# Haochen-Wang409/U2PL

Hardware: AMD Instinct MI355X
Metric: train images/sec at 769x769 (R101-DeepLabv3+) (higher is better)
Workload: dtype f32

## Files before the change

### include/u2pl_hip.h

```cpp
#ifndef U2PL_HIP_H
#define U2PL_HIP_H

#include <stddef.h>
#include <stdint.h>

#ifdef __cplusplus
extern "C" {
#endif

#ifndef __HIP_PLATFORM_AMD__
typedef struct ihipStream_t* hipStream_t;
#endif

#define U2PL_SEL_MAX_SLOTS 8
#define U2PL_SEL_WORD_NVALID 0
#define U2PL_SEL_WORD_NTOTAL 1
#define U2PL_SEL_WORD_VAL 40
#define U2PL_SEL_WORD_THR 56

int u2pl_bilinear_up_f32(const float* in, long sn, long sc, long sh, long sw, int N, int C, int h, int w,
                         float* out_nchw, int H, int W, hipStream_t stream);
int u2pl_bilinear_up_bwd_f32(const float* gout_nchw, int N, int C, int H, int W, float* gin, long sn, long sc,
                             long sh, long sw, int h, int w, hipStream_t stream);
int u2pl_pseudo_label_f32(const float* logits_nchw, int N, int C, int H, int W, float* conf, long long* label,
// ... 32 lines not shown
                          int C, long P, void* workspace, float* proto, const unsigned* lowbits,
                          hipStream_t stream);
size_t u2pl_contra_phase1_workspace_bytes(long P, int C, int D);
int u2pl_contra_phase1(const float* prob, long sn, long sc, long sp, const unsigned* lbits, const float* low_mask,
                       const float* high_mask, int N2, int num_labeled, int C, int h, int w, float thr_p, float thr_n,
                       int low_rank, int high_rank, const float* rows, long ld, int D, unsigned* abits, unsigned* lowbits,
                       unsigned* nbits, int* idx, long cap, unsigned* counts, float* proto, void* workspace,
                       hipStream_t stream);
int u2pl_gather_rows_f32(const float* rows, long ld, int D, const int* list, long n, float* out,
                         hipStream_t stream);
size_t u2pl_bank_state_bytes(int C);
int u2pl_bank_init(long long* state, int C, const long long* caps_host, hipStream_t stream);
int u2pl_bank_enqueue_f32(long long* state, float* storage, int D, const float* rows, long ld, const int* idx,
                          long idx_stride, const long long* row_start_dev, const unsigned* counts_dev, int C,
                          hipStream_t stream);
int u2pl_bank_append_f32(float* bank, long cap, long tail, int D, const float* rows, long ld, const int* list,
                         long n_new, hipStream_t stream);
int u2pl_bank_append_multi_f32(const long long* desc_dev, int nclass, int D, long ld, long max_new,
                               hipStream_t stream);
size_t u2pl_infonce_job_bytes(void);
int u2pl_infonce_f32(const void* jobs_dev, int njobs, const float* rep, long ld, int D, int Q, int K,
                     float temp, float* loss_q, float* ganchor, int* anchor_pix, int* head, int* next,
                     const int* seg_len, hipStream_t stream);
size_t u2pl_infonce_fused_workspace_bytes(int njobs, int Q);
int u2pl_infonce_fused_f32(const void* jobs_dev, int njobs, const float* rep, long ld, int D, int Q, int K, float temp,
                           float* loss_q, float* ganchor, int* anchor_pix, int* head, int* next, const int* seg_len,
                           float* zero_dst, long zero_ld, const int* zero_pix, long zero_n, void* workspace,
                           float inv_valid_seg, float* loss, hipStream_t stream);
int u2pl_infonce_reduce_f32(const float* loss_q, int njobs, int Q, float inv_valid_seg, float* loss,
                            hipStream_t stream);
int u2pl_scatter_rows_ordered_f32(float* dst, long ld, int D, const int* pix, const int* next, int* head,
                                  const int* order, const int* seg_pos, const int* seg_len, const float* src, long n,
                                  const float* gout_dev, float scale, hipStream_t stream);
int u2pl_zero_rows_f32(float* dst, long ld, int D, const int* pix, long n, hipStream_t stream);

size_t u2pl_ce_workspace_bytes(void);
int u2pl_ce_fwd_f32(const float* logits_nchw, const long long* target, int ignore, int N, int C, int H, int W,
                    int unsup_weight, void* workspace, float* out3, hipStream_t stream);
int u2pl_ce_bwd_f32(const float* logits_nchw, const long long* target, int ignore, int N, int C, int H, int W,
                    const float* out3_dev, const float* gout_dev, float gmul, float* grad, hipStream_t stream);
int u2pl_ce_fwd_weighted_f32(const float* logits_nchw, const long long* target, int ignore, int N, int C, int H, int W,
                             const float* class_weight, void* workspace, float* out3, hipStream_t stream);
int u2pl_ce_bwd_weighted_f32(const float* logits_nchw, const long long* target, int ignore, int N, int C, int H, int W,
                             const float* class_weight, const float* out3_dev, const float* gout_dev, float gmul,
                             float* grad, hipStream_t stream);
int u2pl_ohem_prob_f32(const float* logits_nchw, const long long* target, int ignore, int N, int C, int H,
                       int W, float* mask_prob, unsigned* ws, hipStream_t stream);
int u2pl_ohem_apply_i64(const float* mask_prob, const unsigned* thr_bits, const long long* target, int ignore,
                        long n, long long* kept_target, hipStream_t stream);
int u2pl_confusion_hist_f32(const float* logits_nchw, const long long* target, int ignore, int N, int C, int H, int W,
                            long long* hist3c, hipStream_t stream);

int u2pl_predict_map_f32(const float* in, long sn, long sc, long sh, long sw, int N, int C, int h, int w, int H, int W,
                         unsigned char* label, const unsigned char* palette, unsigned char* rgb, hipStream_t stream);
int u2pl_infer_input_u8_f32(const unsigned char* img_hwc, int h, int w, const float* lut, float* out_hwc, int H, int W,
                            hipStream_t stream);
int u2pl_window_fuse_f32(float* pred, float* count, int C, int H, int W, const float* in, long sc, long sh, long sw, int h,
                         int w, int h0, int w0, int hc, int wc, int flip, int softmax, float weight, int bump,
                         hipStream_t stream);
int u2pl_predict_entropy_f32(const float* in, long sn, long sc, long sh, long sw, int N, int C, int h, int w, int H, int W,
                             int prob, unsigned char* label, float* entropy, hipStream_t stream);
int u2pl_reliable_map_u8(unsigned char* label, const float* entropy, const unsigned* thr_bits, long n,
                         const unsigned char* palette, unsigned char* rgb, unsigned char* heat, float heat_scale,
                         unsigned* ndropped, hipStream_t stream);
int u2pl_lut_u8(const unsigned char* in, unsigned char* out, long n, const unsigned char* lut256, hipStream_t stream);

int u2pl_conv2d_fwd_f32(const float* x, long ldx, const float* w, const float* bias, float* y, long ldy, int N,
                        int Hin, int Win, int Cin, int Hout, int Wout, int Cout, int R, int S, int stride,
                        int pad, int dil, hipStream_t stream);
int u2pl_conv2d_fwd_stat_blocks(int N, int Hout, int Wout, int Cout);
int u2pl_conv2d_fwd_bnstats_f32(const float* x, long ldx, const float* w, const float* bias, float* y, long ldy,
                                int N, int Hin, int Win, int Cin, int Hout, int Wout, int Cout, int R, int S,
                                int stride, int pad, int dil, const float* pivot, float* stats_partial,
                                hipStream_t stream);
int u2pl_colreduce_finish_f32(const float* partial, int nblk, int C, double* sums, hipStream_t stream);
int u2pl_conv2d_fwd_bnact_f32(const float* x, long ldx, const float* w, const float* bias, float* y, long ldy, int N,
                              int Hin, int Win, int Cin, int Hout, int Wout, int Cout, int R, int S, int stride,
                              int pad, int dil, const float* mean, const float* invstd, const float* gamma,
                              const float* beta, const float* res, long ldr, int relu, hipStream_t stream);
int u2pl_gemm_batched_f32(const float* x, long ldx, long zx, const float* w, long zw, float* y, long ldy, long zy,
                          long M, int K, int Nn, int batch, hipStream_t stream);
size_t u2pl_wino_tiles(int N, int H, int W, int dil, int mt);
int u2pl_wino_stat_blocks(long tiles, int O);
int u2pl_wino_input_f32(const float* x, long ldx, int N, int H, int W, int C, int dil, int mt, float* V,
                        hipStream_t stream);
int u2pl_wino_weight_f32(const float* w, int O, int C, int transposed, int mt, float* U, hipStream_t stream);
int u2pl_wino_gy_f32(const float* gy, long ldg, int N, int H, int W, int O, int dil, int mt, float* Mg,
                     hipStream_t stream);
int u2pl_wgrad_batched_splits(long M, int Cin, int Cout, int batch);
size_t u2pl_wgrad_batched_workspace_bytes(long M, int Cin, int Cout, int batch);
int u2pl_wgrad_batched_f32(const float* dy, long lddy, long zdy, const float* x, long ldx, long zx, float* part,
                           long M, int Cin, int Cout, int batch, hipStream_t stream);
int u2pl_wino_wgrad_finish_f32(const float* part, int nsplit, int O, int C, int mt, int accumulate, float* dw,
                               hipStream_t stream);
int u2pl_wino_output_f32(const float* Mb, int N, int H, int W, int O, int dil, int mt, const float* bias, float* y,
                         long ldy, float* stats_partial, const float* pivot, hipStream_t stream);
int u2pl_wino_output_bnact_f32(const float* Mb, int N, int H, int W, int O, int dil, int mt, const float* bias, float* y,
                               long ldy, const float* mean, const float* invstd, const float* gamma, const float* beta,
                               const float* res, long ldr, int relu, hipStream_t stream);
int u2pl_conv2d_fwd_bf16op_f32(const float* x, long ldx, const float* w, const float* bias, float* y, long ldy, int N,
                               int Hin, int Win, int Cin, int Hout, int Wout, int Cout, int R, int S, int stride,
                               int pad, int dil, hipStream_t stream);
int u2pl_conv2d_fwd_bnstats_bf16op_f32(const float* x, long ldx, const float* w, const float* bias, float* y, long ldy,
                                       int N, int Hin, int Win, int Cin, int Hout, int Wout, int Cout, int R, int S,
                                       int stride, int pad, int dil, const float* pivot, float* stats_partial,
                                       hipStream_t stream);
int u2pl_conv2d_dgrad_bf16op_f32(const float* dy, long lddy, const float* wT, float* dx, long lddx, int N, int Hin,
                                 int Win, int Cin, int Hout, int Wout, int Cout, int R, int S, int stride, int pad,
                                 int dil, hipStream_t stream);
int u2pl_conv2d_wgrad_bf16op_f32(const float* dy, long lddy, const float* x, long ldx, float* dw, void* workspace,
                                 int accumulate, int N, int Hin, int Win, int Cin, int Hout, int Wout, int Cout, int R,
                                 int S, int stride, int pad, int dil, hipStream_t stream);
int u2pl_conv2d_dgrad_f32(const float* dy, long lddy, const float* wT, float* dx, long lddx, int N, int Hin,
                          int Win, int Cin, int Hout, int Wout, int Cout, int R, int S, int stride, int pad,
                          int dil, hipStream_t stream);
int u2pl_weight_transpose_f32(const float* w, float* wt, int Cout, int RS, int Cin, hipStream_t stream);
size_t u2pl_conv2d_wgrad_workspace_bytes(int N, int Hout, int Wout, int Cin, int Cout, int R, int S);
int u2pl_conv2d_wgrad_f32(const float* dy, long lddy, const float* x, long ldx, float* dw, void* workspace,
                          int accumulate, int N, int Hin, int Win, int Cin, int Hout, int Wout, int Cout, int R,
                          int S, int stride, int pad, int dil, hipStream_t stream);
int u2pl_wgrad_set_tr(int on);
int u2pl_im2col_f32(const float* x, long ldx, float* col, int Kp, int N, int Hin, int Win, int Cin, int Hout,
                    int Wout, int R, int S, int stride, int pad, int dil, hipStream_t stream);

int u2pl_gconv2d_fwd_f32(const float* x, long ldx, const float* w, const float* bias, float* y, long ldy, int N, int Hin,
                         int Win, int Cin, int Hout, int Wout, int Cout, int R, int S, int stride, int pad, int dil,
                         int groups, hipStream_t stream);
int u2pl_gconv2d_dgrad_f32(const float* dy, long lddy, const float* w, float* dx, long lddx, int N, int Hin, int Win,
                           int Cin, int Hout, int Wout, int Cout, int R, int S, int stride, int pad, int dil, int groups,
                           hipStream_t stream);
size_t u2pl_gconv2d_wgrad_workspace_bytes(int N, int Hout, int Wout, int Cin, int Cout, int R, int S, int groups);
int u2pl_gconv2d_wgrad_f32(const float* dy, long lddy, const float* x, long ldx, float* dw, void* workspace,
                           int accumulate, int N, int Hin, int Win, int Cin, int Hout, int Wout, int Cout, int R,
                           int S, int stride, int pad, int dil, int groups, hipStream_t stream);

size_t u2pl_weight_split3_bytes(int rows, int K, int batch);
int u2pl_weight_split3_f32(const float* w, long zw, int rows, int K, int batch, void* out, hipStream_t stream);
int u2pl_weight_split3_multi_f32(const void* jobs, int njobs, long total, hipStream_t stream);
int u2pl_weight_split3_pad_rows(int rows);
int u2pl_wino_weight_multi_f32(const void* jobs, int njobs, long total, hipStream_t stream);
int u2pl_igemm_ws_stat_blocks(int N, int Hout, int Wout);
int u2pl_igemm_ws_set_persist(int on);
int u2pl_conv2d_fwd_ws_f32(const float* x, long ldx, const void* wsplit, const float* bias, float* y, long ldy, int N,
                           int Hin, int Win, int Cin, int Hout, int Wout, int Cout, int R, int S, int stride, int pad,
                           int dil, hipStream_t stream);
int u2pl_conv2d_fwd_bnstats_ws_f32(const float* x, long ldx, const void* wsplit, const float* bias, float* y, long ldy,
                                   int N, int Hin, int Win, int Cin, int Hout, int Wout, int Cout, int R, int S,
                                   int stride, int pad, int dil, const float* pivot, float* stats_partial,
                                   hipStream_t stream);
int u2pl_conv2d_fwd_bnact_ws_f32(const float* x, long ldx, const void* wsplit, const float* bias, float* y, long ldy, int N,
                                 int Hin, int Win, int Cin, int Hout, int Wout, int Cout, int R, int S, int stride,
                                 int pad, int dil, const float* mean, const float* invstd, const float* gamma,
                                 const float* beta, const float* res, long ldr, int relu, hipStream_t stream);
int u2pl_conv2d_dgrad_ws_f32(const float* dy, long lddy, const void* wTsplit, float* dx, long lddx, int N, int Hin,
                             int Win, int Cin, int Hout, int Wout, int Cout, int R, int S, int stride, int pad, int dil,
                             hipStream_t stream);
int u2pl_gemm_batched_ws_f32(const float* x, long ldx, long zx, const void* wsplit, float* y, long ldy, long zy, long M,
                             int K, int Nn, int batch, hipStream_t stream);

size_t u2pl_weight_split2h_bytes(int rows, int K, int batch);
int u2pl_weight_split2h_f32(const float* w, long zw, int rows, int K, int batch, void* out, void* job_scratch, hipStream_t stream);
int u2pl_weight_split2h_multi_f32(const void* jobs, int njobs, long total, hipStream_t stream);
int u2pl_weight_rebuild2h_job_bytes(void);
int u2pl_weight_rebuild2h_span(int which);
int u2pl_weight_rebuild2h_f32(const void* jobs, int n_flat, int n_wino, long seg_total, long amax_total, int wino_mblocks,
                              int wino_pblocks, hipStream_t stream);
int u2pl_amax_words(void);
int u2pl_absmax_f32(const float* x, long ld, long M, int C, float* out, int clear, hipStream_t stream);
int u2pl_bn_apply_amax_f32(const float* x, long ldx, const float* mean, const float* invstd, const float* gamma, const float* beta,
                           const float* res, long ldr, int relu, const float* drop, long rows_per_image, float* y, long ldy, long M,
                           int C, float* y_amax, hipStream_t stream);
int u2pl_bn_bwd_apply_amax_f32(const float* dy, long lddy, const float* x, long ldx, const float* y, long ldy, const float* mean,
                               const float* invstd, const float* gamma, const float* drop, long rows_per_image, const double* sums,
                               double count, float* dx, long lddx, float* dres, long lddr, long M, int C, const double* psums,
                               float* gsink, float* bsink, int accumulate, float* dx_amax, float* dres_amax, const float* relu_beta,
                               hipStream_t stream);
int u2pl_bn_bwd_sums_mx_f32(const float* dy, long lddy, const float* x, long ldx, const float* mean, const float* invstd,
                            const float* gamma, const float* beta, const float* drop, long rows_per_image, long M, int C,
                            void* workspace, double* sums, hipStream_t stream);
int u2pl_bn_apply_bits_f32(const float* x, long ldx, const float* mean, const float* invstd, const float* gamma, const float* beta,
                           const float* res, long ldr, int relu, const float* drop, long rows_per_image, float* y, long ldy, long M,
                           int C, float* y_amax, unsigned* bits, long ldb, hipStream_t stream);
int u2pl_bn_bwd_sums_bits_f32(const float* dy, long lddy, const float* x, long ldx, const unsigned* bits, long ldb,
                              const float* mean, const float* invstd, const float* drop, long rows_per_image, long M, int C,
                              void* workspace, double* sums, hipStream_t stream);
int u2pl_bn_bwd_apply_bits_f32(const float* dy, long lddy, const float* x, long ldx, const unsigned* bits, long ldb,
                               const float* mean, const float* invstd, const float* gamma, const float* drop, long rows_per_image,
                               const double* sums, double count, float* dx, long lddx, float* dres, long lddr, long M, int C,
                               const double* psums, float* gsink, float* bsink, int accumulate, float* dx_amax, float* dres_amax,
                               hipStream_t stream);
int u2pl_wino_input_amax_f32(const float* x, long ldx, int N, int H, int W, int C, int dil, int mt, float* V, float* v_amax,
                             hipStream_t stream);
int u2pl_wino_output_bnact_amax_f32(const float* Mb, int N, int H, int W, int O, int dil, int mt, const float* bias, float* y,
                                    long ldy, const float* mean, const float* invstd, const float* gamma, const float* beta,
                                    const float* res, long ldr, int relu, float* y_amax, hipStream_t stream);
int u2pl_wino_gy_amax_f32(const float* gy, long ldg, int N, int H, int W, int O, int dil, int mt, float* Mg, float* mg_amax,
                          hipStream_t stream);
int u2pl_conv2d_fwd_wsh_f32(const float* x, long ldx, const float* x_amax, const void* wsplit, const float* bias, float* y, long ldy,
                            int N, int Hin, int Win, int Cin, int Hout, int Wout, int Cout, int R, int S, int stride, int pad,
                            int dil, hipStream_t stream);
int u2pl_conv2d_fwd_bnstats_wsh_f32(const float* x, long ldx, const float* x_amax, const void* wsplit, const float* bias, float* y,
                                    long ldy, int N, int Hin, int Win, int Cin, int Hout, int Wout, int Cout, int R, int S,
                                    int stride, int pad, int dil, const float* pivot, float* stats_partial, hipStream_t stream);
int u2pl_conv2d_fwd_bnact_wsh_f32(const float* x, long ldx, const float* x_amax, const void* wsplit, const float* bias, float* y,
                                  long ldy, int N, int Hin, int Win, int Cin, int Hout, int Wout, int Cout, int R, int S,
                                  int stride, int pad, int dil, const float* mean, const float* invstd, const float* gamma,
                                  const float* beta, const float* res, long ldr, int relu, float* y_amax, hipStream_t stream);
int u2pl_conv2d_dgrad_wsh_f32(const float* dy, long lddy, const float* dy_amax, const void* wTsplit, float* dx, long lddx, int N,
                              int Hin, int Win, int Cin, int Hout, int Wout, int Cout, int R, int S, int stride, int pad, int dil,
                              hipStream_t stream);
int u2pl_gemm_batched_wsh_f32(const float* x, long ldx, long zx, const float* x_amax, const void* wsplit, float* y, long ldy, long zy,
                              long M, int K, int Nn, int batch, hipStream_t stream);
int u2pl_wgrad_h_eligible(int Cin, int Cout);
int u2pl_conv2d_wgrad_h_f32(const float* dy, long lddy, const float* dy_amax, const float* x, long ldx, const float* x_amax, float* dw,
                            void* workspace, int accumulate, int N, int Hin, int Win, int Cin, int Hout, int Wout, int Cout, int R,
                            int S, int stride, int pad, int dil, hipStream_t stream);
int u2pl_wgrad_batched_h_f32(const float* dy, long lddy, long zdy, const float* dy_amax, const float* x, long ldx, long zx,
                             const float* x_amax, float* part, long M, int Cin, int Cout, int batch, hipStream_t stream);

size_t u2pl_colreduce_workspace_bytes(long Mseg, int nseg, int C);
int u2pl_bn_stats_f32(const float* x, long ld, long M, int C, const float* pivot, void* workspace, double* sums,
                      hipStream_t stream);
int u2pl_colsum_f32(const float* x, long ld, long Mseg, int nseg, int C, void* workspace, double* sums,
                    hipStream_t stream);
int u2pl_bn_bwd_sums_f32(const float* dy, long lddy, const float* x, long ldx, const float* y, long ldy,
                         const float* mean, const float* invstd, const float* drop, long rows_per_image, long M,
                         int C, void* workspace, double* sums, hipStream_t stream);
int u2pl_bn_finalize_f32(const double* sums, double count, const float* pivot, int C, float eps, float momentum,
                         float* mean, float* invstd, float* running_mean, float* running_var, hipStream_t stream);
int u2pl_bn_eval_invstd_f32(const float* running_var, int C, float eps, float* invstd, hipStream_t stream);
int u2pl_bn_finish_finalize_f32(const float* partial, int nblk, int C, double count, const float* pivot, float eps,
                                float momentum, float* mean, float* invstd, float* running_mean, float* running_var,
                                double* sums_out, hipStream_t stream);
size_t u2pl_bn_eval_invstd_job_bytes(void);
int u2pl_bn_eval_invstd_multi_f32(const void* jobs_dev, int njobs, long total, hipStream_t stream);
int u2pl_bn_apply_f32(const float* x, long ldx, const float* mean, const float* invstd, const float* gamma,
                      const float* beta, const float* res, long ldr, int relu, const float* drop,
                      long rows_per_image, float* y, long ldy, long M, int C, hipStream_t stream);
int u2pl_bn_bwd_apply_f32(const float* dy, long lddy, const float* x, long ldx, const float* y, long ldy,
                          const float* mean, const float* invstd, const float* gamma, const float* drop,
                          long rows_per_image, const double* sums, double count, float* dx, long lddx, float* dres,
                          long lddr, long M, int C, hipStream_t stream);
int u2pl_bn_bwd_apply_pg_f32(const float* dy, long lddy, const float* x, long ldx, const float* y, long ldy,
                             const float* mean, const float* invstd, const float* gamma, const float* drop,
                             long rows_per_image, const double* sums, double count, float* dx, long lddx, float* dres,
                             long lddr, long M, int C, const double* psums, float* gsink, float* bsink, int accumulate,
                             hipStream_t stream);
int u2pl_sums_to_f32(const double* sums, int n, float scale, int accumulate, float* out, hipStream_t stream);
int u2pl_maxpool3s2_fwd_f32(const float* x, long ldx, int N, int H, int W, int C, int Ho, int Wo, float* y, long ldy,
                            unsigned char* tap, hipStream_t stream);
int u2pl_maxpool3s2_bwd_f32(const float* dy, long lddy, const unsigned char* tap, int N, int H, int W, int C, int Ho,
                            int Wo, float* dx, long lddx, hipStream_t stream);
int u2pl_copy_rows_f32(const float* src, long lds, float* dst, long ldd, long M, int C, int accumulate,
                       hipStream_t stream);
int u2pl_copy_cols_f32(const float* src, long lds, float* dst, long ldd, long M, int C, hipStream_t stream);
int u2pl_broadcast_rows_f32(const float* v, long ldv, float scale, float* dst, long ldd, long rows_per_image, long M,
                            int C, hipStream_t stream);
int u2pl_bilinear_rows_fwd_f32(const float* x, long ldx, int N, int h, int w, int C, int H, int W, float* y, long ldy,
                               hipStream_t stream);
int u2pl_bilinear_rows_bwd_f32(const float* dy, long lddy, int N, int h, int w, int C, int H, int W, float* dx,
                               long lddx, hipStream_t stream);
int u2pl_softmax_rows_f32(const float* x, long ldx, float* y, long ldy, long M, int C, hipStream_t stream);
int u2pl_sgd_step_f32(float* p, const float* g, float* buf, long n, long b1, long b2, float lr0, float lr1, float lr2,
                      float momentum, float weight_decay, int first, float grad_scale, hipStream_t stream);
int u2pl_ema_update_f32(float* t, const float* s, long n, float decay, float one_minus_decay, hipStream_t stream);
int u2pl_adam_step_f32(float* p, const float* g, float* exp_avg, float* exp_avg_sq, long n, long b1, long b2, float lr0,
                       float lr1, float lr2, float beta1, float beta2, float eps, float weight_decay,
                       float bias_correction1, float bias_correction2_sqrt, float grad_scale, hipStream_t stream);
size_t u2pl_kernel_launches(void);
int u2pl_conv_set_split(int on);
int u2pl_conv_get_split(void);
int u2pl_debug_phase1_times(unsigned* buf);
size_t u2pl_reliability_fused_workspace_bytes(int G);
size_t u2pl_reliability_fused_cand_floats(long n_px, int G);
int u2pl_reliability_fused(const float* logits_low, long sn, long sc, long sh, long sw, int B, int C, int h, int w,
                           int H, int W, const long long* label_u, const long long* label_l, int ignore, int nspec,
                           const float* q32_host, int negative_high_entropy, int hm, int wm, float* entropy,
                           long long* target_u, float* low_mask, float* high_mask, unsigned* lbits,
                           unsigned* workspace, float* cand, int G, unsigned epoch, int flags, hipStream_t stream);
int u2pl_cutmix_f32(const float* img, const long long* label, const float* conf, const int* boxes_dev, int B, int C,
                    int H, int W, float* out_img, long long* out_label, float* out_conf, hipStream_t stream);

int u2pl_dense_small_f32(const float* x, long ldx, const float* w, const float* bias, float* y, long ldy, int M, int K,
                         int Cout, hipStream_t stream);
int u2pl_strong_aug_f32(const float* img, const long long* label, const float* conf, const int* boxes_dev,
                        const unsigned long long* sel_dev, int mode, int B, int C, int H, int W, float* out_img,
                        long long* out_label, float* out_conf, hipStream_t stream);
int u2pl_label_presence_i64(const long long* label, int B, long HW, unsigned long long* bits, hipStream_t stream);

int u2pl_window_accumulate_f32(float* pred, float* count, int C, int H, int W, const float* src, int h0, int w0,
                               int hc, int wc, hipStream_t stream);
int u2pl_window_normalize_f32(float* pred, const float* count, int C, int H, int W, hipStream_t stream);

int u2pl_augment_u8_f32(const unsigned char* img, const unsigned char* lab, const int* params, int B, int H, int W,
                        int Sh, int Sw, const float* mean3, const float* std3, float* out_img, long long* out_lab,
                        hipStream_t stream);

#define U2PL_AUG_REC 16
#define U2PL_AUG_ROTATE 1
#define U2PL_AUG_BLUR 2
size_t u2pl_augment_ex_scratch_bytes(int B, int Sh, int Sw, int mode);
int u2pl_augment_ex_u8_f32(const unsigned char* img, const unsigned char* lab, const long long* offsets,
                           const int* records, int B, int H, int W, int Sh, int Sw, int ignore_label, int mode,
                           const float* mean3, const float* std3, const float* blur_w, float* scratch, float* out_img,
                           long long* out_lab, hipStream_t stream);
int u2pl_augment_lut_u8_f32(const unsigned char* img, const unsigned char* lab, const long long* offsets,
                            const int* records, int B, int H, int W, int Sh, int Sw, int ignore_label, int mode,
                            const unsigned char* lut256, const float* mean3, const float* std3, const float* blur_w,
                            float* scratch, float* out_img, long long* out_lab, hipStream_t stream);

int u2pl_half_weight_f16(const float* w, int Cout, int Cin, int R, int S, unsigned short* out, hipStream_t stream);
int u2pl_hconv2d_fwd_f16(const unsigned short* x, long ldx, const unsigned short* w, const float* scale,
                         const float* shift, const unsigned short* res, long ldr, void* y, long ldy, int N, int Hin,
                         int Win, int Cin, int Hout, int Wout, int Cout, int R, int S, int stride, int pad, int dil,
                         int relu, int out_f32, int tile, int* sat, hipStream_t stream);
int u2pl_hconv2d_stem_f16(const float* x, long ldx, const unsigned short* w, const float* scale, const float* shift,
                          unsigned short* y, long ldy, int N, int Hin, int Win, int Cin, int Hout, int Wout, int Cout,
                          int R, int S, int stride, int pad, int dil, int relu, int* sat, hipStream_t stream);
int u2pl_hmaxpool3s2_f16(const unsigned short* x, long ldx, int N, int H, int W, int C, int Ho, int Wo,
                         unsigned short* y, long ldy, hipStream_t stream);
int u2pl_hgap_f16(const unsigned short* x, long ldx, int N, int HW, int C, unsigned short* y, hipStream_t stream);
int u2pl_hbilinear_f16(const unsigned short* x, long ldx, int N, int h, int w, int C, unsigned short* y, long ldy,
                       int H, int W, hipStream_t stream);

int u2pl_wide_words(int C);
int u2pl_reliability_masks_wide(const float* entropy, const unsigned* thr_lo_bits, const unsigned* thr_hi_bits,
                                const long long* label_l, const long long* label_u, int ignore, int B, int H, int W,
                                int h, int w, int negative_high_entropy, int C, float* low_mask, float* high_mask,
                                unsigned* lbits, hipStream_t stream);
int u2pl_reliability_apply_wide(const float* entropy, const unsigned* thr_bits, const long long* label_l,
                                const long long* label_u, int ignore, int B, int H, int W, int h, int w,
                                int negative_high_entropy, int C, long long* target_u, unsigned* nkept, float* low_mask,
                                float* high_mask, unsigned* lbits, hipStream_t stream);
int u2pl_pack_class_bits_wide(const long long* onehot, int N, int C, int h, int w, unsigned* bits, hipStream_t stream);
int u2pl_unpack_class_bits_wide(const unsigned* bits, int N, int C, int h, int w, long long* onehot, hipStream_t stream);
size_t u2pl_contra_wide_workspace_bytes(long P, int C);
int u2pl_contra_wide_block_pixels(int C);
int u2pl_contra_wide_staged(int C);
int u2pl_contra_classify_wide(const float* prob, long sn, long sc, long sp, const unsigned* lbits, const float* low_mask,
                              const float* high_mask, int N2, int num_labeled, int C, int h, int w, float thr_p,
                              float thr_n, int low_rank, int high_rank, unsigned* abits, unsigned* lowbits,
                              unsigned* nbits, void* workspace, unsigned* counts, long long* offsets,
                              hipStream_t stream);
int u2pl_compact_lists_wide(const unsigned* abits, const unsigned* lowbits, const unsigned* nbits, long P, int C,
                            const void* workspace, const long long* offsets, int* idx, long idx_len,
                            hipStream_t stream);
int u2pl_class_prototypes_wide(const float* rows, long ld, int D, const int* idx, const long long* offsets,
                               const unsigned* counts, int C, float* proto, hipStream_t stream);
int u2pl_bank_init_wide(long long* state, int C, const long long* caps_host, hipStream_t stream);
int u2pl_bank_enqueue_wide_f32(long long* state, float* storage, int D, const float* rows, long ld, const int* idx,
                               const long long* list_off_dev, const long long* row_start_dev,
                               const unsigned* counts_dev, int C, hipStream_t stream);

#ifdef __cplusplus
}
#endif
#endif
```

### u2pl_amd/csrc/common.h

```cpp
#pragma once
#include <hip/hip_runtime.h>
#include <stdint.h>

#define U2PL_API extern "C" __attribute__((visibility("default")))

#define U2PL_LAUNCH_CHECK()                      \
    do {                                         \
        hipError_t e__ = hipGetLastError();      \
        if (e__ != hipSuccess) return (int)e__;  \
    } while (0)

#define U2PL_EINVAL 1001

#include <atomic>
extern std::atomic<unsigned long long> u2pl_kernel_launch_count;
#define U2PL_LAUNCH(...)                        \
    do {                                        \
        u2pl_kernel_launch_count.fetch_add(1, std::memory_order_relaxed);             \
        hipLaunchKernelGGL(__VA_ARGS__);        \
    } while (0)

#ifdef U2PL_HBM_MAXW
#define U2PL_HBM_KERNEL __attribute__((amdgpu_waves_per_eu(1, U2PL_HBM_MAXW)))
#else
// ... 2 lines not shown

static inline int cdiv(long a, long b) { return (int)((a + b - 1) / b); }
static inline int grid_for(long n, int block, int max_blocks = 256 * 16) {
    long g = (n + block - 1) / block;
    if (g > max_blocks) g = max_blocks;
    if (g < 1) g = 1;
    return (int)g;
}

__device__ __forceinline__ float wave_sum(float v) {
#pragma unroll
    for (int o = 32; o > 0; o >>= 1) v += __shfl_xor(v, o, 64);
    return v;
}
template <int CTRL>
__device__ __forceinline__ float dpp_add(float v) {
    return v + __builtin_bit_cast(float, __builtin_amdgcn_update_dpp(0, __builtin_bit_cast(int, v), CTRL, 0xf, 0xf, false));
}
__device__ __forceinline__ float wave_allsum_dpp(float v) {
    v = dpp_add<0x128>(v);
    v = dpp_add<0x124>(v);
    v = dpp_add<0x122>(v);
    v = dpp_add<0x121>(v);
    const int b = __builtin_bit_cast(int, v);
    const float r0 = __builtin_bit_cast(float, __builtin_amdgcn_readlane(b, 0)), r1 = __builtin_bit_cast(float, __builtin_amdgcn_readlane(b, 16));
    const float r2 = __builtin_bit_cast(float, __builtin_amdgcn_readlane(b, 32)), r3 = __builtin_bit_cast(float, __builtin_amdgcn_readlane(b, 48));
    return (r0 + r1) + (r2 + r3);
}
__device__ __forceinline__ float wave_sum_sgpr(float v) {
    v = dpp_add<0x128>(v);
    v = dpp_add<0x124>(v);
    v = dpp_add<0x122>(v);
    v = dpp_add<0x121>(v);
    v += __builtin_bit_cast(float, __builtin_amdgcn_update_dpp(0, __builtin_bit_cast(int, v), 0x142, 0xa, 0xf, false));
    v += __builtin_bit_cast(float, __builtin_amdgcn_update_dpp(0, __builtin_bit_cast(int, v), 0x143, 0xc, 0xf, false));
    return __builtin_bit_cast(float, __builtin_amdgcn_readlane(__builtin_bit_cast(int, v), 63));
}
__device__ __forceinline__ float lane_put(float old, float val, int lane) {
    return (int)(threadIdx.x & 63) == lane ? val : old;
}
__device__ __forceinline__ float lane_get(float v, int lane) {
    return __builtin_bit_cast(float, __builtin_amdgcn_readlane(__builtin_bit_cast(int, v), lane));
}
__device__ __forceinline__ double wave_sum_d(double v) {
#pragma unroll
    for (int o = 32; o > 0; o >>= 1) v += __shfl_xor(v, o, 64);
    return v;
}
__device__ __forceinline__ unsigned wave_sum_u(unsigned v) {
#pragma unroll
    for (int o = 32; o > 0; o >>= 1) v += __shfl_xor(v, o, 64);
    return v;
}
__device__ __forceinline__ float wave_max(float v) {
#pragma unroll
    for (int o = 32; o > 0; o >>= 1) v = fmaxf(v, __shfl_xor(v, o, 64));
    return v;
}

#define U2PL_AMAX_SHARDS 64
#define U2PL_AMAX_STRIDE 32
#define U2PL_AMAX_WORDS (U2PL_AMAX_SHARDS * U2PL_AMAX_STRIDE)
__device__ __forceinline__ unsigned amax_bits(unsigned m, float v) {
    const unsigned b = __float_as_uint(v) & 0x7fffffffu;
    return b > m ? b : m;
}
__device__ __forceinline__ unsigned amax_bits4(unsigned m, float4 v) {
    return amax_bits(amax_bits(amax_bits(amax_bits(m, v.x), v.y), v.z), v.w);
}
__device__ __forceinline__ unsigned wave_max_u(unsigned m) {
#pragma unroll
    for (int o = 32; o > 0; o >>= 1) {
        const unsigned t = (unsigned)__shfl_xor((int)m, o, 64);
        m = t > m ? t : m;
    }
    return m;
}
__device__ __forceinline__ void amax_wave_publish(unsigned m, unsigned* __restrict__ obj) {
    m = wave_max_u(m);
    if ((threadIdx.x & 63) == 0 && m != 0u) {
        const unsigned wave = blockIdx.x * (blockDim.x >> 6) + (threadIdx.x >> 6);
        atomicMax(obj + (wave & (U2PL_AMAX_SHARDS - 1)) * U2PL_AMAX_STRIDE, m);
    }
}
__device__ __forceinline__ unsigned amax_read(const unsigned* __restrict__ obj) {
    const unsigned v = *(const __attribute__((address_space(1))) unsigned*)(obj + (threadIdx.x & 63) * U2PL_AMAX_STRIDE);
    return (unsigned)__builtin_amdgcn_readfirstlane((int)wave_max_u(v));
}

__device__ __forceinline__ void block_count_flush(unsigned cnt, unsigned* __restrict__ dst) {
    __shared__ unsigned s_cnt;
    if (threadIdx.x == 0) s_cnt = 0;
    __syncthreads();
    cnt = wave_sum_u(cnt);
    if ((threadIdx.x & 63) == 0 && cnt) atomicAdd(&s_cnt, cnt);
    __syncthreads();
    if (threadIdx.x == 0 && s_cnt) atomicAdd(dst, s_cnt);
}

__device__ __forceinline__ unsigned f32_key(float f) {
    unsigned u = __float_as_uint(f);
    return (u & 0x80000000u) ? ~u : (u | 0x80000000u);
}
__device__ __forceinline__ float key_f32(unsigned k) {
    unsigned u = (k & 0x80000000u) ? (k & 0x7fffffffu) : ~k;
    return __uint_as_float(u);
}

struct AcCoord {
    int i0, i1;
    float l0, l1;
};
__device__ __forceinline__ AcCoord ac_coord(int dst, float scale, int in_size) {
    AcCoord c;
    float src = __fmul_rn((float)dst, scale);
    c.i0 = (int)src;
    if (c.i0 > in_size - 1) c.i0 = in_size - 1;
    c.i1 = c.i0 + (c.i0 < in_size - 1 ? 1 : 0);
    c.l1 = __fsub_rn(src, (float)c.i0);
    c.l0 = __fsub_rn(1.0f, c.l1);
    return c;
}
static inline float ac_scale_host(long in, long out) {
    return out > 1 ? (float)(in - 1) / (float)(out - 1) : 0.0f;
}
__device__ __forceinline__ int nearest_src(int dst, float scale, int in_size) {
    int s = (int)floorf(__fmul_rn((float)dst, scale));
    return s < in_size - 1 ? s : in_size - 1;
}

typedef unsigned int u32x4 __attribute__((ext_vector_type(4)));
#define OOB_OFF ((int)0x80000000u)
__device__ __forceinline__ __amdgpu_buffer_rsrc_t make_rsrc(const void* p, unsigned bytes) {
    return __builtin_amdgcn_make_buffer_rsrc((void*)p, (short)0, (int)bytes, 0x00020000);
}
__device__ __forceinline__ float4 buf_load4s(__amdgpu_buffer_rsrc_t r, int lane_off, int uniform_off) {
    u32x4 v = __builtin_amdgcn_raw_buffer_load_b128(r, lane_off, uniform_off, 0);
    return make_float4(__uint_as_float(v.x), __uint_as_float(v.y), __uint_as_float(v.z), __uint_as_float(v.w));
}
__device__ __forceinline__ float4 buf_load4(__amdgpu_buffer_rsrc_t r, int byte_off) {
    u32x4 v = __builtin_amdgcn_raw_buffer_load_b128(r, byte_off, 0, 0);
    return make_float4(__uint_as_float(v.x), __uint_as_float(v.y), __uint_as_float(v.z), __uint_as_float(v.w));
}

#define U2PL_GLOBAL __attribute__((address_space(1)))
template <class T>
__device__ __forceinline__ T ldg(const T* p) { return *(const U2PL_GLOBAL T*)p; }

struct BnEpi {
    const float *mean, *invstd, *gamma, *beta, *res;
    long ldr;
    int relu;
    unsigned* y_amax;
};
```

### u2pl_amd/csrc/igemm_ws.hip

```cpp
#include <stdlib.h>
#include <type_traits>
#include "common.h"
#include "conv_geom.h"
#include "u2pl_hip.h"
#include "wino_t.h"

template <int B, int E, class F>
__device__ __forceinline__ void static_for(F&& f) {
    if constexpr (B < E) {
        f(std::integral_constant<int, B>{});
        static_for<B + 1, E>(f);
    }
}

#define WS_ROW_B 64
__host__ __device__ static inline int ws_pad_rows(int rows) { return rows <= 128 ? 128 : (rows + 255) & ~255; }

__global__ void k_weight_split3(const float* __restrict__ w, long zw, unsigned short* __restrict__ out, long zo, int rows,
                                int Np, int K) {
    w += (long)blockIdx.y * zw;
    out += (long)blockIdx.y * zo;
    const int nseg = K / 8;
    const long total = (long)Np * nseg;
    for (long i = blockIdx.x * (long)blockDim.x + threadIdx.x; i < total; i += (long)gridDim.x * blockDim.x) {
// ... 371 lines not shown
        const unsigned dk_q = (8u * dq) / Cout, dk_r = 8u * dq - dk_q * Cout;
        for (; i < jend; i += 256) {
            const int n = j.kind == 0 ? (int)slow : (int)fst, sg = j.kind == 0 ? (int)fst : (int)slow;
            float4 v0 = make_float4(0.f, 0.f, 0.f, 0.f), v1 = v0;
            if (n < j.rows) {
                if (j.kind == 0) {
                    const float4* src = (const float4*)(j.src + (long)n * j.K + sg * 8);
                    v0 = src[0];
                    v1 = src[1];
                } else {
                    float e[8];
                    unsigned rs = rs0, co = co0;
#pragma unroll
                    for (int q = 0; q < 8; ++q) {
                        e[q] = j.src[((long)co * j.RS + rs) * j.rows + n];
                        if (++co == Cout) { co = 0; ++rs; }
                    }
                    v0 = make_float4(e[0], e[1], e[2], e[3]);
                    v1 = make_float4(e[4], e[5], e[6], e[7]);
                }
            }
            uint2 a0, a1, b0, b1;
            split2_f16(v0, sc, a0, a1);
            split2_f16(v1, sc, b0, b1);
            const int c = sg >> 2, s_ = sg & 3;
            const long base = (((long)c * 2) * j.Np + n) * 32 + ((s_ ^ ((n >> 2) & 3)) << 3);
            *(uint4*)(j.out + base) = make_uint4(a0.x, a0.y, b0.x, b0.y);
            *(uint4*)(j.out + base + pl) = make_uint4(a1.x, a1.y, b1.x, b1.y);
            slow += dq;
            fst += dr;
            rs0 += dk_q;
            co0 += dk_r;
            if (fst >= fast) { fst -= fast; ++slow; co0 += 8u; }
            while (co0 >= Cout) { co0 -= Cout; ++rs0; }
        }
        if (i >= end) return;
    }
}
template <int MT>
__device__ __forceinline__ void rb_pieces_wino(const RebuildJob& j, int lb) {
    constexpr int A = WinoT<MT>::A;
    const bool tr = j.kind == 3;
    const int C = tr ? j.rows : j.K;
    const unsigned total = (unsigned)j.Np * (unsigned)(j.K >> 3);
    const unsigned* __restrict__ amax = rb_tail(j);
    const long pl = (long)j.Np * 32, zs = (long)(j.K / 32) * 2 * pl;
    unsigned u = (unsigned)lb * RB_WINO_PSPAN + threadIdx.x;
    const int s_ = (int)(u & 3);
    int c = (int)((u >> 2) / (unsigned)j.Np), n = (int)((u >> 2) - (unsigned)c * (unsigned)j.Np);
    for (int it = 0; it < RB_WINO_PSPAN / 256 && u < total; ++it, u += 256) {
        const int k0 = c * 32 + s_ * 8;
        const bool live = n < j.rows;
        float tp[9][8];
        if (!tr) {
            const float* __restrict__ p = j.src + (long)(live ? n : 0) * 9 * C + k0;
#pragma unroll
            for (int t = 0; t < 9; ++t) {
                const float4 lo = *(const float4*)(p + (long)t * C), hi = *(const float4*)(p + (long)t * C + 4);
                tp[t][0] = lo.x; tp[t][1] = lo.y; tp[t][2] = lo.z; tp[t][3] = lo.w;
                tp[t][4] = hi.x; tp[t][5] = hi.y; tp[t][6] = hi.z; tp[t][7] = hi.w;
            }
        } else {
            const float* __restrict__ p = j.src + (long)k0 * 9 * C + (live ? n : 0);
#pragma unroll
            for (int q = 0; q < 8; ++q)
#pragma unroll
                for (int t = 0; t < 9; ++t) tp[8 - t][q] = p[((long)q * 9 + t) * C];
        }
        unsigned short* __restrict__ out = j.out + (((long)c * 2) * j.Np + n) * 32 + ((s_ ^ ((n >> 2) & 3)) << 3);
        static_for<0, A>([&](auto i_c) __attribute__((always_inline)) {
            constexpr int I = decltype(i_c)::value;
            float comp[A][8];
#pragma unroll
            for (int q = 0; q < 8; ++q) {
                float r[A];
                wino_filter_row<MT, I>([&](int r_, int s) { return tp[r_ * 3 + s][q]; }, r);
#pragma unroll
                for (int jj = 0; jj < A; ++jj) comp[jj][q] = live ? r[jj] : 0.f;
            }
#pragma unroll
            for (int jj = 0; jj < A; ++jj) {
                const int z = I * A + jj;
                const float sc = split2_scale(split2_exp_bits(amax[z]));
                uint2 a0, a1, b0, b1;
                split2_f16(make_float4(comp[jj][0], comp[jj][1], comp[jj][2], comp[jj][3]), sc, a0, a1);
                split2_f16(make_float4(comp[jj][4], comp[jj][5], comp[jj][6], comp[jj][7]), sc, b0, b1);
                *(uint4*)(out + z * zs) = make_uint4(a0.x, a0.y, b0.x, b0.y);
                *(uint4*)(out + z * zs + pl) = make_uint4(a1.x, a1.y, b1.x, b1.y);
            }
        });
        n += 64;
        if (n >= j.Np) { n -= j.Np; ++c; }
    }
}
__global__ __launch_bounds__(256) void k_rebuild_pieces_wino(const RebuildJob* __restrict__ wj, int n_wino) {
    const int b = (int)blockIdx.x;
    const int ji = rb_find(n_wino, b, [&](int m) { return (long)wj[m].pblk_begin; });
    const RebuildJob j = wj[ji];
    if (j.mt == 4) rb_pieces_wino<4>(j, b - j.pblk_begin);
    else rb_pieces_wino<2>(j, b - j.pblk_begin);
}
U2PL_API int u2pl_weight_rebuild2h_job_bytes(void) { return (int)sizeof(RebuildJob); }
U2PL_API int u2pl_weight_rebuild2h_span(int which) { return which == 0 ? WS_AMAX_SPAN : which == 1 ? RB_WINO_MSPAN : which == 2 ? RB_WINO_PSPAN : 0; }
U2PL_API int u2pl_weight_rebuild2h_f32(const void* jobs, int n_flat, int n_wino, long seg_total, long amax_total, int wino_mblocks,
                                       int wino_pblocks, hipStream_t stream) {
    if (n_flat < 0 || n_wino < 0 || seg_total < 0 || amax_total < 0 || wino_mblocks < 0 || wino_pblocks < 0) return U2PL_EINVAL;
    if ((n_flat == 0) != (seg_total == 0) || (n_flat == 0) != (amax_total == 0)) return U2PL_EINVAL;
    if ((n_wino == 0) != (wino_mblocks == 0) || (n_wino == 0) != (wino_pblocks == 0)) return U2PL_EINVAL;
    if (n_flat + n_wino == 0) return 0;
    const RebuildJob* rj = (const RebuildJob*)jobs;
    const int flat_blocks = cdiv(amax_total, WS_AMAX_SPAN);
    U2PL_LAUNCH(k_rebuild_clear, dim3(cdiv(n_flat + n_wino, 256)), dim3(256), 0, stream, rj, n_flat + n_wino);
    U2PL_LAUNCH_CHECK();
    U2PL_LAUNCH(k_rebuild_amax, dim3((unsigned)(flat_blocks + wino_mblocks)), dim3(256), 0, stream, rj, n_flat, n_wino, amax_total, flat_blocks);
    U2PL_LAUNCH_CHECK();
    if (n_flat) {
        U2PL_LAUNCH(k_rebuild_pieces_flat, dim3((unsigned)cdiv(seg_total, WS_AMAX_SPAN)), dim3(256), 0, stream, rj, n_flat, seg_total);
        U2PL_LAUNCH_CHECK();
    }
    if (n_wino) {
        U2PL_LAUNCH(k_rebuild_pieces_wino, dim3((unsigned)wino_pblocks), dim3(256), 0, stream, rj + n_flat, n_wino);
        U2PL_LAUNCH_CHECK();
    }
    return 0;
}
__global__ void k_absmax_rows(const float* __restrict__ x, long ld, long M, int C4, unsigned* __restrict__ out) {
    const long total = M * C4;
    unsigned m = 0;
    for (long i = blockIdx.x * (long)blockDim.x + threadIdx.x; i < total; i += (long)gridDim.x * blockDim.x) {
        const long r = i / C4;
        const int c = (int)(i - r * C4);
        m = amax_bits4(m, *(const float4*)(x + r * ld + c * 4));
    }
    amax_wave_publish(m, out);
}
U2PL_API int u2pl_amax_words(void) { return U2PL_AMAX_WORDS; }
U2PL_API int u2pl_absmax_f32(const float* x, long ld, long M, int C, float* out, int clear, hipStream_t stream) {
    if (M < 0 || C <= 0 || (C & 3) || (ld & 3)) return U2PL_EINVAL;
    if (clear) {
        hipError_t e = hipMemsetAsync(out, 0, (size_t)U2PL_AMAX_WORDS * 4, stream);
        if (e != hipSuccess) return (int)e;
    }
    if (M == 0) return 0;
    U2PL_LAUNCH(k_absmax_rows, dim3(grid_for(M * (C / 4), 512, 2048)), dim3(512), 0, stream, x, ld, M, C / 4, (unsigned*)out);
    U2PL_LAUNCH_CHECK();
    return 0;
}

#ifdef U2PL_WS_STAMPS
__device__ unsigned long long* d_ws_stamps;
static unsigned long long* g_ws_stamps = nullptr;
U2PL_API int u2pl_igemm_ws_set_stamp_buffer(void* p) { g_ws_stamps = (unsigned long long*)p; return 0; }
#endif
template <int TM, int TN, int WM, int WN, bool PW, int ABL = 0, int NP = 3>
__device__ __forceinline__ void igemm_ws_body(
    const float* __restrict__ x, long ldx, const float* __restrict__ x_amax, const unsigned short* __restrict__ ws,
    const unsigned* __restrict__ b_amax, const float* __restrict__ bias,
    float* __restrict__ y, long ldy, const ConvGeom& g, unsigned xbytes, unsigned wsbytes, unsigned ybytes, unsigned resbytes, int Np,
    float* __restrict__ stats, const float* __restrict__ pivot, long zx, long zws, long zy, const BnEpi& epi, int mtiles, int ntiles,
    int total_tiles, int tile0, const int bid, const int G) {
    constexpr int BM = 32 * TM * WM, BN = 32 * TN * WN, NT = 64 * WM * WN;
    constexpr int RPP = NT / 8, RA = BM / RPP;
    constexpr int UB = NP * BN * 4, RBU = UB / NT;
    static_assert(BM % RPP == 0 && UB % NT == 0, "tile / thread-count mismatch");
    static_assert(NP == 2 || NP == 3, "pieces per operand");
    constexpr int A_ST = NP * BM * WS_ROW_B, B_ST = NP * BN * WS_ROW_B, ST = A_ST + B_ST;
    constexpr int NPROD = NP == 3 ? 6 : 3;
    using C0 = std::integral_constant<int, 0>;
    using C1 = std::integral_constant<int, 1>;

    auto tile_of = [&](int v, int& mt, int& nt, int& z) __attribute__((always_inline)) {
        const int xcd = v & 7, j = v >> 3;
        const int q = total_tiles >> 3, r = total_tiles & 7;
        const int t = tile0 + (xcd < r ? xcd * (q + 1) : r * (q + 1) + (xcd - r) * q) + j;
        nt = t % ntiles;
        const int rest = t / ntiles;
        mt = rest % mtiles;
        z = rest / mtiles;
    };
    __amdgpu_buffer_rsrc_t rx = make_rsrc(x, xbytes), rw = make_rsrc(ws, wsbytes), ry = make_rsrc(y, ybytes);
    extern __shared__ __attribute__((aligned(16))) unsigned char smem[];
#ifdef U2PL_WS_STAMPS
    unsigned long long ph[4];
    ph[0] = __builtin_readcyclecounter();
#endif

    const int tid = threadIdx.x, lane = tid & 63, wave = tid >> 6;
    const int wm = wave / WN, wn = wave % WN;
    const long M = (long)g.N * g.Hout * g.Wout;
    const int K = g.R * g.S * g.Cin;
    const int nk = K / BK;
    int ea = 0;
    float sa = 1.f;
    if constexpr (NP == 2) {
        ea = split2_exp_bits(amax_read((const unsigned*)x_amax));
        sa = split2_scale(ea);
    }
    const int nk2 = (nk + 1) & ~1;
    const int n_my = (total_tiles - bid + G - 1) / G;
    const int cpt = g.S * (g.Cin / BK);
    auto tile_taps = [&](int mt, int& rb_, int& re_) __attribute__((always_inline)) {
        rb_ = 0;
        re_ = g.R;
        if constexpr (!PW) {
            if (g.R > 1) {
                const long mf = (long)mt * BM, ml_ = mf + BM - 1, ml = ml_ < M ? ml_ : M - 1;
                const unsigned hw = (unsigned)(g.Hout * g.Wout);
                const unsigned nf = (unsigned)mf / hw, nl = (unsigned)ml / hw;
                const int hf = (int)(((unsigned)mf - nf * hw) / (unsigned)g.Wout), hl = (int)(((unsigned)ml - nl * hw) / (unsigned)g.Wout);
                const int lim = g.Hin << g.log2div;
                auto reach = [&](int r, int ha, int hb) { return hb * g.mul + g.off_h + r * g.step >= 0 && ha * g.mul + g.off_h + r * g.step < lim; };
                int lo = g.R, hi = -1;
                for (int r = 0; r < g.R; ++r) {
                    const bool ok = nf == nl ? reach(r, hf, hl)
                                             : (reach(r, hf, g.Hout - 1) || reach(r, 0, hl) || (nl > nf + 1 && reach(r, 0, g.Hout - 1)));
                    if (ok) { lo = r < lo ? r : lo; hi = r; }
                }
                if (hi >= 0) { rb_ = lo; re_ = hi + 1; } else { rb_ = 0; re_ = 1; }
                rb_ = __builtin_amdgcn_readfirstlane(rb_);
                re_ = __builtin_amdgcn_readfirstlane(re_);
            }
        }
    };

    const int kq = tid & 7, r0 = tid >> 3;
    const int ldxb = (int)ldx * 4;
    int a_v = bid, a_kc = 0, a_c0 = 0, a_r = 0, a_s = 0;
    int a_nk = nk, a_nk2 = nk2;
    int bh[RA], bw[RA], nb[RA];
    bool mv[RA];
    int aoff[RA];
    auto a_tile_setup = [&]() __attribute__((always_inline)) {
        int mt, nt, z;
        tile_of(a_v, mt, nt, z);
        rx = make_rsrc(x + (long)__builtin_amdgcn_readfirstlane(z) * zx, xbytes);
        if constexpr (!PW) {
            int rb_, re_;
            tile_taps(mt, rb_, re_);
            a_r = rb_;
            a_nk = (re_ - rb_) * cpt;
            a_nk2 = (a_nk + 1) & ~1;
        }
#pragma unroll
        for (int i = 0; i < RA; ++i) {
            const long m = (long)mt * BM + r0 + RPP * i;
            mv[i] = m < M;
            const unsigned mm = mv[i] ? (unsigned)m : 0u;
            if constexpr (PW) {
                aoff[i] = mv[i] ? (int)mm * ldxb + kq * 16 : OOB_OFF;
            } else {
                const unsigned tq = mm / (unsigned)g.Wout;
                const int wo = (int)(mm - tq * (unsigned)g.Wout);
                const unsigned n_ = tq / (unsigned)g.Hout;
                const int ho = (int)(tq - n_ * (unsigned)g.Hout);
                bh[i] = ho * g.mul + g.off_h;
                bw[i] = wo * g.mul + g.off_w;
                nb[i] = (int)n_ * g.Hin * g.Win;
            }
        }
    };
    a_tile_setup();
    float4 ra[2][RA];
    u32x4 rb[RBU];
    auto load_a_row = [&](auto set_c, auto i_c) __attribute__((always_inline)) {
        constexpr int SET = decltype(set_c)::value, i = decltype(i_c)::value;
        const bool live = a_kc < a_nk;
        if constexpr (PW) {
            ra[SET][i] = buf_load4s(rx, live ? aoff[i] : OOB_OFF, a_kc * (BK * 4));
        } else {
            int ih, iw;
            const bool okh = gather_coord(bh[i], a_r, g.step, g.log2div, g.Hin, ih);
            const bool okw = gather_coord(bw[i], a_s, g.step, g.log2div, g.Win, iw);
            const int off = (nb[i] + ih * g.Win + iw) * ldxb + kq * 16;
            ra[SET][i] = buf_load4s(rx, (live & mv[i] & okh & okw) ? off : OOB_OFF, a_c0 * 4);
        }
    };
    auto advance_a = [&]() __attribute__((always_inline)) {
        if (a_kc + 1 < a_nk2) {
            ++a_kc;
            a_c0 += BK;
            if (a_c0 == g.Cin) {
                a_c0 = 0;
                if (++a_s == g.S) { a_s = 0; ++a_r; }
            }
        } else if (a_v + G < total_tiles) {
            a_v += G;
            a_kc = a_c0 = a_r = a_s = 0;
            a_tile_setup();
        }
    };
    auto load_a = [&](auto set_c) __attribute__((always_inline)) {
        static_for<0, RA>([&](auto i) __attribute__((always_inline)) { load_a_row(set_c, i); });
        advance_a();
    };
    int boff[RBU];
    int blds[RBU];
#pragma unroll
    for (int j = 0; j < RBU; ++j) {
        const int u = tid + j * NT, p = u / (BN * 4), wi = u - p * (BN * 4);
        boff[j] = p * Np * WS_ROW_B + wi * 16;
        blds[j] = A_ST + p * BN * WS_ROW_B + wi * 16;
    }
    const int chunk_b = NP * Np * WS_ROW_B;
    int b_v = bid, b_kc = 0, b_toff = 0;
    int b_nk = nk, b_nk2 = nk2, b_base = 0;
    auto b_tile_setup = [&]() __attribute__((always_inline)) {
        int mt, nt, z;
// ... 138 lines not shown
        constexpr int LD_START = (BS_START + RBU + RBU + RA <= NMF) ? BS_START + RBU : NMF - RBU - RA;
        static_assert(F1_START + NRD <= TAIL + NPROD * PER, "k block 1 operands would be read after their first use");
        static_assert(LD_START + RBU + RA <= NMF && LD_START >= BS_START && LD_START >= SP_START + SP_N, "plan does not fit the chunk");
        using CUR = std::integral_constant<int, cur>;
#ifdef U2PL_WS_STAMPS
        unsigned long long ts[14];
        ts[0] = __builtin_readcyclecounter();
#endif
        if constexpr (!(ABL & 16)) static_for<0, F0_PRE>([&](auto j) __attribute__((always_inline)) { do_read(CUR{}, C0{}, j); });
        __builtin_amdgcn_sched_barrier(0);
        static_for<0, NMF>([&](auto sl_c) __attribute__((always_inline)) {
            constexpr int sl = decltype(sl_c)::value;
#ifdef U2PL_WS_STAMPS
            if constexpr (sl % 4 == 0 && sl != 0) ts[sl / 4] = __builtin_readcyclecounter();
#endif
            do_mfma(std::integral_constant<int, (sl < TAIL ? NMF - TAIL + sl : sl - TAIL)>{});
            if constexpr (!(ABL & 16)) {
                if constexpr (sl < TAIL)
                    static_for<0, F0_PER>([&](auto u) __attribute__((always_inline)) { do_read(CUR{}, C0{}, std::integral_constant<int, F0_PRE + sl * F0_PER + decltype(u)::value>{}); });
                if constexpr (sl >= F1_START) do_read(CUR{}, C1{}, std::integral_constant<int, sl - F1_START>{});
            }
            if constexpr (sl >= SP_START && sl < SP_START + SP_N) {
                constexpr int k = (sl - SP_START) / SPS, step = (sl - SP_START) % SPS;
                if constexpr (step == 0) {
                    const float4 v = ra[nxt][k >> 1];
                    sp_l = (k & 1) ? v.z : v.x;
                    sp_h = (k & 1) ? v.w : v.y;
                }
                unsigned w;
                if constexpr (ABL & 1) w = (__float_as_uint(sp_h) & 0xffff0000u) | (__float_as_uint(sp_l) >> 16);
                else if constexpr (NP == 2) {
                    if constexpr (step == 0) w = split2_first(sp_l, sp_h, sa);
                    else w = split2_second(sp_l, sp_h, sa, (k & 1) ? pc[0].y : pc[0].x);
                } else {
                    if constexpr (step == 0) w = pack2_bf16_first(sp_l, sp_h);
                    else w = pack2_bf16(sp_l, sp_h);
                    if constexpr (step < 2) {
                        sp_l = sp_l - bf16_lo_f(w);
                        sp_h = sp_h - bf16_hi_f(w);
                    }
                }
                if constexpr (k & 1) pc[step].y = w; else pc[step].x = w;
                if constexpr ((k & 1) && step == SPS - 1) {
                    if constexpr (ABL & 4) {
                        asm volatile("" ::"v"(pc[0].x), "v"(pc[0].y), "v"(pc[1].x), "v"(pc[1].y));
                        if constexpr (NP == 3) asm volatile("" ::"v"(pc[2].x), "v"(pc[2].y));
                    } else {
                        unsigned char* d = smem + nxt * ST + alds[k >> 1];
                        *(uint2*)d = pc[0];
                        *(uint2*)(d + BM * WS_ROW_B) = pc[1];
                        if constexpr (NP == 3) *(uint2*)(d + 2 * BM * WS_ROW_B) = pc[2];
                    }
                }
            }
            if constexpr (sl >= BS_START && sl < BS_START + RBU) {
                constexpr int k = sl - BS_START;
                if constexpr (ABL & 2) { asm volatile("" ::"v"(rb[k].x), "v"(rb[k].y), "v"(rb[k].z), "v"(rb[k].w)); }
                else store_b(nxt, k);
            }
            if constexpr (!(ABL & 8)) {
                if constexpr (sl >= LD_START && sl < LD_START + RBU) {
                    load_b_unit(std::integral_constant<int, sl - LD_START>{});
                    if constexpr (sl == LD_START + RBU - 1) advance_b();
                }
                if constexpr (sl >= LD_START + RBU && sl < LD_START + RBU + RA) {
                    load_a_row(std::integral_constant<int, nxt>{}, std::integral_constant<int, sl - LD_START - RBU>{});
                    if constexpr (sl == LD_START + RBU + RA - 1) advance_a();
                }
            }
            __builtin_amdgcn_sched_barrier(0);
        });
#ifdef U2PL_WS_STAMPS
        ts[12] = __builtin_readcyclecounter();
#endif
        if constexpr (!(ABL & 32)) __syncthreads();
#ifdef U2PL_WS_STAMPS
        ts[13] = __builtin_readcyclecounter();
        {
            const int bsel = blockIdx.x == 0 ? 0 : blockIdx.x == 100 ? 1 : -1;
            if (d_ws_stamps && bsel >= 0 && kc >= 8 && kc < 12 && (wave == 0 || wave == (WM * WN) / 2) && lane == 0)
                for (int i = 0; i < 14; ++i) d_ws_stamps[((bsel * 2 + (wave != 0)) * 4 + (kc - 8)) * 14 + i] = ts[i];
        }
#endif
    };

    int c_v = bid;
    int c_nk2 = nk2;
    auto c_tile_setup = [&]() __attribute__((always_inline)) {
        if constexpr (!PW) {
            if (c_v < total_tiles) {
                int mt, nt, z, rb_, re_;
                tile_of(c_v, mt, nt, z);
                tile_taps(mt, rb_, re_);
                c_nk2 = ((re_ - rb_) * cpt + 1) & ~1;
            }
        }
    };
    c_tile_setup();
    float* red = (float*)(smem + 2 * ST);
    unsigned y_am = 0u;
#ifdef U2PL_WS_STAMPS
    int te_n = 0;
#endif
    auto tile_end = [&]() __attribute__((always_inline)) {
#ifdef U2PL_WS_STAMPS
        unsigned long long te[5];
        te[0] = __builtin_readcyclecounter();
#endif
        int mt, nt, z;
        tile_of(c_v, mt, nt, z);
        const int n0 = nt * BN;
        const long m0 = (long)mt * BM;
        int tid = threadIdx.x;
        asm volatile("" : "+v"(tid));
        const int lane = tid & 63, li = lane & 31, lh = lane >> 5;
        (void)lane;
        const int zs = __builtin_amdgcn_readfirstlane(z);
        ry = make_rsrc(y + (long)zs * zy, ybytes);
        const bool bn_all = epi.mean != nullptr;
        const unsigned cbytes = (unsigned)g.Cout * 4u;
        auto colparam = [&](const float* p, int col) __attribute__((always_inline)) {
            return p ? __uint_as_float(__builtin_amdgcn_raw_buffer_load_b32(make_rsrc(p, cbytes), col * 4, 0, 0)) : 0.f;
        };
        float bias_v[TN], mu[TN], is[TN], ga[TN], be[TN], pv[TN];
#pragma unroll
        for (int b = 0; b < TN; ++b) {
            const int col = n0 + wn * 32 * TN + b * 32 + li;
            bias_v[b] = colparam(bias, col);
            mu[b] = is[b] = ga[b] = be[b] = pv[b] = 0.f;
            if (bn_all) { mu[b] = colparam(epi.mean, col); is[b] = colparam(epi.invstd, col); ga[b] = colparam(epi.gamma, col); be[b] = colparam(epi.beta, col); }
            if (stats) pv[b] = colparam(pivot, col);
        }
        int dexp = 0;
        if constexpr (NP == 2) dexp = -(ea + split2_exp_bits(__builtin_amdgcn_readfirstlane((int)ldg(b_amax + zs))));
        __builtin_amdgcn_sched_barrier(0);
        static_for<0, TAIL>([&](auto sl) __attribute__((always_inline)) { do_mfma(std::integral_constant<int, NMF - TAIL + decltype(sl)::value>{}); });
        if constexpr (NP == 2) {
#pragma unroll
            for (int a = 0; a < TM; ++a)
#pragma unroll
                for (int b = 0; b < TN; ++b)
#pragma unroll
                    for (int e = 0; e < 16; ++e) acc[a][b][e] = __builtin_ldexpf(acc[a][b][e], dexp);
        }
#ifdef U2PL_WS_STAMPS
        te[1] = te[2] = __builtin_readcyclecounter();
#endif
        __builtin_amdgcn_sched_barrier(0);
        const int ldyb = (int)ldy * 4;
        const int mrow = (int)m0 + wm * 32 * TM + 4 * lh;
        if (bn_all) {
            const int ldrb = (int)epi.ldr * 4;
            const __amdgpu_buffer_rsrc_t rr = make_rsrc(epi.res, resbytes);
#pragma unroll
            for (int b = 0; b < TN; ++b) {
                const int col = n0 + wn * 32 * TN + b * 32 + li;
                float rv[TM][16];
                if (epi.res) {
#pragma unroll
                    for (int a = 0; a < TM; ++a) {
                        const int rbase = col < g.Cout ? ((mrow + a * 32) * (int)epi.ldr + col) * 4 : OOB_OFF;
#pragma unroll
                        for (int e = 0; e < 16; ++e)
                            rv[a][e] = __uint_as_float(__builtin_amdgcn_raw_buffer_load_b32(rr, rbase + ((e & 3) + 8 * (e >> 2)) * ldrb, 0, 0));
                    }
                }
#pragma unroll
                for (int a = 0; a < TM; ++a)
#pragma unroll
                    for (int e = 0; e < 16; ++e) {
                        float v = acc[a][b][e] + bias_v[b];
                        v = (v - mu[b]) * is[b] * ga[b] + be[b];
                        if (epi.res) v += rv[a][e];
                        if (epi.relu) v = fmaxf(v, 0.f);
                        acc[a][b][e] = v;
                        if (epi.y_amax && col < g.Cout && (long)(mrow + a * 32 + (e & 3) + 8 * (e >> 2)) < M) y_am = amax_bits(y_am, v);
                    }
            }
            __builtin_amdgcn_sched_barrier(0);
        }
#pragma unroll
        for (int b = 0; b < TN; ++b) {
            const int col = n0 + wn * 32 * TN + b * 32 + li;
            const float badd = bn_all ? 0.f : bias_v[b];
#pragma unroll
            for (int a = 0; a < TM; ++a) {
                const int vbase = col < g.Cout ? ((mrow + a * 32) * (int)ldy + col) * 4 : OOB_OFF;
#pragma unroll
                for (int e = 0; e < 16; ++e) {
                    const float v = bn_all ? acc[a][b][e] : acc[a][b][e] + badd;
                    __builtin_amdgcn_raw_buffer_store_b32(__float_as_uint(v), ry, vbase + ((e & 3) + 8 * (e >> 2)) * ldyb, 0, 0);
                }
            }
        }
        __builtin_amdgcn_sched_barrier(0);
        if (stats && !bn_all) {
            static_assert(BM == 128, "statistics blocks are 128 rows");
            const long left = M - m0;
            const int lim = (int)(left < BM ? left : BM) - (wm * 32 * TM + 4 * lh);
#pragma unroll
            for (int b = 0; b < TN; ++b) {
                const int cl = wn * 32 * TN + b * 32 + li;
                const float sh = bias_v[b] - pv[b];
#pragma unroll
                for (int a = 0; a < TM; ++a) {
                    float s1 = 0.f, s2 = 0.f;
#pragma unroll
                    for (int e = 0; e < 16; ++e) {
                        const float v = (a * 32 + (e & 3) + 8 * (e >> 2)) < lim ? acc[a][b][e] + sh : 0.f;
                        s1 += v;
                        s2 += v * v;
                    }
                    s1 += __shfl_xor(s1, 32, 64);
                    s2 += __shfl_xor(s2, 32, 64);
                    if (lh == 0) {
                        red[((wm * TM + a) * 2 + 0) * BN + cl] = s1;
                        red[((wm * TM + a) * 2 + 1) * BN + cl] = s2;
                    }
                }
            }
            __syncthreads();
            float* out = stats + (long)mt * 2 * g.Cout;
            for (int c = tid; c < BN; c += NT) {
                const int co = n0 + c;
                if (co < g.Cout) {
                    float a1 = red[0 * BN + c], a2 = red[1 * BN + c];
#pragma unroll
                    for (int r = 1; r < 4; ++r) { a1 += red[(2 * r) * BN + c]; a2 += red[(2 * r + 1) * BN + c]; }
                    out[co] = a1;
                    out[g.Cout + co] = a2;
                }
            }
        }
#pragma unroll
        for (int a = 0; a < TM; ++a)
#pragma unroll
            for (int b = 0; b < TN; ++b)
#pragma unroll
                for (int e = 0; e < 16; ++e) acc[a][b][e] = 0.f;
        zero_tail_operands();
        c_v += G;
        c_tile_setup();
#ifdef U2PL_WS_STAMPS
        te[3] = __builtin_readcyclecounter();
        asm volatile("s_waitcnt vmcnt(0)" ::: "memory");
        te[4] = __builtin_readcyclecounter();
        if (d_ws_stamps && blockIdx.x == 0 && (wave == 0 || wave == 5) && lane == 0 && te_n < 4)
            for (int i = 0; i < 5; ++i) d_ws_stamps[224 + 4096 + ((wave != 0) * 4 + te_n) * 5 + i] = te[i];
        ++te_n;
#endif
    };
    for (int it = 0; it < n_my; ++it) {
        for (kc = 0; kc < c_nk2; kc += 2) {
            chunk(C0{});
            chunk(C1{});
        }
        tile_end();
    }
    if (epi.y_amax) amax_wave_publish(y_am, epi.y_amax);
#ifdef U2PL_WS_STAMPS
    ph[2] = ph[3] = __builtin_readcyclecounter();
    if (d_ws_stamps && blockIdx.x < 1024 && tid == 0)
        for (int i = 0; i < 4; ++i) d_ws_stamps[224 + blockIdx.x * 4 + i] = ph[i];
#endif
}

template <int TM, int TN, int WM, int WN, bool PW, int ABL = 0, int NP = 3>
__global__ __launch_bounds__(64 * WM * WN, (WM * WN) / 4) void k_igemm_ws(
    const float* __restrict__ x, long ldx, const float* __restrict__ x_amax, const unsigned short* __restrict__ ws,
    const unsigned* __restrict__ b_amax, const float* __restrict__ bias,
    float* __restrict__ y, long ldy, ConvGeom g, unsigned xbytes, unsigned wsbytes, unsigned ybytes, unsigned resbytes, int Np,
    float* __restrict__ stats, const float* __restrict__ pivot, long zx, long zws, long zy, BnEpi epi, int mtiles, int ntiles,
    int total_tiles, int tile0) {
    igemm_ws_body<TM, TN, WM, WN, PW, ABL, NP>(x, ldx, x_amax, ws, b_amax, bias, y, ldy, g, xbytes, wsbytes, ybytes, resbytes, Np, stats,
                                               pivot, zx, zws, zy, epi, mtiles, ntiles, total_tiles, tile0, (int)blockIdx.x, (int)gridDim.x);
}
template <bool PW, int NP = 3>
__global__ __launch_bounds__(512, 2) void k_igemm_ws_mix(
    const float* __restrict__ x, long ldx, const float* __restrict__ x_amax, const unsigned short* __restrict__ ws,
    const unsigned* __restrict__ b_amax, const float* __restrict__ bias,
    float* __restrict__ y, long ldy, ConvGeom g, unsigned xbytes, unsigned wsbytes, unsigned ybytes, unsigned resbytes, int Np,
    float* __restrict__ stats, const float* __restrict__ pivot, long zx, long zws, long zy, BnEpi epi, int mtiles, int ntiles_w,
    int nwide, int wide_tiles, int narrow_tiles) {
    if ((int)blockIdx.x < nwide)
        igemm_ws_body<2, 2, 2, 4, PW, 0, NP>(x, ldx, x_amax, ws, b_amax, bias, y, ldy, g, xbytes, wsbytes, ybytes, resbytes, Np, stats, pivot,
                                             zx, zws, zy, epi, mtiles, ntiles_w, wide_tiles, 0, (int)blockIdx.x, nwide);
    else
        igemm_ws_body<2, 1, 2, 4, PW, 0, NP>(x, ldx, x_amax, ws, b_amax, bias, y, ldy, g, xbytes, wsbytes, ybytes, resbytes, Np, stats, pivot,
                                             zx, zws, zy, epi, mtiles, 2 * ntiles_w, narrow_tiles, 2 * wide_tiles, (int)blockIdx.x - nwide,
                                             (int)gridDim.x - nwide);
}

#define WS_NUM_CUS 256
static double ws_fix2() {
    static double v = -1.0;
    if (v < 0) { const char* e = getenv("U2PL_WS_FIX2"); v = (e && *e) ? atof(e) : 2.0; }
    return v;
}
static int g_ws_persist = -1;
static int ws_persist() {
    if (g_ws_persist < 0) { const char* e = getenv("U2PL_WS_PERSIST"); g_ws_persist = (e && *e) ? (atoi(e) != 0) : 1; }
    return g_ws_persist;
}
U2PL_API int u2pl_igemm_ws_set_persist(int on) { const int old = ws_persist(); g_ws_persist = on != 0; return old; }
template <int TM, int TN, int WM, int WN, bool PW, int ABL = 0, int NP = 3>
static int launch_igemm_ws(const float* x, long ldx, const float* x_amax, const void* ws, const float* bias, float* y, long ldy,
                           const ConvGeom& g, hipStream_t stream, float* stats, const float* pivot, int batch, long zx,
                           long zy, const BnEpi* epi, long tile_first = 0, long tile_count = -1) {
    constexpr int BM = 32 * TM * WM, BN = 32 * TN * WN;
    const long M = (long)g.N * g.Hout * g.Wout;
    if (M <= 0) return 0;
    const int K = g.R * g.S * g.Cin, Np = ws_pad_rows(g.Cout);
    const BnEpi ep = epi ? *epi : BnEpi{nullptr, nullptr, nullptr, nullptr, nullptr, 0, 0, nullptr};
    const size_t lds = (size_t)2 * NP * (BM + BN) * WS_ROW_B + (size_t)8 * BN * sizeof(float);
    static bool attr_set = false;
    if (!attr_set) {
        (void)hipFuncSetAttribute((const void*)k_igemm_ws<TM, TN, WM, WN, PW, ABL, NP>, hipFuncAttributeMaxDynamicSharedMemorySize, (int)lds);
        attr_set = true;
    }
    if (NP == 2 && !x_amax) return U2PL_EINVAL;
    const long xb = (((long)g.N * g.Hin * g.Win - 1) * ldx + g.Cin) * 4;
    const long yb = ((M - 1) * ldy + g.Cout) * 4;
    const long wsb1 = (long)(K / 32) * NP * Np * WS_ROW_B;
    const unsigned* b_amax = (const unsigned*)((const char*)ws + (size_t)batch * wsb1);
    if (xb >= (1L << 31) || wsb1 >= (1L << 31) || yb >= (1L << 31)) return U2PL_EINVAL;
    const long resb = ep.res ? ((M - 1) * ep.ldr + g.Cout) * 4 : 0;
    if (resb >= (1L << 31)) return U2PL_EINVAL;
    const int mtiles = cdiv(M, BM), ntiles = cdiv(g.Cout, BN);
    const long all_tiles = (long)mtiles * ntiles * batch;
    if (all_tiles >= (1L << 30)) return U2PL_EINVAL;
    const long total = tile_count < 0 ? all_tiles : tile_count;
    if (total <= 0) return 0;
    const unsigned grid = (unsigned)((total < WS_NUM_CUS || !ws_persist()) ? total : WS_NUM_CUS);
#ifdef U2PL_WS_STAMPS
    (void)hipMemcpyToSymbolAsync(HIP_SYMBOL(d_ws_stamps), &g_ws_stamps, sizeof(void*), 0, hipMemcpyHostToDevice, stream);
#endif
    U2PL_LAUNCH((k_igemm_ws<TM, TN, WM, WN, PW, ABL, NP>), dim3(grid), dim3(64 * WM * WN), lds, stream, x, ldx, x_amax,
                (const unsigned short*)ws, b_amax, bias, y, ldy, g, (unsigned)xb, (unsigned)wsb1, (unsigned)yb, (unsigned)resb, Np, stats, pivot, zx,
                wsb1 / 2, zy, ep, mtiles, ntiles, (int)total, (int)tile_first);
    U2PL_LAUNCH_CHECK();
    return 0;
}

template <bool PW, int NP = 3>
static int launch_igemm_ws_mix(const float* x, long ldx, const float* x_amax, const void* ws, const float* bias, float* y, long ldy,
                               const ConvGeom& g, hipStream_t stream, float* stats, const float* pivot, int batch, long zx,
                               long zy, const BnEpi* epi, long wide_tiles, long narrow_tiles) {
    const long M = (long)g.N * g.Hout * g.Wout;
    const int K = g.R * g.S * g.Cin, Np = ws_pad_rows(g.Cout);
    const BnEpi ep = epi ? *epi : BnEpi{nullptr, nullptr, nullptr, nullptr, nullptr, 0, 0, nullptr};
    const size_t lds = (size_t)2 * NP * (128 + 256) * WS_ROW_B + (size_t)8 * 256 * sizeof(float);
    static bool attr_set = false;
    if (!attr_set) {
        (void)hipFuncSetAttribute((const void*)k_igemm_ws_mix<PW, NP>, hipFuncAttributeMaxDynamicSharedMemorySize, (int)lds);
        attr_set = true;
    }
    if (NP == 2 && !x_amax) return U2PL_EINVAL;
    const long xb = (((long)g.N * g.Hin * g.Win - 1) * ldx + g.Cin) * 4;
    const long yb = ((M - 1) * ldy + g.Cout) * 4;
    const long wsb1 = (long)(K / 32) * NP * Np * WS_ROW_B;
    const unsigned* b_amax = (const unsigned*)((const char*)ws + (size_t)batch * wsb1);
    if (xb >= (1L << 31) || wsb1 >= (1L << 31) || yb >= (1L << 31)) return U2PL_EINVAL;
    const long resb = ep.res ? ((M - 1) * ep.ldr + g.Cout) * 4 : 0;
    if (resb >= (1L << 31)) return U2PL_EINVAL;
    const int mtiles = cdiv(M, 128), ntw = cdiv(g.Cout, 256);
    if ((long)mtiles * 2 * ntw * batch >= (1L << 30)) return U2PL_EINVAL;
    U2PL_LAUNCH((k_igemm_ws_mix<PW, NP>), dim3((unsigned)(WS_NUM_CUS + narrow_tiles)), dim3(512), lds, stream, x, ldx, x_amax,
                (const unsigned short*)ws, b_amax, bias, y, ldy, g, (unsigned)xb, (unsigned)wsb1, (unsigned)yb, (unsigned)resb, Np, stats, pivot, zx,
                wsb1 / 2, zy, ep, mtiles, ntw, WS_NUM_CUS, (int)wide_tiles, (int)narrow_tiles);
    U2PL_LAUNCH_CHECK();
    return 0;
}

#ifdef U2PL_WS_ABLATE
static int g_ws_abl = 0;
U2PL_API int u2pl_igemm_ws_set_ablate(int v) { const int old = g_ws_abl; g_ws_abl = v; return old; }
#endif

template <int NP>
static int run_igemm_ws_np(const float* x, long ldx, const float* x_amax, const void* ws, const float* bias, float* y, long ldy,
                           const ConvGeom& g, hipStream_t stream, float* stats, const float* pivot, int batch, long zx, long zy,
                           const BnEpi* epi) {
    if (g.Cin % BK || !ws) return U2PL_EINVAL;
    if (epi && (stats || batch != 1 || (g.Cout & 3))) return U2PL_EINVAL;
    const bool pw = g.R == 1 && g.S == 1 && g.mul == 1 && g.off_h == 0 && g.off_w == 0 && g.log2div == 0 &&
                    g.Hin == g.Hout && g.Win == g.Wout;
    auto go = [&](bool narrow, long first, long count) {
        if (!narrow) return pw ? launch_igemm_ws<2, 2, 2, 4, true, 0, NP>(x, ldx, x_amax, ws, bias, y, ldy, g, stream, stats, pivot, batch, zx, zy, epi, first, count)
                               : launch_igemm_ws<2, 2, 2, 4, false, 0, NP>(x, ldx, x_amax, ws, bias, y, ldy, g, stream, stats, pivot, batch, zx, zy, epi, first, count);
        return pw ? launch_igemm_ws<2, 1, 2, 4, true, 0, NP>(x, ldx, x_amax, ws, bias, y, ldy, g, stream, stats, pivot, batch, zx, zy, epi, first, count)
                  : launch_igemm_ws<2, 1, 2, 4, false, 0, NP>(x, ldx, x_amax, ws, bias, y, ldy, g, stream, stats, pivot, batch, zx, zy, epi, first, count);
    };
#ifdef U2PL_WS_ABLATE
    if (g_ws_abl && g.Cout > 128 && pw) {
#define WS_ABL(A_) case A_: return launch_igemm_ws<2, 2, 2, 4, true, A_, NP>(x, ldx, x_amax, ws, bias, y, ldy, g, stream, stats, pivot, batch, zx, zy, epi)
        switch (g_ws_abl) { WS_ABL(1); WS_ABL(2); WS_ABL(4); WS_ABL(8); WS_ABL(16); WS_ABL(32); WS_ABL(7); WS_ABL(15); WS_ABL(31); WS_ABL(63); default: return U2PL_EINVAL; }
#undef WS_ABL
    }
#endif
    if (g.Cout <= 128) return go(true, 0, -1);
    static int force = -2;
    if (force == -2) { const char* e = getenv("U2PL_WS_NARROW"); force = (e && *e) ? atoi(e) : -1; }
    const long M_ = (long)g.N * g.Hout * g.Wout;
    const long mt = cdiv(M_, 128), nkc = (long)(g.R * g.S * g.Cin) / BK;
    const long ntw = cdiv(g.Cout, 256), ntn = cdiv(g.Cout, 128);
    const long tw = mt * ntw * batch, tn = mt * ntn * batch;
    const double fix = NP == 3 ? 1.0 : ws_fix2();
    const double cw1 = nkc + 4.0 * fix, cn1 = 0.5 * 1.15 * nkc + 2.0 * fix;
    const double cw = (double)cdiv(tw, WS_NUM_CUS) * cw1, cn = (double)cdiv(tn, WS_NUM_CUS) * cn1;
    if (force == 0) return go(false, 0, -1);
    if (force == 1) return go(g.Cout <= 256, 0, -1);
    const long full = tw / WS_NUM_CUS * WS_NUM_CUS, rem = tw - full;
    const bool can_mix = force != 2 && ws_persist() && ntn == 2 * ntw && full > 0 && rem > 0 && 2 * rem <= WS_NUM_CUS;
    static int two_launch = -1;
    if (two_launch < 0) { const char* e = getenv("U2PL_WS_MIX2"); two_launch = (e && *e) ? (atoi(e) != 0) : 0; }
    const double cm = can_mix ? (double)(full / WS_NUM_CUS) * cw1 + cn1 + (two_launch ? 8.0 : 2.0) * fix : 1e30;
    if (cm < 0.97 * cw && cm < cn) {
        if (!two_launch)
            return pw ? launch_igemm_ws_mix<true, NP>(x, ldx, x_amax, ws, bias, y, ldy, g, stream, stats, pivot, batch, zx, zy, epi, full, 2 * rem)
                      : launch_igemm_ws_mix<false, NP>(x, ldx, x_amax, ws, bias, y, ldy, g, stream, stats, pivot, batch, zx, zy, epi, full, 2 * rem);
        const int rc = go(false, 0, full);
        return rc ? rc : go(true, 2 * full, 2 * rem);
    }
    return go(cn < 0.97 * cw, 0, -1);
}

static int run_igemm_ws(const float* x, long ldx, const void* ws, const float* bias, float* y, long ldy, const ConvGeom& g,
                        hipStream_t stream, float* stats = nullptr, const float* pivot = nullptr, int batch = 1,
                        long zx = 0, long zy = 0, const BnEpi* epi = nullptr, const float* x_amax = nullptr) {
    return x_amax ? run_igemm_ws_np<2>(x, ldx, x_amax, ws, bias, y, ldy, g, stream, stats, pivot, batch, zx, zy, epi)
                  : run_igemm_ws_np<3>(x, ldx, nullptr, ws, bias, y, ldy, g, stream, stats, pivot, batch, zx, zy, epi);
}

U2PL_API int u2pl_igemm_ws_stat_blocks(int N, int Hout, int Wout) { return cdiv((long)N * Hout * Wout, 128); }

U2PL_API int u2pl_conv2d_fwd_ws_f32(const float* x, long ldx, const void* wsplit, const float* bias, float* y, long ldy,
                                    int N, int Hin, int Win, int Cin, int Hout, int Wout, int Cout, int R, int S,
                                    int stride, int pad, int dil, hipStream_t stream) {
    ConvGeom g = {N, Hin, Win, Cin, Hout, Wout, Cout, R, S, stride, -pad, -pad, dil, 0};
    return run_igemm_ws(x, ldx, wsplit, bias, y, ldy, g, stream);
}
U2PL_API int u2pl_conv2d_fwd_bnstats_ws_f32(const float* x, long ldx, const void* wsplit, const float* bias, float* y,
                                            long ldy, int N, int Hin, int Win, int Cin, int Hout, int Wout, int Cout,
                                            int R, int S, int stride, int pad, int dil, const float* pivot,
                                            float* stats_partial, hipStream_t stream) {
    ConvGeom g = {N, Hin, Win, Cin, Hout, Wout, Cout, R, S, stride, -pad, -pad, dil, 0};
    return run_igemm_ws(x, ldx, wsplit, bias, y, ldy, g, stream, stats_partial, pivot);
}
U2PL_API int u2pl_conv2d_fwd_bnact_ws_f32(const float* x, long ldx, const void* wsplit, const float* bias, float* y,
                                          long ldy, int N, int Hin, int Win, int Cin, int Hout, int Wout, int Cout, int R,
                                          int S, int stride, int pad, int dil, const float* mean, const float* invstd,
                                          const float* gamma, const float* beta, const float* res, long ldr, int relu,
                                          hipStream_t stream) {
    if (!mean || !invstd || !gamma || !beta || (Cout & 3) || (res && (ldr & 3))) return U2PL_EINVAL;
    ConvGeom g = {N, Hin, Win, Cin, Hout, Wout, Cout, R, S, stride, -pad, -pad, dil, 0};
    const BnEpi epi = {mean, invstd, gamma, beta, res, ldr, relu, nullptr};
    return run_igemm_ws(x, ldx, wsplit, bias, y, ldy, g, stream, nullptr, nullptr, 1, 0, 0, &epi);
}
U2PL_API int u2pl_conv2d_dgrad_ws_f32(const float* dy, long lddy, const void* wTsplit, float* dx, long lddx, int N, int Hin,
                                      int Win, int Cin, int Hout, int Wout, int Cout, int R, int S, int stride, int pad,
                                      int dil, hipStream_t stream) {
    int l2 = 0;
    while ((1 << l2) < stride) ++l2;
    if ((1 << l2) != stride) return U2PL_EINVAL;
    ConvGeom g = {N, Hout, Wout, Cout, Hin, Win, Cin, R, S, 1, pad, pad, -dil, l2};
    return run_igemm_ws(dy, lddy, wTsplit, nullptr, dx, lddx, g, stream);
}
U2PL_API int u2pl_gemm_batched_ws_f32(const float* x, long ldx, long zx, const void* wsplit, float* y, long ldy, long zy,
                                      long M, int K, int Nn, int batch, hipStream_t stream) {
    if (M <= 0 || batch <= 0) return 0;
    if (M >= (1L << 31)) return U2PL_EINVAL;
    ConvGeom g = {1, (int)M, 1, K, (int)M, 1, Nn, 1, 1, 1, 0, 0, 1, 0};
    return run_igemm_ws(x, ldx, wsplit, nullptr, y, ldy, g, stream, nullptr, nullptr, batch, zx, zy);
}

U2PL_API int u2pl_conv2d_fwd_wsh_f32(const float* x, long ldx, const float* x_amax, const void* wsplit, const float* bias, float* y, long ldy,
                                     int N, int Hin, int Win, int Cin, int Hout, int Wout, int Cout, int R, int S,
                                     int stride, int pad, int dil, hipStream_t stream) {
    if (!x_amax) return U2PL_EINVAL;
    ConvGeom g = {N, Hin, Win, Cin, Hout, Wout, Cout, R, S, stride, -pad, -pad, dil, 0};
    return run_igemm_ws(x, ldx, wsplit, bias, y, ldy, g, stream, nullptr, nullptr, 1, 0, 0, nullptr, x_amax);
}
U2PL_API int u2pl_conv2d_fwd_bnstats_wsh_f32(const float* x, long ldx, const float* x_amax, const void* wsplit, const float* bias, float* y,
                                             long ldy, int N, int Hin, int Win, int Cin, int Hout, int Wout, int Cout,
                                             int R, int S, int stride, int pad, int dil, const float* pivot,
                                             float* stats_partial, hipStream_t stream) {
    if (!x_amax) return U2PL_EINVAL;
    ConvGeom g = {N, Hin, Win, Cin, Hout, Wout, Cout, R, S, stride, -pad, -pad, dil, 0};
    return run_igemm_ws(x, ldx, wsplit, bias, y, ldy, g, stream, stats_partial, pivot, 1, 0, 0, nullptr, x_amax);
}
U2PL_API int u2pl_conv2d_fwd_bnact_wsh_f32(const float* x, long ldx, const float* x_amax, const void* wsplit, const float* bias, float* y,
                                           long ldy, int N, int Hin, int Win, int Cin, int Hout, int Wout, int Cout, int R,
                                           int S, int stride, int pad, int dil, const float* mean, const float* invstd,
                                           const float* gamma, const float* beta, const float* res, long ldr, int relu,
                                           float* y_amax, hipStream_t stream) {
    if (!x_amax || !mean || !invstd || !gamma || !beta || (Cout & 3) || (res && (ldr & 3))) return U2PL_EINVAL;
    ConvGeom g = {N, Hin, Win, Cin, Hout, Wout, Cout, R, S, stride, -pad, -pad, dil, 0};
    const BnEpi epi = {mean, invstd, gamma, beta, res, ldr, relu, (unsigned*)y_amax};
    return run_igemm_ws(x, ldx, wsplit, bias, y, ldy, g, stream, nullptr, nullptr, 1, 0, 0, &epi, x_amax);
}
U2PL_API int u2pl_conv2d_dgrad_wsh_f32(const float* dy, long lddy, const float* dy_amax, const void* wTsplit, float* dx, long lddx, int N,
                                       int Hin, int Win, int Cin, int Hout, int Wout, int Cout, int R, int S, int stride, int pad,
                                       int dil, hipStream_t stream) {
    if (!dy_amax) return U2PL_EINVAL;
    int l2 = 0;
    while ((1 << l2) < stride) ++l2;
    if ((1 << l2) != stride) return U2PL_EINVAL;
    ConvGeom g = {N, Hout, Wout, Cout, Hin, Win, Cin, R, S, 1, pad, pad, -dil, l2};
    return run_igemm_ws(dy, lddy, wTsplit, nullptr, dx, lddx, g, stream, nullptr, nullptr, 1, 0, 0, nullptr, dy_amax);
}
U2PL_API int u2pl_gemm_batched_wsh_f32(const float* x, long ldx, long zx, const float* x_amax, const void* wsplit, float* y, long ldy,
                                       long zy, long M, int K, int Nn, int batch, hipStream_t stream) {
    if (!x_amax) return U2PL_EINVAL;
    if (M <= 0 || batch <= 0) return 0;
    if (M >= (1L << 31)) return U2PL_EINVAL;
    ConvGeom g = {1, (int)M, 1, K, (int)M, 1, Nn, 1, 1, 1, 0, 0, 1, 0};
    return run_igemm_ws(x, ldx, wsplit, nullptr, y, ldy, g, stream, nullptr, nullptr, batch, zx, zy, nullptr, x_amax);
}
```

### u2pl_amd/graphs.py

```python
import os
import warnings

import torch
import torch.distributed as dist

from . import _lib
from . import nn as K

WARM = int(os.environ.get("U2PL_GRAPH_WARM", "2"))
STATS = {"captures": 0, "replays": 0, "eager": 0, "aborted": 0}


def enabled():
    if os.environ.get("U2PL_GRAPHS", "1") == "0" or _lib.PROFILE is not None or K.DROPOUT_HOOK is not None:
        return False
    if K.dist_active():
        return False
    return True


_WARNED = set()


def _capture_failed(name, ent, exc):
    ent["failed"] = ent.get("failed", 0) + 1
    STATS["aborted"] += 1
    key = (name, ent["failed"] >= 2)
    if key not in _WARNED:
        _WARNED.add(key)
        warnings.warn("u2pl_amd.graphs: capture of segment '%s' aborted (%s: %s); %s" % (
            name, type(exc).__name__, str(exc)[:300],
            "the segment stays eager from now on" if ent["failed"] >= 2 else "running it eagerly, one more capture attempt follows"),
            RuntimeWarning, stacklevel=3)
    if os.environ.get("U2PL_GRAPH_DEBUG"):
        raise exc


def _bns(modules):
    return [m for mod in modules for m in mod.modules() if isinstance(m, K.BatchNorm2d)]


class _Capture:

    def __init__(self, graph, bns, pool=None):
        self.graph, self.bns, self.pool = graph, bns, pool

    def __enter__(self):
        self.nbt0 = [m._nbt for m in self.bns]
        self.ctx = torch.cuda.graph(self.graph, pool=self.pool, capture_error_mode="thread_local")
        self.ctx.__enter__()
        _lib.CAPTURING[0] = True
        K.amax_pool_reset()
        return self

    def __exit__(self, et, ev, tb):
        _lib.CAPTURING[0] = False
        K.amax_pool_reset()
        try:
            self.ctx.__exit__(et, ev, tb)
        finally:
            self.bumps = [(m, m._nbt - n0) for m, n0 in zip(self.bns, self.nbt0) if m._nbt != n0]
            for m, n0 in zip(self.bns, self.nbt0):
                m._nbt = n0
        return False


def _conv_weights(modules):
    return [p for mod in modules for p in mod.parameters() if p.dim() == 4]


def _refresh_operands(ent, modules, owner):
    ws = ent.get("weights")
    if ws is None:
        ws = ent["weights"] = _conv_weights(modules)
    sig = (K.WEIGHT_EPOCH[0], sum(p._version for p in ws))
    if sig != ent.get("sig"):
        if ent.get("sig") is not None:
            K.presplit(ws, owner)
        ent["sig"] = sig


def _key(xs, modules):
    algo = tuple(sorted(K.CONV_ALGO.items())) + (K.CONV_WS["on"], K.CONV_H["on"], _lib.query("u2pl_conv_get_split"), K.FUSE_EVAL_BN,
                                                 K._WGRAD["enabled"], K.FUSE_BN_FINISH, K.FUSE_RES_GRAD, K.RELU_MASK_FROM_X)
    bn = tuple(b.training for mod in modules for b in mod.modules() if isinstance(b, K.BatchNorm2d))
    rg = tuple(p.requires_grad for mod in modules for p in mod.parameters())
    return (tuple((tuple(x.shape), x.dtype, x.device.index) for x in xs) + tuple(m.training for m in modules) + algo
            + (hash(bn), hash(rg)))


class GraphedNoGrad:

    def __init__(self, fn, modules, name, uniforms=None):
        self.fn, self.modules, self.name, self.cache, self.uniforms = fn, list(modules), name, {}, uniforms

    def _eager(self, xs):
        STATS["eager"] += 1
        n = self.uniforms(xs) if self.uniforms else 0
        with K.dropout_pool(torch.empty(n, device=xs[0].device).uniform_() if n else None):
            return self.fn(*xs)

    def __call__(self, *xs):
        if not enabled():
            return self._eager(xs)
        key = _key(xs, self.modules)
        ent = self.cache.setdefault(key, {"count": 0, "graph": None})
        if ent["graph"] is None:
            if ent["count"] < WARM or ent.get("failed", 0) >= 2:
                ent["count"] += 1
                return self._eager(xs)
            static_in = [x.clone() for x in xs]
            K.prewarm_globals(self.modules, xs[0].device)
            n = self.uniforms(xs) if self.uniforms else 0
            u = torch.empty(n, device=xs[0].device) if n else None
            g = torch.cuda.CUDAGraph()
            cap = _Capture(g, _bns(self.modules))
            try:
                with cap, K.dropout_pool(u):
                    outs = self.fn(*static_in)
            except (_lib.HipError, RuntimeError) as e:
                _capture_failed(self.name, ent, e)
                return self._eager(xs)
            ent.update(graph=g, static_in=static_in, outs=outs, bumps=cap.bumps, u=u)
            STATS["captures"] += 1
        _refresh_operands(ent, self.modules, self)
        for s, x in zip(ent["static_in"], xs):
            if s.data_ptr() != x.data_ptr():
                s.copy_(x)
        if ent["u"] is not None:
            ent["u"].uniform_()
        ent["graph"].replay()
        for m, d in ent["bumps"]:
            m._nbt += d
        STATS["replays"] += 1
        return ent["outs"]


class _Bridge(torch.autograd.Function):

    @staticmethod
    def forward(ctx, owner, ent, dummy, *outs):
        ctx.owner, ctx.ent = owner, ent
        return tuple(o.detach() for o in outs)

    @staticmethod
    def backward(ctx, *gs):
        ent = ctx.ent
        for buf, g in zip(ent["gouts"], gs):
            if g is None:
                buf.zero_()
            else:
                buf.copy_(g)
        ent["bwd"].replay()
        STATS["replays"] += 1
        return (None, None, None) + (None,) * len(gs)


class GraphedTrain:

    def __init__(self, model, name="student"):
        self.model, self.name, self.cache = model, name, {}
        self._dummy = None

    def _eager(self, x):
        STATS["eager"] += 1
        n = K.dropout_uniforms_needed(self.model, x.shape[0]) if self.model.training else 0
        with K.dropout_pool(torch.empty(n, device=x.device).uniform_() if n else None):
            return self.model(x)

    def __call__(self, x):
        if not (enabled() and torch.is_grad_enabled()):
            return self._eager(x)
        key = _key((x,), (self.model,))
        ent = self.cache.setdefault(key, {"count": 0, "fwd": None})
        if ent["fwd"] is None:
            if ent["count"] < WARM or ent.get("failed", 0) >= 2:
                ent["count"] += 1
                return self._eager(x)
            static_x = x.clone()
            K.prewarm_globals([self.model], x.device)
            bns = _bns([self.model])
            fwd, bwd = torch.cuda.CUDAGraph(), torch.cuda.CUDAGraph()
            pool = torch.cuda.graph_pool_handle()
            n = K.dropout_uniforms_needed(self.model, x.shape[0]) if self.model.training else 0
            u = torch.empty(n, device=x.device) if n else None
            try:
                cap = _Capture(fwd, bns, pool)
                with cap, K.dropout_pool(u):
                    outs = self.model(static_x)
                keys = sorted(outs)
                souts = [outs[k] for k in keys]
                gouts = [torch.zeros_like(o) for o in souts]
                cap_b = _Capture(bwd, bns, pool)
                with cap_b:
                    torch.autograd.backward(souts, gouts)
            except (_lib.HipError, RuntimeError) as e:
                K.wgrad_stream_sync()
                _capture_failed(self.name, ent, e)
                return self._eager(x)
            ent.update(fwd=fwd, bwd=bwd, static_x=static_x, keys=keys, outs=souts, gouts=gouts, bumps=cap.bumps, u=u)
            STATS["captures"] += 2
        if self._dummy is None:
            self._dummy = torch.zeros((), device=x.device, requires_grad=True)
        _refresh_operands(ent, [self.model], self)
        ent["static_x"].copy_(x)
        if ent["u"] is not None:
            ent["u"].uniform_()
        ent["fwd"].replay()
        for m, d in ent["bumps"]:
            m._nbt += d
        STATS["replays"] += 1
        outs = _Bridge.apply(self, ent, self._dummy, *[o.detach() for o in ent["outs"]])
        return dict(zip(ent["keys"], outs))
```

### u2pl_amd/nn.py

```python
import contextlib
import math
import os
import weakref

import torch
import torch.distributed as dist
import torch.nn as nn

from . import _lib
from ._lib import HipError, call, query

from .comm import (COMM_DEBUG, COMM_STATS, _all_reduce, _digest_of, _world, check_comm_sequence, comm_sequence_digest,
                   dist_active, note_collective)
from .layout import _CL, _ws, as_rows, new_act
from .operands import (AMAX_STATS, CONV_H, CONV_WS, PRESPLIT, WEIGHT_EPOCH, _AMAX_POOL, _DerivedCache, _derived, _split_of,
                       _weight_stamp, _ws_ok, amax_of, amax_pool_reset, amax_slot, bump_weight_epoch, invalidate_weights, presplit,
                       set_amax, ws_dgrad, ws_forward, ws_wino)


_WGRAD = {"stream": None, "enabled": os.environ.get("U2PL_NO_WGRAD_STREAM") is None}


def wgrad_stream_sync():
    _WGRAD["queued"] = False
# ... 16 lines not shown
        if t_ is not None:
            t_.record_stream(side)
    if not _WGRAD.get("queued"):
        _WGRAD["queued"] = True
        torch.autograd.Variable._execution_engine.queue_callback(wgrad_stream_sync)
    with torch.cuda.stream(side):
        yield side


def _grad_sink(p):
    return getattr(p, "_u2pl_grad", None)


def _mark_ready(sink):
    if sink is not None:
        owner = getattr(sink, "_u2pl_ready", None)
        if owner is not None:
            owner[0].mark_ready(owner[1])


CONV_ALGO = {"wino": int(os.environ.get("U2PL_CONV_WINO", "4")), "min_gain": float(os.environ.get("U2PL_WINO_MIN_GAIN", "1.7")),
             "wgrad": int(os.environ.get("U2PL_WINO_WGRAD", "1")), "bf16": int(os.environ.get("U2PL_CONV_BF16", "0"))}


def wino_tile(Cin, Cout, R, S, stride, pad, dil, H, W):
    mt = CONV_ALGO["wino"]
    if mt not in (2, 4) or R != 3 or S != 3 or stride != 1 or pad != dil or Cin % 32 or Cout % 4 or Cout < 32:
        return 0
    th, tw = -(-(-(-H // dil)) // mt), -(-(-(-W // dil)) // mt)
    eff = (H * W) / float(dil * dil * th * tw * mt * mt)
    gain = 9.0 * mt * mt / ((mt + 2) ** 2) * eff
    return mt if gain >= CONV_ALGO["min_gain"] else 0


def _out_size(n, k, stride, pad, dil):
    return (n + 2 * pad - dil * (k - 1) - 1) // stride + 1


def _check_weight_layout(weight, cin="Cin"):
    R, S = weight.shape[2:]
    if not weight.is_contiguous(memory_format=_CL) and not (R == 1 and S == 1 and weight.is_contiguous()):
        raise HipError("conv weight must be stored channels_last ([Cout][R][S][%s])" % cin)


def _ws_call(stem, src, head, planes, weight, *rest, h_tail=()):
    if CONV_H["on"]:
        amax = amax_of(src, head[0], head[1])
        call(stem + "_wsh_f32", *head, amax, planes(weight, True), *rest, *h_tail)
        return amax
    call(stem + "_ws_f32", *head, planes(weight, False), *rest)
    return None


def _stem_patches(x, ldx, weight, N, H, W, Cin, Ho, Wo, R, S, stride, pad, dil):
    Cout = weight.shape[0]
    Kp = ((R * S * Cin + 31) // 32) * 32
    col = torch.empty((N * Ho * Wo, Kp), dtype=torch.float32, device=x.device)
    call("u2pl_im2col_f32", x, ldx, col, Kp, N, H, W, Cin, Ho, Wo, R, S, stride, pad, dil)
    wp = torch.zeros((Cout, Kp), dtype=torch.float32, device=x.device)
    wp[:, : R * S * Cin] = weight.permute(0, 2, 3, 1).reshape(Cout, R * S * Cin)
    return col, wp, Kp


def _wino_input(x, ldx, N, H, W, C, dil, mt, tiles, with_amax):
    V = torch.empty((mt + 2) ** 2 * tiles * C, dtype=torch.float32, device=x.device)
    if not with_amax:
        call("u2pl_wino_input_f32", x, ldx, N, H, W, C, dil, mt, V)
        return V, None
    v_amax = amax_slot(x.device)
    call("u2pl_wino_input_amax_f32", x, ldx, N, H, W, C, dil, mt, V, v_amax)
    return V, v_amax


def _wino_conv(x, ldx, weight, bias, y, N, H, W, Cin, Cout, dil, mt, transposed, pivot=None, epi=None, y_amax=None):
    dev = x.device
    a2 = (mt + 2) ** 2
    Ci, Co = (Cout, Cin) if transposed else (Cin, Cout)
    tiles = query("u2pl_wino_tiles", N, H, W, dil, mt)
    ws = _ws_ok(Co, Ci) and weight.is_leaf
    V, v_amax = _wino_input(x, ldx, N, H, W, Ci, dil, mt, tiles, ws and CONV_H["on"])
    Mb = torch.empty(a2 * tiles * Co, dtype=torch.float32, device=dev)
    if ws:
        if v_amax is not None:
            set_amax(V, v_amax)
        _ws_call("u2pl_gemm_batched", V, (V, Ci, tiles * Ci), lambda w, h: ws_wino(w, transposed, mt, h), weight, Mb, Co, tiles * Co,
                 tiles, Ci, Co, a2)
    else:
        U = torch.empty(a2 * Cout * Cin, dtype=torch.float32, device=dev)
        call("u2pl_wino_weight_f32", weight, Cout, Cin, int(transposed), mt, U)
        call("u2pl_gemm_batched_f32", V, Ci, tiles * Ci, U, Co * Ci, Mb, Co, tiles * Co, tiles, Ci, Co, a2)
    part = None
    if pivot is not None:
        nblk = query("u2pl_wino_stat_blocks", tiles, Co)
        part = torch.empty((nblk, 2, Co), dtype=torch.float32, device=dev)
    if epi is not None and y_amax is not None:
        call("u2pl_wino_output_bnact_amax_f32", Mb, N, H, W, Co, dil, mt, bias, y, Co, *epi, y_amax)
    elif epi is not None:
        call("u2pl_wino_output_bnact_f32", Mb, N, H, W, Co, dil, mt, bias, y, Co, *epi)
    else:
        call("u2pl_wino_output_f32", Mb, N, H, W, Co, dil, mt, bias, y, Co, part, pivot)
    return part, V


class _ConvFn(torch.autograd.Function):
    @staticmethod
    def forward(ctx, x, weight, bias, stride, pad, dil, wsink, bsink, pivot=None, recording=True, link=None):
        x_in = x
        x, ldx = as_rows(x)
        N, Cin, H, W = x.shape
        Cout, _, R, S = weight.shape
        Ho, Wo = _out_size(H, R, stride, pad, dil), _out_size(W, S, stride, pad, dil)
        _check_weight_layout(weight)
        ctx.set_materialize_grads(False)
        ctx.link = link
        ctx.x_amax = ctx.col_amax = None
        y = new_act(N, Cout, Ho, Wo, x.device)
        col = None
        use_bf = (bool(CONV_ALGO.get("bf16", 0)) and recording and any(ctx.needs_input_grad[:3]) and Cin % 32 == 0
                  and H * W > 1)
        ctx.bf = use_bf
        sfx = "_bf16op_f32" if use_bf else "_f32"
        geom = (N, H, W, Cin, Ho, Wo, Cout, R, S, stride, pad, dil)
        if H * W == 1 and R == 1 and S == 1 and stride == 1 and pad == 0 and N <= 16 and Cin % 4 == 0:
            call("u2pl_dense_small_f32", x, ldx, weight, bias, y, Cout, N, Cin, Cout)
            pivot = None if pivot is None else False
        elif Cin % 32:
            col, wp, Kp = _stem_patches(x, ldx, weight, N, H, W, Cin, Ho, Wo, R, S, stride, pad, dil)
            call("u2pl_conv2d_fwd_f32", col, Kp, wp, bias, y, Cout, N, Ho, Wo, Kp, Ho, Wo, Cout, 1, 1, 1, 0, 1)
        elif not use_bf and (mt := wino_tile(Cin, Cout, R, S, stride, pad, dil, H, W)):
            part, V = _wino_conv(x, ldx, weight, bias, y, N, H, W, Cin, Cout, dil, mt, False, pivot)
            if ctx.needs_input_grad[1]:
                col = V
                ent = getattr(V, "_u2pl_amax", None)
                ctx.col_amax = ent[0] if ent is not None else None
            if pivot is not None:
                sums = part
        elif pivot is not None and pivot is not False:
            ws = not use_bf and _ws_ok(Cout, R * S * Cin)
            nblk = query("u2pl_igemm_ws_stat_blocks", N, Ho, Wo) if ws else query("u2pl_conv2d_fwd_stat_blocks", N, Ho, Wo, Cout)
            part = torch.empty((nblk, 2, Cout), dtype=torch.float32, device=x.device)
            if ws:
                ctx.x_amax = _ws_call("u2pl_conv2d_fwd_bnstats", x_in, (x, ldx), ws_forward, weight, bias, y, Cout, *geom, pivot, part)
            else:
                call("u2pl_conv2d_fwd_bnstats" + sfx, x, ldx, weight, bias, y, Cout, *geom, pivot, part)
            sums = part
        elif not use_bf and _ws_ok(Cout, R * S * Cin):
            ctx.x_amax = _ws_call("u2pl_conv2d_fwd", x_in, (x, ldx), ws_forward, weight, bias, y, Cout, *geom)
        else:
            call("u2pl_conv2d_fwd" + sfx, x, ldx, weight, bias, y, Cout, *geom)
        ctx.save_for_backward(x, weight, col)
        ctx.geom = geom + (ldx,)
        ctx.has_bias = bias is not None
        ctx.wsink, ctx.bsink = wsink, bsink
        if pivot is not None:
            if Cin % 32 or pivot is False:
                return y, None
            ctx.mark_non_differentiable(sums)
            return y, sums
        return y

    @staticmethod
    def backward(ctx, gy, gsums=None):
        if gy is None:
            return (None,) * 11
        x, weight, col = ctx.saved_tensors
        N, H, W, Cin, Ho, Wo, Cout, R, S, stride, pad, dil, ldx = ctx.geom
        gy_in = gy
        gy, ldg = as_rows(gy)
        dev = gy.device
        M = N * Ho * Wo
        Cp, weight_k = Cout, weight
        if Cout % 32:
            Cp = (Cout + 31) // 32 * 32
            gp = torch.zeros((M, Cp), dtype=torch.float32, device=dev)
            call("u2pl_copy_cols_f32", gy, ldg, gp, Cp, M, Cout)
            gy, ldg = gp, Cp
            weight_k = torch.zeros((Cp, Cin, R, S), dtype=torch.float32, device=dev).contiguous(memory_format=_CL)
            weight_k[:Cout] = weight
        dx = dw = db = None
        join = ctx.link
        if join is not None and not ctx.needs_input_grad[0]:
            raise HipError("gradient join on a convolution whose input needs no gradient")
        if ctx.needs_input_grad[0]:
            dx, included = _conv_dgrad(ctx, gy_in, gy, ldg, weight, weight_k, Cp, join.acc if join is not None else None)
            if join is not None:
                dx = join.settle(dx, included)
        need_w, need_b = ctx.needs_input_grad[1], ctx.has_bias and ctx.needs_input_grad[2]
        wg_mt = (wino_tile(Cin, Cout, R, S, stride, pad, dil, H, W)
                 if need_w and Cp == Cout and not ctx.bf and CONV_ALGO.get("wgrad", 1) else 0)
        wg_h = (CONV_H["on"] and need_w and Cp == Cout and not ctx.bf and Cin % 32 == 0
                and query("u2pl_wgrad_h_eligible", Cin, Cout) == 1)
        gy_amax = x_amax = None
        if wg_h and not wg_mt:
            gy_amax = amax_of(gy_in, gy, ldg)
            x_amax = ctx.x_amax if ctx.x_amax is not None else amax_of(x, x, ldx)
        with _wgrad_side(need_w or need_b, gy, x, col, gy_amax, x_amax, ctx.col_amax) as side:
            if need_w:
                dw = _conv_wgrad(ctx, gy, ldg, x, weight, weight_k, col, Cp, wg_mt, wg_h, gy_amax, x_amax)
                _mark_ready(ctx.wsink)
            if need_b:
                db = _bias_grad(gy, ldg, M, Cp, Cout, ctx.bsink)
        if side is not None and (dw is not None or db is not None):
            torch.cuda.current_stream().wait_stream(side)
        return dx, dw, db, None, None, None, None, None, None, None, None


def _conv_dgrad(ctx, gy_in, gy, ldg, weight, weight_k, Cp, prev):
    N, H, W, Cin, Ho, Wo, Cout, R, S, stride, pad, dil, _ = ctx.geom
    dev = gy.device
    dx = new_act(N, Cin, H, W, dev)
    included = prev is None
    epi = None
    if prev is not None and Cin % 4 == 0:
        one, zero = _identity_bn(Cin, dev)
        rr, ldr = as_rows(prev)
        epi = (zero, one, one, zero, rr, ldr, 0)
    mt = wino_tile(Cp, Cin, R, S, stride, pad, dil, H, W) if (Cp == Cout and not ctx.bf) else 0
    if mt:
        _wino_conv(gy, ldg, weight_k, None, dx, N, H, W, Cin, Cout, dil, mt, True, None, epi)
        included = included or epi is not None
    elif (epi is not None and R == 1 and S == 1 and stride == 1 and pad == 0 and Cp == Cout and not ctx.bf
          and _ws_ok(Cin, Cout)):
        _ws_call("u2pl_conv2d_fwd_bnact", gy_in, (gy, ldg), ws_dgrad, weight, None, dx, Cin, N, H, W, Cout, H, W, Cin, 1, 1, 1, 0, 1,
                 *epi, h_tail=(None,))
        included = True
    elif Cp == Cout and not ctx.bf and _ws_ok(Cin, R * S * Cout):
        _ws_call("u2pl_conv2d_dgrad", gy_in, (gy, ldg), ws_dgrad, weight, dx, Cin, N, H, W, Cin, Ho, Wo, Cout, R, S, stride, pad, dil)
    else:
        wT = torch.empty(Cin * R * S * Cp, dtype=torch.float32, device=dev)
        call("u2pl_weight_transpose_f32", weight_k, wT, Cp, R * S, Cin)
        call("u2pl_conv2d_dgrad_bf16op_f32" if ctx.bf else "u2pl_conv2d_dgrad_f32", gy, ldg, wT, dx, Cin, N, H, W, Cin,
             Ho, Wo, Cp, R, S, stride, pad, dil)
    return dx, included


def _conv_wgrad(ctx, gy, ldg, x, weight, weight_k, col, Cp, mt, wg_h, gy_amax, x_amax):
    N, H, W, Cin, Ho, Wo, Cout, R, S, stride, pad, dil, ldx = ctx.geom
    dev = gy.device
    sink = ctx.wsink
    if Cin % 32:
        Kp = col.shape[1]
        tmp = torch.empty((Cp, Kp), dtype=torch.float32, device=dev)
        wsb = _ws(query("u2pl_conv2d_wgrad_workspace_bytes", N, Ho, Wo, Kp, Cp, 1, 1), dev)
        call("u2pl_conv2d_wgrad_f32", gy, ldg, col, Kp, tmp, wsb, 0, N, Ho, Wo, Kp, Ho, Wo, Cp, 1, 1, 1, 0, 1)
        g = tmp[:Cout, : R * S * Cin].reshape(Cout, R, S, Cin).permute(0, 3, 1, 2)
        if sink is not None:
            sink.add_(g)
            return None
        return g.contiguous(memory_format=_CL)
    if mt:
        a2 = (mt + 2) ** 2
        tiles = query("u2pl_wino_tiles", N, H, W, dil, mt)
        V, v_amax = col, ctx.col_amax
        if V is None:
            V, v_amax = _wino_input(x, ldx, N, H, W, Cin, dil, mt, tiles, wg_h)
        Mg = torch.empty(a2 * tiles * Cout, dtype=torch.float32, device=dev)
        ns = query("u2pl_wgrad_batched_splits", tiles, Cin, Cout, a2)
        part = torch.empty(ns * Cout * a2 * Cin, dtype=torch.float32, device=dev)
        if wg_h:
            if v_amax is None:
                v_amax = amax_slot(dev)
                call("u2pl_absmax_f32", V, Cin, a2 * tiles, Cin, v_amax, 0)
            mg_amax = amax_slot(dev)
            call("u2pl_wino_gy_amax_f32", gy, ldg, N, H, W, Cout, dil, mt, Mg, mg_amax)
            call("u2pl_wgrad_batched_h_f32", Mg, Cout, tiles * Cout, mg_amax, V, Cin, tiles * Cin, v_amax, part, tiles, Cin,
                 Cout, a2)
        else:
            call("u2pl_wino_gy_f32", gy, ldg, N, H, W, Cout, dil, mt, Mg)
            call("u2pl_wgrad_batched_f32", Mg, Cout, tiles * Cout, V, Cin, tiles * Cin, part, tiles, Cin, Cout, a2)
        tgt = sink if sink is not None else torch.empty_like(weight)
        call("u2pl_wino_wgrad_finish_f32", part, ns, Cout, Cin, mt, int(sink is not None), tgt)
        return tgt if sink is None else None
    wsb = _ws(query("u2pl_conv2d_wgrad_workspace_bytes", N, Ho, Wo, Cin, Cp, R, S), dev)
    direct = sink is not None and Cp == Cout
    tgt = sink if direct else torch.empty_like(weight_k)
    if gy_amax is not None:
        call("u2pl_conv2d_wgrad_h_f32", gy, ldg, gy_amax, x, ldx, x_amax, tgt, wsb, int(direct), N, H, W, Cin, Ho, Wo,
             Cp, R, S, stride, pad, dil)
    else:
        call("u2pl_conv2d_wgrad_bf16op_f32" if ctx.bf else "u2pl_conv2d_wgrad_f32", gy, ldg, x, ldx, tgt, wsb,
             int(direct), N, H, W, Cin, Ho, Wo, Cp, R, S, stride, pad, dil)
    if direct:
        return None
    if sink is not None:
        sink.add_(tgt[:Cout])
        return None
    return tgt[:Cout] if Cp != Cout else tgt


def _bias_grad(gy, ldg, M, Cp, Cout, bsink):
    sums = torch.empty(2 * Cp, dtype=torch.float64, device=gy.device)
    wsb = _ws(query("u2pl_colreduce_workspace_bytes", M, 1, Cp), gy.device)
    call("u2pl_colsum_f32", gy, ldg, M, 1, Cp, wsb, sums)
    if bsink is not None:
        call("u2pl_sums_to_f32", sums, Cout, 1.0, 1, bsink)
        _mark_ready(bsink)
        return None
    db = torch.empty(Cout, dtype=torch.float32, device=gy.device)
    call("u2pl_sums_to_f32", sums, Cout, 1.0, 0, db)
    return db


_IDENT_BN = {}


def prewarm_globals(modules, dev):
    for mod in modules:
        for m in mod.modules():
            if isinstance(m, Conv2d):
                _identity_bn(m.in_channels, dev)


def _identity_bn(C, dev):
    k = (C, str(dev))
    v = _IDENT_BN.get(k)
    if v is None:
        v = _IDENT_BN[k] = (torch.ones(C, dtype=torch.float32, device=dev), torch.zeros(C, dtype=torch.float32, device=dev))
    return v


FUSE_RES_GRAD = os.environ.get("U2PL_NO_RES_GRAD_FUSION") is None


class GradJoin:
    __slots__ = ("left", "acc", "armed")

    def __init__(self, n):
        self.left, self.acc, self.armed = n, None, False

    def _check(self):
        if self.left > 0 and self.acc is not None:
            raise HipError("GradJoin: %d wired consumer(s) never ran their backward -- the gradient of the shared input is "
                           "incomplete (set U2PL_NO_RES_GRAD_FUSION=1 for partial backward passes)" % self.left)

    def settle(self, t, included=False):
        if not self.armed:
            self.armed = True
            try:
                torch.autograd.Variable._execution_engine.queue_callback(self._check)
            except RuntimeError:
                pass
        if self.acc is not None and not included:
            t.add_(self.acc)
        self.left -= 1
        if self.left > 0:
            self.acc = t
            return None
        self.acc = None
        return t


def grad_join(x, n):
    if n >= 2 and FUSE_RES_GRAD and torch.is_grad_enabled() and x.requires_grad:
        return GradJoin(n)
    return None


def residual_grad_link(x):
    return grad_join(x, 2)


def dgrad_fusable(conv, x):
    if conv.groups != 1:
        return False
    Cout, Cin, R, S = conv.weight.shape
    H, W = x.shape[2], x.shape[3]
    if R == 1 and S == 1 and conv.stride == 1 and conv.padding == 0:
        return _ws_ok(Cin, Cout) and Cin % 4 == 0 and Cout % 32 == 0
    return bool(wino_tile(Cout, Cin, R, S, conv.stride, conv.padding, conv.dilation, H, W)) and Cout % 32 == 0 and Cin % 4 == 0


def gconv_constraint(Cin, Cout, groups, stride):
    if groups < 1 or Cin % groups or Cout % groups:
        return "in_channels (%d) and out_channels (%d) must be divisible by groups (%d)" % (Cin, Cout, groups)
    cig, cog = Cin // groups, Cout // groups
    if cig % 4 or cog % 4 or cig > 64 or cog > 64:
        return ("channels per group must be a multiple of 4 up to 64, got in %d / out %d (groups=%d; depthwise and odd widths "
                "are not supported)" % (cig, cog, groups))
    if stride not in (1, 2):
        return "stride must be 1 or 2, got %d" % stride
    return None


class _GroupedConvFn(torch.autograd.Function):

    @staticmethod
    def forward(ctx, x, weight, bias, stride, pad, dil, groups, wsink, bsink, link=None):
        x, ldx = as_rows(x)
        N, Cin, H, W = x.shape
        Cout, cig, R, S = weight.shape
        why = gconv_constraint(Cin, Cout, groups, stride)
        if why is None and cig * groups != Cin:
            why = "weight has %d input channels per group, the input %d channels in %d groups" % (cig, Cin, groups)
        if why is not None:
            raise HipError("grouped convolution: " + why)
        _check_weight_layout(weight, "Cin/groups")
        Ho, Wo = _out_size(H, R, stride, pad, dil), _out_size(W, S, stride, pad, dil)
        ctx.set_materialize_grads(False)
        ctx.link = link
        y = new_act(N, Cout, Ho, Wo, x.device)
        call("u2pl_gconv2d_fwd_f32", x, ldx, weight, bias, y, Cout, N, H, W, Cin, Ho, Wo, Cout, R, S, stride, pad, dil, groups)
        ctx.save_for_backward(x, weight)
        ctx.geom = (N, H, W, Cin, Ho, Wo, Cout, R, S, stride, pad, dil, groups, ldx)
        ctx.has_bias = bias is not None
        ctx.wsink, ctx.bsink = wsink, bsink
        return y

    @staticmethod
    def backward(ctx, gy):
        if gy is None:
            return (None,) * 10
        x, weight = ctx.saved_tensors
        N, H, W, Cin, Ho, Wo, Cout, R, S, stride, pad, dil, groups, ldx = ctx.geom
        gy, ldg = as_rows(gy)
        dev = gy.device
        dx = dw = db = None
        join = ctx.link
        if join is not None and not ctx.needs_input_grad[0]:
            raise HipError("gradient join on a convolution whose input needs no gradient")
        if ctx.needs_input_grad[0]:
            dx = new_act(N, Cin, H, W, dev)
            call("u2pl_gconv2d_dgrad_f32", gy, ldg, weight, dx, Cin, N, H, W, Cin, Ho, Wo, Cout, R, S, stride, pad, dil, groups)
            if join is not None:
                dx = join.settle(dx, False)
        need_w, need_b = ctx.needs_input_grad[1], ctx.has_bias and ctx.needs_input_grad[2]
        with _wgrad_side(need_w or need_b, gy, x) as side:
            if need_w:
                sink = ctx.wsink
                wsb = _ws(query("u2pl_gconv2d_wgrad_workspace_bytes", N, Ho, Wo, Cin, Cout, R, S, groups), dev)
                tgt = sink if sink is not None else torch.empty_like(weight)
                call("u2pl_gconv2d_wgrad_f32", gy, ldg, x, ldx, tgt, wsb, int(sink is not None), N, H, W, Cin, Ho, Wo, Cout, R, S,
                     stride, pad, dil, groups)
                if sink is None:
                    dw = tgt
                _mark_ready(sink)
            if need_b:
                db = _bias_grad(gy, ldg, N * Ho * Wo, Cout, Cout, ctx.bsink)
        if side is not None and (dw is not None or db is not None):
            torch.cuda.current_stream().wait_stream(side)
        return dx, dw, db, None, None, None, None, None, None, None


class Conv2d(nn.Module):

    def __init__(self, in_channels, out_channels, kernel_size, stride=1, padding=0, dilation=1, bias=True, groups=1):
        super().__init__()
        k = kernel_size
        if groups < 1 or in_channels % groups or out_channels % groups:
            raise ValueError("in_channels and out_channels must be divisible by groups")
        self.in_channels, self.out_channels, self.groups = in_channels, out_channels, groups
        self.kernel_size, self.stride, self.padding, self.dilation = (k, k), stride, padding, dilation
        w = torch.empty(out_channels, in_channels // groups, k, k)
        nn.init.kaiming_uniform_(w, a=math.sqrt(5))
        self.weight = nn.Parameter(w.contiguous(memory_format=_CL))
        if bias:
            fan_in = (in_channels // groups) * k * k
            bound = 1 / math.sqrt(fan_in) if fan_in > 0 else 0
            b = torch.empty(out_channels)
            nn.init.uniform_(b, -bound, bound)
            self.bias = nn.Parameter(b)
        else:
            self.register_parameter("bias", None)

    def forward(self, x, stat_pivot=None, grad_link=None):
        if self.groups != 1:
            y = _GroupedConvFn.apply(x, self.weight, self.bias, self.stride, self.padding, self.dilation, self.groups,
                                     _grad_sink(self.weight), _grad_sink(self.bias) if self.bias is not None else None, grad_link)
            return y if stat_pivot is None else (y, None)
        out = _ConvFn.apply(x, self.weight, self.bias, self.stride, self.padding, self.dilation,
                            _grad_sink(self.weight), _grad_sink(self.bias) if self.bias is not None else None, stat_pivot,
                            torch.is_grad_enabled(), grad_link)
        return out

    def extra_repr(self):
        s = f"{self.in_channels}, {self.out_channels}, k={self.kernel_size}, s={self.stride}, p={self.padding}, d={self.dilation}"
        return s if self.groups == 1 else s + f", g={self.groups}"


def finished_sums(pre, C, out=None):
    if pre.dtype == torch.float32:
        if out is None:
            out = torch.empty(2 * C + 1, dtype=torch.float64, device=pre.device)
        call("u2pl_colreduce_finish_f32", pre, pre.shape[0], C, out)
        return out
    if out is not None:
        out.copy_(pre)
        return out
    return pre


def _bn_local_sums(x, ldx, mod, pre_sums, out=None, fuse_finish=False):
    N, C, H, W = x.shape
    if pre_sums is not None:
        if fuse_finish and FUSE_BN_FINISH and pre_sums.dtype == torch.float32:
            return pre_sums
        return finished_sums(pre_sums, C, out)
    if out is None:
        out = torch.empty(2 * C + 1, dtype=torch.float64, device=x.device)
    wsb = _ws(query("u2pl_colreduce_workspace_bytes", N * H * W, 1, C), x.device)
    call("u2pl_bn_stats_f32", x, ldx, N * H * W, C, mod.running_mean, wsb, out)
    return out


def _exchange_count(M):
    return float(M * _world())


def _bn_finalize(sums, count, mod):
    C = mod.num_features
    mean = torch.empty(C, dtype=torch.float32, device=sums.device)
    invstd = torch.empty(C, dtype=torch.float32, device=sums.device)
    if sums.dtype == torch.float32:
        call("u2pl_bn_finish_finalize_f32", sums, sums.shape[0], C, count, mod.running_mean, mod.eps, mod.momentum, mean, invstd,
             mod.running_mean, mod.running_var, None)
    else:
        call("u2pl_bn_finalize_f32", sums, count, mod.running_mean, C, mod.eps, mod.momentum, mean, invstd, mod.running_mean,
             mod.running_var)
    mod._nbt += 1
    return mean, invstd


def _act_with_mask_bits(N, C, H, W, device):
    M = N * H * W
    buf = torch.empty(M * C + M * (C // 32), dtype=torch.float32, device=device)
    return buf[:M * C].view(N, H, W, C).permute(0, 3, 1, 2), buf[M * C:].view(torch.int32).view(M, C // 32)


def _bn_apply(x, ldx, mean, invstd, gamma, beta, res, ldr, relu, drop, plain=False, mask_bits=False):
    N, C, H, W = x.shape
    y, bits = _act_with_mask_bits(N, C, H, W, x.device) if mask_bits else (new_act(N, C, H, W, x.device), None)
    act = 3 if mask_bits else int(relu)
    if CONV_H["on"] and not plain:
        y_amax = amax_slot(x.device)
        call("u2pl_bn_apply_amax_f32", x, ldx, mean, invstd, gamma, beta, res, ldr, act, drop, H * W, y, C, N * H * W, C, y_amax)
        set_amax(y, y_amax)
    else:
        call("u2pl_bn_apply_f32", x, ldx, mean, invstd, gamma, beta, res, ldr, act, drop, H * W, y, C, N * H * W, C)
    return (y, bits) if mask_bits else y


def _bn_bwd_sums(gy, ldg, x, ldx, y, mean, invstd, drop, out, gamma=None, rbeta=None, bits=None):
    N, C, H, W = x.shape
    wsb = _ws(query("u2pl_colreduce_workspace_bytes", N * H * W, 1, C), gy.device)
    if bits is not None:
        call("u2pl_bn_bwd_sums_bits_f32", gy, ldg, x, ldx, bits, C // 32, mean, invstd, drop, H * W, N * H * W, C, wsb, out)
    elif rbeta is not None:
        call("u2pl_bn_bwd_sums_mx_f32", gy, ldg, x, ldx, mean, invstd, gamma, rbeta, drop, H * W, N * H * W, C, wsb, out)
    else:
        call("u2pl_bn_bwd_sums_f32", gy, ldg, x, ldx, y, C, mean, invstd, drop, H * W, N * H * W, C, wsb, out)


def _param_grads(sums, C, gsink, bsink, need):
    if not need:
        return None, None
    acc = gsink is not None
    dgamma = gsink if acc else torch.empty(C, dtype=torch.float32, device=sums.device)
    dbeta = bsink if acc else torch.empty(C, dtype=torch.float32, device=sums.device)
    call("u2pl_sums_to_f32", sums[C:], C, 1.0, int(acc), dgamma)
    call("u2pl_sums_to_f32", sums, C, 1.0, int(acc), dbeta)
    if not acc:
        return dgamma, dbeta
    _mark_ready(gsink)
    _mark_ready(bsink)
    return None, None


def _bn_bwd_apply(gy, ldg, x, ldx, y, mean, invstd, gamma, drop, sums, count, with_dres=False, pg=None, rbeta=None, maxima=False,
                  bits=None):
    N, C, H, W = x.shape
    hw, M, dev = H * W, N * H * W, gy.device
    dx = new_act(N, C, H, W, dev)
    dres = new_act(N, C, H, W, dev) if with_dres else None
    psums, gsink, bsink = pg or (None, None, None)
    amax_entry = maxima or rbeta is not None or bits is not None
    if amax_entry:
        dx_amax = amax_slot(dev) if maxima else None
        dres_amax = amax_slot(dev) if (with_dres and maxima) else None
        if bits is not None:
            call("u2pl_bn_bwd_apply_bits_f32", gy, ldg, x, ldx, bits, C // 32, mean, invstd, gamma, drop, hw, sums, count, dx, C,
                 dres, C, M, C, psums, gsink, bsink, 1, dx_amax, dres_amax)
        else:
            call("u2pl_bn_bwd_apply_amax_f32", gy, ldg, x, ldx, y, C, mean, invstd, gamma, drop, hw, sums, count, dx, C, dres, C, M,
                 C, psums, gsink, bsink, 1, dx_amax, dres_amax, rbeta)
        if dx_amax is not None:
            set_amax(dx, dx_amax)
        if dres_amax is not None:
            set_amax(dres, dres_amax)
    elif pg is not None:
        call("u2pl_bn_bwd_apply_pg_f32", gy, ldg, x, ldx, y, C, mean, invstd, gamma, drop, hw, sums, count, dx, C, dres, C, M, C,
             psums, gsink, bsink, 1)
    else:
        call("u2pl_bn_bwd_apply_f32", gy, ldg, x, ldx, y, C, mean, invstd, gamma, drop, hw, sums, count, dx, C, dres, C, M, C)
    if pg is not None:
        _mark_ready(gsink)
        _mark_ready(bsink)
    return dx, dres


class _BNFn(torch.autograd.Function):

    @staticmethod
    def forward(ctx, x, gamma, beta, res, drop, mod, relu, gsink, bsink, pre_sums=None, link=None, record=False):
        x, ldx = as_rows(x)
        N, C, H, W = x.shape
        ctx.link = link if res is not None else None
        rr, ldr = (None, 0) if res is None else as_rows(res)
        exchange = mod.training and mod.sync and dist_active()
        count = float(N * H * W)
        if mod.training:
            sums = _bn_local_sums(x, ldx, mod, pre_sums, fuse_finish=not exchange)
            if exchange:
                _all_reduce(sums[:2 * C], "syncbn_allreduce", group=mod.group)
                count = _exchange_count(N * H * W)
            mean, invstd = _bn_finalize(sums, count, mod)
        else:
            mean, invstd = mod.running_mean, _eval_invstd(mod, C, x.device)
        ctx.mask_from_x = bool(relu and res is None and RELU_MASK_FROM_X and beta is not None)
        ctx.mask_bits = bool(relu and res is not None and RELU_MASK_BITS and C % 32 == 0 and record
                             and any(ctx.needs_input_grad))
        y = _bn_apply(x, ldx, mean, invstd, gamma, beta, rr, ldr, relu, drop, mask_bits=ctx.mask_bits)
        bits = None
        if ctx.mask_bits:
            y, bits = y
        ctx.save_for_backward(x, y if (relu and not ctx.mask_from_x and not ctx.mask_bits) else None, mean, invstd, gamma, drop,
                              beta if ctx.mask_from_x else None, bits)
        ctx.meta = (ldx, mod.training, exchange, count, res is not None)
        ctx.gsink, ctx.bsink, ctx.group = gsink, bsink, mod.group
        return y

    @staticmethod
    def backward(ctx, gy):
        x, y, mean, invstd, gamma, drop, rbeta, bits = ctx.saved_tensors
        ldx, training, exchange, count, has_res = ctx.meta
        need_dx, need_pg, need_dres = ctx.needs_input_grad[0], ctx.needs_input_grad[1], has_res and ctx.needs_input_grad[3]
        if need_dres and not need_dx:
            raise HipError("BatchNorm backward: a residual gradient without an input gradient has no kernel form")
        C = x.shape[1]
        gy, ldg = as_rows(gy)
        sums = torch.empty(2 * C, dtype=torch.float64, device=gy.device)
        _bn_bwd_sums(gy, ldg, x, ldx, y, mean, invstd, drop, sums, gamma, rbeta, bits)
        maxima = CONV_H["on"]
        amax_entry = maxima or rbeta is not None or bits is not None
        pg_fused = FUSE_BN_FINISH and need_pg and ctx.gsink is not None and need_dx and (not exchange or amax_entry)
        dgamma = dbeta = pg = None
        if pg_fused:
            pg = (sums.clone() if exchange else sums, ctx.gsink, ctx.bsink)
        else:
            dgamma, dbeta = _param_grads(sums, C, ctx.gsink, ctx.bsink, need_pg)
        if exchange:
            _all_reduce(sums, "syncbn_allreduce", group=ctx.group)
        dx = dres = None
        if need_dx:
            dx, dres = _bn_bwd_apply(gy, ldg, x, ldx, y, mean, invstd, gamma, drop, sums if training else None, count, need_dres,
                                     pg, rbeta, maxima, bits)
        if ctx.link is not None and dres is not None:
            dres = ctx.link.settle(dres)
        return dx, dgamma, dbeta, dres, None, None, None, None, None, None, None, None


class _BNGroupFn(torch.autograd.Function):

    @staticmethod
    def forward(ctx, n, *flat):
        meta = flat[5 * n]
        units = [as_rows(flat[5 * i]) + flat[5 * i + 1:5 * i + 5] for i in range(n)]
        group = meta[0][0].group
        packed = torch.zeros(sum(2 * u[0].shape[1] + 1 for u in units), dtype=torch.float64, device=units[0][0].device)
        slots, off = [], 0
        for (x, ldx, gamma, beta, drop, pre), (mod, relu, gs, bs) in zip(units, meta):
            slots.append(packed[off:off + 2 * x.shape[1] + 1])
            off += 2 * x.shape[1] + 1
            _bn_local_sums(x, ldx, mod, pre, slots[-1])
        _all_reduce(packed, "syncbn_allreduce", group=group)
        outs, saved, ctx.meta = [], [], []
        for (x, ldx, gamma, beta, drop, pre), (mod, relu, gs, bs), sums in zip(units, meta, slots):
            count = _exchange_count(x.numel() // x.shape[1])
            mean, invstd = _bn_finalize(sums, count, mod)
            y = _bn_apply(x, ldx, mean, invstd, gamma, beta, None, 0, relu, drop)
            outs.append(y)
            saved += [x, y if relu else None, mean, invstd, gamma, drop]
            ctx.meta.append((ldx, count, gs, bs))
        ctx.save_for_backward(*saved)
        ctx.n, ctx.group = n, group
        return tuple(outs)

    @staticmethod
    def backward(ctx, *gys):
        n, sv = ctx.n, ctx.saved_tensors
        packed = torch.empty(sum(2 * sv[6 * i].shape[1] for i in range(n)), dtype=torch.float64, device=gys[0].device)
        work, off = [], 0
        for i in range(n):
            x, y, mean, invstd, gamma, drop = sv[6 * i:6 * i + 6]
            ldx, count, gs, bs = ctx.meta[i]
            C = x.shape[1]
            gy, ldg = as_rows(gys[i])
            sums = packed[off:off + 2 * C]
            off += 2 * C
            _bn_bwd_sums(gy, ldg, x, ldx, y, mean, invstd, drop, sums)
            dg, db = _param_grads(sums, C, gs, bs, ctx.needs_input_grad[1 + 5 * i + 1])
            work.append(((gy, ldg, x, ldx, y, mean, invstd, gamma, drop, sums, count), dg, db))
        _all_reduce(packed, "syncbn_allreduce", group=ctx.group)
        grads = [None]
        for i, (args, dg, db) in enumerate(work):
            dx = _bn_bwd_apply(*args)[0] if ctx.needs_input_grad[1 + 5 * i] else None
            grads += [dx, dg, db, None, None]
        grads.append(None)
        return tuple(grads)


class _BNResPairFn(torch.autograd.Function):

    @staticmethod
    def forward(ctx, xa, ga, ba, pre_a, xb, gb, bb, pre_b, meta):
        (mod_a, gsa, bsa), (mod_b, gsb, bsb) = meta
        xa, lda = as_rows(xa)
        xb, ldb = as_rows(xb)
        N, C, H, W = xa.shape
        packed = torch.zeros(2 * (2 * C + 1), dtype=torch.float64, device=xa.device)
        _bn_local_sums(xa, lda, mod_a, pre_a, packed[:2 * C + 1])
        _bn_local_sums(xb, ldb, mod_b, pre_b, packed[2 * C + 1:])
        _all_reduce(packed, "syncbn_allreduce", group=mod_a.group)
        count = _exchange_count(N * H * W)
        mean_a, inv_a = _bn_finalize(packed[:2 * C + 1], count, mod_a)
        mean_b, inv_b = _bn_finalize(packed[2 * C + 1:], count, mod_b)
        ident = _bn_apply(xb, ldb, mean_b, inv_b, gb, bb, None, 0, False, None, plain=True)
        y = _bn_apply(xa, lda, mean_a, inv_a, ga, ba, ident, C, True, None)
        ctx.save_for_backward(xa, xb, y, mean_a, inv_a, mean_b, inv_b, ga, gb)
        ctx.meta = (lda, ldb, count, gsa, bsa, gsb, bsb, mod_a.group)
        return y

    @staticmethod
    def backward(ctx, gy):
        xa, xb, y, mean_a, inv_a, mean_b, inv_b, ga, gb = ctx.saved_tensors
        lda, ldb, count, gsa, bsa, gsb, bsb, group = ctx.meta
        C = xa.shape[1]
        gy, ldg = as_rows(gy)
        packed = torch.empty(4 * C, dtype=torch.float64, device=gy.device)
        sa, sb = packed[:2 * C], packed[2 * C:]
        _bn_bwd_sums(gy, ldg, xa, lda, y, mean_a, inv_a, None, sa)
        _bn_bwd_sums(gy, ldg, xb, ldb, y, mean_b, inv_b, None, sb)
        dga, dba = _param_grads(sa, C, gsa, bsa, ctx.needs_input_grad[1])
        dgb, dbb = _param_grads(sb, C, gsb, bsb, ctx.needs_input_grad[5])
        _all_reduce(packed, "syncbn_allreduce", group=group)
        dxa = _bn_bwd_apply(gy, ldg, xa, lda, y, mean_a, inv_a, ga, None, sa, count)[0] if ctx.needs_input_grad[0] else None
        dxb = _bn_bwd_apply(gy, ldg, xb, ldb, y, mean_b, inv_b, gb, None, sb, count)[0] if ctx.needs_input_grad[4] else None
        return dxa, dga, dba, None, dxb, dgb, dbb, None, None


def _packable(bns):
    return (dist_active() and os.environ.get("U2PL_NO_SYNCBN_PACK") is None
            and all(b.training and b.sync for b in bns) and len({id(b.group) for b in bns}) == 1)


def _conv_with_stats(conv, bn, x, grad_link=None):
    if conv.in_channels % 32 == 0:
        y, sums = conv(x, stat_pivot=bn.running_mean, grad_link=grad_link)
        return y, sums
    return conv(x, grad_link=grad_link), None


def conv_bn_group(units):
    units = [tuple(u) + (None,) * (6 - len(u)) for u in units]
    if not _packable([u[1] for u in units]) or len(units) < 2:
        return [conv_bn(c, b, x, relu=r, drop=d, grad_link=j) for c, b, x, r, d, j in units]
    flat, meta = [], []
    for conv, bn, x, relu, drop, j in units:
        y, sums = _conv_with_stats(conv, bn, x, j)
        flat += [y, bn.weight, bn.bias, drop, sums]
        meta.append((bn, relu, _grad_sink(bn.weight), _grad_sink(bn.bias)))
    return list(_BNGroupFn.apply(len(units), *flat, meta))


def conv_bn_res_pair(conv_a, bn_a, xa, conv_b, bn_b, xb, grad_link_b=None):
    if not _packable([bn_a, bn_b]):
        identity = conv_bn(conv_b, bn_b, xb, grad_link=grad_link_b)
        return conv_bn(conv_a, bn_a, xa, res=identity, relu=True)
    ya, sa = _conv_with_stats(conv_a, bn_a, xa)
    yb, sb = _conv_with_stats(conv_b, bn_b, xb, grad_link_b)
    meta = ((bn_a, _grad_sink(bn_a.weight), _grad_sink(bn_a.bias)), (bn_b, _grad_sink(bn_b.weight), _grad_sink(bn_b.bias)))
    return _BNResPairFn.apply(ya, bn_a.weight, bn_a.bias, sa, yb, bn_b.weight, bn_b.bias, sb, meta)


def _bn_write_nbt(m, prefix, keep_vars):
    m.num_batches_tracked.fill_(m._nbt)


def _bn_read_nbt(m, incompatible):
    m._nbt = int(m.num_batches_tracked)


class BatchNorm2d(nn.Module):

    def __init__(self, num_features, eps=1e-5, momentum=0.1, sync=False):
        super().__init__()
        self.num_features, self.eps, self.momentum, self.sync = num_features, eps, momentum, sync
        self.group = None
        self.weight = nn.Parameter(torch.ones(num_features))
        self.bias = nn.Parameter(torch.zeros(num_features))
        self.register_buffer("running_mean", torch.zeros(num_features))
        self.register_buffer("running_var", torch.ones(num_features))
        self.register_buffer("num_batches_tracked", torch.tensor(0, dtype=torch.long))
        self._nbt = 0
        self.register_state_dict_pre_hook(_bn_write_nbt)
        self.register_load_state_dict_post_hook(_bn_read_nbt)

    def forward(self, x, res=None, relu=False, drop=None, pre_sums=None, res_link=None):
        return _BNFn.apply(x, self.weight, self.bias, res, drop, self, relu, _grad_sink(self.weight),
                           _grad_sink(self.bias), pre_sums, res_link, torch.is_grad_enabled())


FUSE_EVAL_BN = os.environ.get("U2PL_NO_EVAL_BN_FUSION") is None
RELU_MASK_FROM_X = os.environ.get("U2PL_NO_RELU_MASK_FROM_X") is None
RELU_MASK_BITS = os.environ.get("U2PL_NO_RELU_MASK_BITS") is None
FUSE_BN_FINISH = os.environ.get("U2PL_NO_BN_FINISH_FUSION") is None
_EVAL_INVSTD = {}
_EVAL_PREP = weakref.WeakKeyDictionary()


def _eval_invstd(bn, C, dev):
    v = _EVAL_INVSTD.get(id(bn))
    if v is not None:
        return v
    invstd = torch.empty(C, dtype=torch.float32, device=dev)
    call("u2pl_bn_eval_invstd_f32", bn.running_var, C, bn.eps, invstd)
    return invstd


class eval_invstd:

    def __init__(self, model):
        self.model = model

    def __enter__(self):
        import numpy as np
        if not FUSE_BN_FINISH:
            self.ids = []
            return self
        m = self.model
        bns = [b for b in m.modules() if isinstance(b, BatchNorm2d)]
        key = tuple(b.running_var.data_ptr() for b in bns)
        prep = _EVAL_PREP.get(m)
        if prep is None or prep["key"] != key:
            if not bns or not bns[0].running_var.is_cuda:
                self.ids = []
                return self
            dev = bns[0].running_var.device
            total = sum(b.num_features for b in bns)
            out = torch.empty(total, dtype=torch.float32, device=dev)
            jobs = np.zeros(len(bns), dtype=np.dtype([("rv", "<u8"), ("out", "<u8"), ("begin", "<i8"), ("C", "<i4"), ("eps", "<f4")]))
            assert jobs.dtype.itemsize == query("u2pl_bn_eval_invstd_job_bytes")
            off, views = 0, []
            for i, b in enumerate(bns):
                jobs[i] = (b.running_var.data_ptr(), out.data_ptr() + 4 * off, off, b.num_features, b.eps)
                views.append(out[off:off + b.num_features])
                off += b.num_features
            from .hipops import h2d
            prep = _EVAL_PREP[m] = dict(key=key, bns=bns, out=out, views=views, total=total,
                                        jobs=h2d(torch.from_numpy(jobs.view(np.uint8).copy()), dev))
        call("u2pl_bn_eval_invstd_multi_f32", prep["jobs"], len(prep["bns"]), prep["total"])
        self.ids = [id(b) for b in prep["bns"]]
        for b, v in zip(prep["bns"], prep["views"]):
            _EVAL_INVSTD[id(b)] = v
        return self

    def __exit__(self, *a):
        for i in self.ids:
            _EVAL_INVSTD.pop(i, None)
        return False


def conv_bn_eval(conv, bn, x, res=None, relu=False):
    x_in = x
    x, ldx = as_rows(x)
    N, Cin, H, W = x.shape
    weight, bias = conv.weight, conv.bias
    Cout, _, R, S = weight.shape
    stride, pad, dil = conv.stride, conv.padding, conv.dilation
    if H * W == 1 or Cout % 4:
        return None
    Ho, Wo = _out_size(H, R, stride, pad, dil), _out_size(W, S, stride, pad, dil)
    dev = x.device
    invstd = _eval_invstd(bn, Cout, dev)
    rr, ldr = (None, 0) if res is None else as_rows(res)
    epi = (bn.running_mean, invstd, bn.weight, bn.bias, rr, ldr, int(relu))
    y = new_act(N, Cout, Ho, Wo, dev)
    geom = (N, H, W, Cin, Ho, Wo, Cout, R, S, stride, pad, dil)
    if Cin % 32:
        col, wp, Kp = _stem_patches(x, ldx, weight, N, H, W, Cin, Ho, Wo, R, S, stride, pad, dil)
        call("u2pl_conv2d_fwd_bnact_f32", col, Kp, wp, bias, y, Cout, N, Ho, Wo, Kp, Ho, Wo, Cout, 1, 1, 1, 0, 1, *epi)
    elif mt := wino_tile(Cin, Cout, R, S, stride, pad, dil, H, W):
        y_amax = amax_slot(dev) if CONV_H["on"] else None
        _wino_conv(x, ldx, weight, bias, y, N, H, W, Cin, Cout, dil, mt, False, None, epi, y_amax)
        if y_amax is not None:
            set_amax(y, y_amax)
    elif _ws_ok(Cout, R * S * Cin):
        y_amax = amax_slot(dev) if CONV_H["on"] else None
        _ws_call("u2pl_conv2d_fwd_bnact", x_in, (x, ldx), ws_forward, weight, bias, y, Cout, *geom, *epi, h_tail=(y_amax,))
        if y_amax is not None:
            set_amax(y, y_amax)
    else:
        call("u2pl_conv2d_fwd_bnact_f32", x, ldx, weight, bias, y, Cout, *geom, *epi)
    return y


def conv_bn(conv, bn, x, res=None, relu=False, drop=None, grad_link=None, res_link=None):
    if (FUSE_EVAL_BN and not bn.training and drop is None and conv.groups == 1
            and not (torch.is_grad_enabled() and (x.requires_grad or conv.weight.requires_grad or bn.weight.requires_grad))):
        y = conv_bn_eval(conv, bn, x, res=res, relu=relu)
        if y is not None:
            return y
    if bn.training and conv.in_channels % 32 == 0:
        y, sums = conv(x, stat_pivot=bn.running_mean, grad_link=grad_link)
        return bn(y, res=res, relu=relu, drop=drop, pre_sums=sums, res_link=res_link)
    return bn(conv(x, grad_link=grad_link), res=res, relu=relu, drop=drop, res_link=res_link)


def use_process_group(model, group):
    for m in model.modules():
        if isinstance(m, BatchNorm2d):
            m.group = group


class SyncBatchNorm(BatchNorm2d):
    def __init__(self, num_features, eps=1e-5, momentum=0.1):
        super().__init__(num_features, eps, momentum, sync=True)


DROPOUT_HOOK = None

# ... 229 lines not shown
```

### u2pl_amd/roofline.py

```python
import os
import time

import torch

from . import _lib

PEAK_F32_MFMA_TFLOPS = 157.3
PEAK_HBM_GBS = 8000.0
ALGO_TFLOP_PER_IMAGE_769 = 6.60

_CONV_GEOM = {
    "u2pl_conv2d_fwd_f32": 6, "u2pl_conv2d_fwd_bnstats_f32": 6, "u2pl_conv2d_fwd_bnact_f32": 6, "u2pl_conv2d_dgrad_f32": 5, "u2pl_conv2d_wgrad_f32": 7,
    "u2pl_conv2d_fwd_bf16op_f32": 6, "u2pl_conv2d_fwd_bnstats_bf16op_f32": 6, "u2pl_conv2d_dgrad_bf16op_f32": 5,
    "u2pl_conv2d_wgrad_bf16op_f32": 7,
    "u2pl_conv2d_fwd_ws_f32": 6, "u2pl_conv2d_fwd_bnstats_ws_f32": 6, "u2pl_conv2d_fwd_bnact_ws_f32": 6, "u2pl_conv2d_dgrad_ws_f32": 5,
    "u2pl_conv2d_fwd_wsh_f32": 7, "u2pl_conv2d_fwd_bnstats_wsh_f32": 7, "u2pl_conv2d_fwd_bnact_wsh_f32": 7, "u2pl_conv2d_dgrad_wsh_f32": 6,
    "u2pl_conv2d_wgrad_h_f32": 9,
}
H_NAMES = ("u2pl_conv2d_fwd_wsh_f32", "u2pl_conv2d_fwd_bnstats_wsh_f32", "u2pl_conv2d_fwd_bnact_wsh_f32", "u2pl_conv2d_dgrad_wsh_f32",
           "u2pl_gemm_batched_wsh_f32", "u2pl_conv2d_wgrad_h_f32", "u2pl_wgrad_batched_h_f32")


def piece_products(name):
    return 3 if name in H_NAMES else 6
PEAK_BF16_MFMA_TFLOPS = 2500.0
PEAK_SPLIT_F32_TFLOPS = PEAK_BF16_MFMA_TFLOPS / 6.0


def conv_split_on():
    return bool(_lib.lib().cdll.u2pl_conv_get_split())


def _mfma_fields(ach, pipe_flops=None, flops=None):
    if conv_split_on():
        ratio = (pipe_flops / flops) if (pipe_flops and flops) else 6.0
        peak = PEAK_BF16_MFMA_TFLOPS / ratio
        return {"peak": round(peak, 1), "frac": round(ach / peak, 4),
                "frac_vs_fp32_mfma_peak": round(ach / PEAK_F32_MFMA_TFLOPS, 4),
                "piece_products_per_fp32_product": round(ratio, 3),
                "matrix_pipe_tflops": round(ach * ratio, 1),
                "frac_vs_six_product_bound": round(ach / PEAK_SPLIT_F32_TFLOPS, 4),
                "arithmetic": "fp32 products on the 16-bit matrix cores, fp32 accumulate: THREE fp16 piece products of a two-piece "
                              "split of the power-of-two-scaled operands (v_mfma_f32_32x32x16_f16; default since round 6, "
                              "csrc/conv_geom.h) or SIX bf16 piece products of an exact three-piece split "
                              "(v_mfma_f32_32x32x16_bf16: U2PL_CONV_H=0, and the <= 64-channel layers); U2PL_CONV_SPLIT=0: "
                              "v_mfma_f32_32x32x2_f32.  achieved = fp32-equivalent FLOP/s; peak = 2500 TF (bf16 = fp16 dense) / "
                              "piece_products_per_fp32_product of the launches; frac = matrix-pipe FLOP/s over 2500; "
                              "frac_vs_fp32_mfma_peak = achieved / 157.3"}
    return {"peak": PEAK_F32_MFMA_TFLOPS, "frac": round(ach / PEAK_F32_MFMA_TFLOPS, 4),
            "arithmetic": "v_mfma_f32_32x32x2_f32 (U2PL_CONV_SPLIT=0)"}


def _conv_flops(name, args):
    if name == "u2pl_gemm_batched_f32":
        M, K, Nn, batch = args[8:12]
        return 2.0 * M * K * Nn * batch
    if name == "u2pl_gemm_batched_ws_f32":
        M, K, Nn, batch = args[7:11]
        return 2.0 * M * K * Nn * batch
    if name == "u2pl_gemm_batched_wsh_f32":
        M, K, Nn, batch = args[8:12]
        return 2.0 * M * K * Nn * batch
    if name == "u2pl_wgrad_batched_f32":
        M, Cin, Cout, batch = args[7:11]
        return 2.0 * M * Cin * Cout * batch
    if name == "u2pl_wgrad_batched_h_f32":
        M, Cin, Cout, batch = args[9:13]
        return 2.0 * M * Cin * Cout * batch
    i = _CONV_GEOM[name]
    N, Hin, Win, Cin, Hout, Wout, Cout, R, S = args[i:i + 9]
    return 2.0 * N * Hout * Wout * Cout * R * S * Cin


def _conv_bytes(name, args):
    if name in ("u2pl_gemm_batched_f32", "u2pl_gemm_batched_ws_f32", "u2pl_gemm_batched_wsh_f32"):
        M, K, Nn, batch = args[7:11] if name == "u2pl_gemm_batched_ws_f32" else args[8:12]
        wb = 6 if name.endswith("_ws_f32") else 4
        return batch * (4.0 * M * K + wb * Nn * K + 4.0 * M * Nn)
    i = _CONV_GEOM[name]
    N, Hin, Win, Cin, Hout, Wout, Cout, R, S = args[i:i + 9]
    wb = 6 if "_ws_" in name else 4
    return 4.0 * N * Hin * Win * Cin + wb * Cout * R * S * Cin + 4.0 * N * Hout * Wout * Cout


def profile_step(step_fn):
    _lib.PROFILE = []
    try:
        step_fn()
        torch.cuda.synchronize()
        rec = _lib.PROFILE
    finally:
        _lib.PROFILE = None
    agg, shapes = {}, {}
    agg["_dense"] = replay_dense(rec)
    for name, args, e0, e1, nk, full in [r[:4] + (r[7], r[6]) for r in rec]:
        d = agg.setdefault(name, dict(ms=0.0, calls=0, flops=0.0, kernels=0, bytes=0.0))
        if name in MFMA_GROUPS["igemm"]:
            d["bytes"] += _conv_bytes(name, args)
            ri = 23 if "_wsh_" in name else 22
            if "_bnact" in name and len(full) > ri and full[ri] is not None:
                i = _CONV_GEOM[name]
                d["bytes"] += 4.0 * args[i] * args[i + 4] * args[i + 5] * args[i + 6]
        ms = e0.elapsed_time(e1)
        d["ms"] += ms
        d["calls"] += 1
        d["kernels"] += nk
        if name in ("u2pl_wgrad_batched_f32", "u2pl_wgrad_batched_h_f32"):
            d["flops"] += _conv_flops(name, args)
        elif name in ("u2pl_gemm_batched_f32", "u2pl_gemm_batched_ws_f32", "u2pl_gemm_batched_wsh_f32"):
            fl = _conv_flops(name, args)
            d["flops"] += fl
            o = 7 if name == "u2pl_gemm_batched_ws_f32" else 8
            key = ("wino_gemm", args[o + 3], args[o], 1, args[o + 1], args[o], 1, args[o + 2], 1, 1, 1, 0, 1)
            sd = shapes.setdefault(key, dict(ms=0.0, calls=0, flops=0.0))
            sd["ms"] += ms
            sd["calls"] += 1
            sd["flops"] += fl
        elif name in _CONV_GEOM:
            fl = _conv_flops(name, args)
            d["flops"] += fl
            i = _CONV_GEOM[name]
            key = (name[12:-4].replace("fwd_bnstats", "fwd").replace("fwd_bnact", "fwd").replace("_bf16op", "@bf16").replace("_wsh", "@wsh").replace("_ws", "@ws"),) + tuple(args[i:i + 9]) + tuple(args[i + 9:i + 12])
            sd = shapes.setdefault(key, dict(ms=0.0, calls=0, flops=0.0))
            sd["ms"] += ms
            sd["calls"] += 1
            sd["flops"] += fl
    agg["_shapes"] = shapes
    return agg


MFMA_GROUPS = {
    "igemm": ("u2pl_conv2d_fwd_f32", "u2pl_conv2d_fwd_bnstats_f32", "u2pl_conv2d_fwd_bnact_f32", "u2pl_conv2d_dgrad_f32",
              "u2pl_gemm_batched_f32", "u2pl_conv2d_fwd_ws_f32", "u2pl_conv2d_fwd_bnstats_ws_f32", "u2pl_conv2d_fwd_bnact_ws_f32",
              "u2pl_conv2d_dgrad_ws_f32", "u2pl_gemm_batched_ws_f32",
              "u2pl_conv2d_fwd_wsh_f32", "u2pl_conv2d_fwd_bnstats_wsh_f32", "u2pl_conv2d_fwd_bnact_wsh_f32",
              "u2pl_conv2d_dgrad_wsh_f32", "u2pl_gemm_batched_wsh_f32"),
    "wgrad": ("u2pl_conv2d_wgrad_f32", "u2pl_wgrad_batched_f32", "u2pl_conv2d_wgrad_h_f32", "u2pl_wgrad_batched_h_f32"),
    "bf16": ("u2pl_conv2d_fwd_bf16op_f32", "u2pl_conv2d_fwd_bnstats_bf16op_f32", "u2pl_conv2d_dgrad_bf16op_f32",
             "u2pl_conv2d_wgrad_bf16op_f32"),
}


def replay_dense(rec):
    out = {}
    for gname, names in MFMA_GROUPS.items():
        calls = [(r[4], r[5]) for r in rec if r[0] in names]
        if not calls:
            continue
        sp = _lib.stream_ptr()
        torch.cuda.synchronize()
        e0, e1 = torch.cuda.Event(enable_timing=True), torch.cuda.Event(enable_timing=True)
        torch.cuda._sleep(40_000_000)
        e0.record()
        for fn, conv in calls:
            fn(*conv, sp)
        e1.record()
        torch.cuda.synchronize()
        out[gname] = e0.elapsed_time(e1)
    return out


def replay_hbm_group(reps=10):
    from . import hipops as H

    R = H.REPLAY or {}
    out = {}

    def timed(fn):
        torch.cuda.synchronize()
        e0, e1 = torch.cuda.Event(enable_timing=True), torch.cuda.Event(enable_timing=True)
        torch.cuda._sleep(60_000_000)
        e0.record()
        for _ in range(reps):
            fn()
        e1.record()
        torch.cuda.synchronize()
        return e0.elapsed_time(e1) / reps * 1e3

    saved, H.REPLAY = H.REPLAY, None
    try:
        if "rel" in R:
            tl, hw, label_l, label_u, low_shape, percents, neg_high = R["rel"]
            out["reliability_us"] = timed(lambda: H.reliability_split(tl, hw, label_l, label_u, low_shape, percents,
                                                                      negative_high_entropy=neg_high))
        if "phase1" in R:
            out["phase1_us"] = timed(lambda: H.contra_phase1(*R["phase1"]))
        if "append" in R:
            dd, n, D, ld, mx = R["append"][:5]
            out["bank_append_us"] = timed(lambda: _lib.call("u2pl_bank_append_multi_f32", dd, n, D, ld, mx))
        if "enqueue" in R and R.get("bank") is not None:
            bank = R["bank"]
            rows, ld, idx, idx_stride, counts_dev = R["enqueue"]
            st0 = bank.state.clone()
            scratch = torch.empty_like(bank.storage)
            st = st0.clone()

            def enq():
                _lib.call("u2pl_bank_enqueue_f32", st, scratch, bank.D, rows, ld, idx, idx_stride, None, counts_dev, bank.C)
            out["bank_append_us"] = timed(enq)
            del scratch
        if "infonce" in R:
            rep_rows, jobs_dev, njobs, Q, K, temp, valid_seg, groups, keep = R["infonce"]

            def nce():
                H.infonce_kernels_once(rep_rows, jobs_dev, njobs, Q, K, temp, valid_seg, groups)
            out["infonce_fwd_bwd_us"] = timed(nce)
    finally:
        H.REPLAY = saved
    return out


def split_phase_table():
    from . import hipops as H
    names = [(18, "A_tile_and_labels"), (19, "A_entropies"), (10, "A_owner_hist"), (11, "P_scan_prefix_totals"), (12, "P_counting_sort"), (13, "P_run_stores"), (1, "P_drain"),
             (2, "barrier"), (14, "C_totals_scan"), (15, "C_ranks_bins_lists"), (16, "G_prefix_pairs"), (17, "G_block_prefix"),
             (3, "G_members"), (8, "D_sync"), (9, "D_select"), (5, "D_thresholds"), (6, "apply"), (7, "end")]
    out = {}
    for slot in H._RF_WS.values():
        acc = slot[1][7168:7200].cpu().numpy().astype("int64")
        if acc[31] <= 0:
            continue
        prev = 0.0
        for k, nm in names:
            cur = acc[k] / acc[31]
            out[nm] = round((cur - prev) / 100.0, 2)
            prev = cur
        out["launches"] = int(acc[31])
        break
    return out


def kernel_source_hash():
    import hashlib
    root = os.path.dirname(os.path.abspath(__file__))
    hs = hashlib.sha256()
    files = []
    for d in (os.path.join(root, "csrc"), os.path.join(os.path.dirname(root), "include")):
        files += [os.path.join(d, f) for f in sorted(os.listdir(d)) if f.endswith((".hip", ".h"))]
    for f in files:
        hs.update(os.path.basename(f).encode())
        hs.update(open(f, "rb").read())
    return hs.hexdigest()[:12]


def hbm_algorithmic_bytes(B, C, H, W, h, w, D, stats):
    px = B * H * W
    rel = px * (4 * C + 24) + (2 * 4 + 8) * 2 * B * h * w
    Q, K = stats.get("Q", 256), stats.get("K", 50)
    con = (2 * D * h * w * 4 + 2 * B * C * h * w * 4 + 2 * B * h * w * 9 + stats.get("n_keys", 0) * D * 4
           + stats.get("njobs", 0) * Q * (2 + K) * D * 4 + stats.get("njobs", 0) * Q * D * 4)
    return rel, con


def measure(trainer, batch, args, ms_per_step):
    from .utils import loss_helper as LH

    from . import hipops as H

    il, ll, iu = batch
    saved = getattr(trainer, "_side", None)
    trainer._side = torch.cuda.current_stream()
    H.REPLAY = {}
    try:
        agg = profile_step(lambda: trainer.train_step(il, ll, iu, epoch=1))
        replay = replay_hbm_group()
    finally:
        trainer._side = saved
        H.REPLAY = None
    shapes = agg.pop("_shapes")
    dense = agg.pop("_dense")
    out = {}
    if os.environ.get("U2PL_BENCH_SHAPES"):
        top = sorted(shapes.items(), key=lambda kv: -kv[1]["ms"])[:40]
        out["conv_shapes"] = [dict(op=k[0], N=k[1], Hin=k[2], Cin=k[4], Hout=k[5], Cout=k[7], k=k[8], s=k[10], d=k[12],
                                   calls=v["calls"], ms=round(v["ms"], 2),
                                   tflops=round(v["flops"] / (v["ms"] * 1e-3) / 1e12, 1)) for k, v in top]
    ig = [(n_, agg.get(n_)) for n_ in MFMA_GROUPS["igemm"]]
    pipe = sum(x["flops"] * piece_products(n_) for n_, x in ig if x)
    ig = [x for _, x in ig if x]
    if ig:
        fl, t_ev, n = sum(x["flops"] for x in ig), sum(x["ms"] for x in ig), sum(x["calls"] for x in ig)
        nker = sum(x["kernels"] for x in ig)
        t = dense.get("igemm", t_ev)
        ach = fl / (t * 1e-3) / 1e12
        out["roofline"] = {"kernel": "k_igemm_ws / k_conv_igemm (direct conv fwd [+BN-stat / eval-BN epilogue] + dgrad, and the batched Winograd component GEMMs; executed fp32 FLOPs)", "bound": "mfma",
                           "achieved": round(ach, 2), **_mfma_fields(ach, pipe, fl), "unit": "TFLOP/s", "traffic": None,
                           "abi_calls_per_step": n, "kernel_launches_per_step": nker, "avg_launch_ms": round(t / max(nker, 1), 4),
                           "avg_abi_call_ms": round(t / n, 4),
                           "executed_tflop_per_step": round(fl / 1e12, 3), "ms_per_step": round(t, 2),
# ... 104 lines not shown
```

Baseline: 37.86.

## Defer residual-branch gradient materialization by applying ReLU mask inside dgrad epilogue

In BN backward for residual bottlenecks, the residual gradient (gy masked by the ReLU bit mask) is no longer written as a separate tensor. The raw upstream gradient and the mask bits are parked in a slot or join, and the pointwise dgrad conv reads them, applying the mask through new MRES variants of the igemm epilogue (bit loads plus ds_bpermute). This removes a full-size elementwise write and read of the residual gradient per block. In exchange it adds new kernel template instantiations, extra bit loads in the epilogue, and more fragile autograd bookkeeping that raises errors on unsupported paths.

```diff
diff --git a/include/u2pl_hip.h b/include/u2pl_hip.h
--- a/include/u2pl_hip.h
+++ b/include/u2pl_hip.h
@@ -208,6 +208,11 @@
                                  int Hin, int Win, int Cin, int Hout, int Wout, int Cout, int R, int S, int stride,
                                  int pad, int dil, const float* mean, const float* invstd, const float* gamma,
                                  const float* beta, const float* res, long ldr, int relu, hipStream_t stream);
+int u2pl_conv2d_fwd_bnact_mres_ws_f32(const float* x, long ldx, const void* wsplit, const float* bias, float* y, long ldy, int N,
+                                      int Hin, int Win, int Cin, int Hout, int Wout, int Cout, int R, int S, int stride,
+                                      int pad, int dil, const float* mean, const float* invstd, const float* gamma,
+                                      const float* beta, const float* res, long ldr, const unsigned* res_bits, long ldb, int relu,
+                                      hipStream_t stream);
 int u2pl_conv2d_dgrad_ws_f32(const float* dy, long lddy, const void* wTsplit, float* dx, long lddx, int N, int Hin,
                              int Win, int Cin, int Hout, int Wout, int Cout, int R, int S, int stride, int pad, int dil,
                              hipStream_t stream);
@@ -262,6 +267,11 @@
                                   long ldy, int N, int Hin, int Win, int Cin, int Hout, int Wout, int Cout, int R, int S,
                                   int stride, int pad, int dil, const float* mean, const float* invstd, const float* gamma,
                                   const float* beta, const float* res, long ldr, int relu, float* y_amax, hipStream_t stream);
+int u2pl_conv2d_fwd_bnact_mres_wsh_f32(const float* x, long ldx, const float* x_amax, const void* wsplit, const float* bias, float* y,
+                                       long ldy, int N, int Hin, int Win, int Cin, int Hout, int Wout, int Cout, int R, int S,
+                                       int stride, int pad, int dil, const float* mean, const float* invstd, const float* gamma,
+                                       const float* beta, const float* res, long ldr, const unsigned* res_bits, long ldb, int relu,
+                                       float* y_amax, hipStream_t stream);
 int u2pl_conv2d_dgrad_wsh_f32(const float* dy, long lddy, const float* dy_amax, const void* wTsplit, float* dx, long lddx, int N,
                               int Hin, int Win, int Cin, int Hout, int Wout, int Cout, int R, int S, int stride, int pad, int dil,
                               hipStream_t stream);
diff --git a/u2pl_amd/csrc/common.h b/u2pl_amd/csrc/common.h
--- a/u2pl_amd/csrc/common.h
+++ b/u2pl_amd/csrc/common.h
@@ -178,4 +178,6 @@
     long ldr;
     int relu;
     unsigned* y_amax;
+    const unsigned* res_bits;
+    long ldb;
 };
diff --git a/u2pl_amd/csrc/igemm_ws.hip b/u2pl_amd/csrc/igemm_ws.hip
--- a/u2pl_amd/csrc/igemm_ws.hip
+++ b/u2pl_amd/csrc/igemm_ws.hip
@@ -547,7 +547,7 @@
 static unsigned long long* g_ws_stamps = nullptr;
 U2PL_API int u2pl_igemm_ws_set_stamp_buffer(void* p) { g_ws_stamps = (unsigned long long*)p; return 0; }
 #endif
-template <int TM, int TN, int WM, int WN, bool PW, int ABL = 0, int NP = 3>
+template <int TM, int TN, int WM, int WN, bool PW, int ABL = 0, int NP = 3, bool MRES = false>
 __device__ __forceinline__ void igemm_ws_body(
     const float* __restrict__ x, long ldx, const float* __restrict__ x_amax, const unsigned short* __restrict__ ws,
     const unsigned* __restrict__ b_amax, const float* __restrict__ bias,
@@ -992,17 +992,37 @@
         if (bn_all) {
             const int ldrb = (int)epi.ldr * 4;
             const __amdgpu_buffer_rsrc_t rr = make_rsrc(epi.res, resbytes);
+            const int ldbb = (int)epi.ldb * 4;
+            const __amdgpu_buffer_rsrc_t rbits =
+                make_rsrc(epi.res_bits, MRES ? (unsigned)(((M - 1) * epi.ldb + (g.Cout >> 5)) * 4) : 0u);
 #pragma unroll
             for (int b = 0; b < TN; ++b) {
                 const int col = n0 + wn * 32 * TN + b * 32 + li;
                 float rv[TM][16];
                 if (epi.res) {
+                    int wd[TM];
+                    if constexpr (MRES) {
+#pragma unroll
+                        for (int a = 0; a < TM; ++a) {
+                            const int boff = col < g.Cout ? (mrow - 4 * lh + a * 32 + li) * ldbb + (col >> 5) * 4 : OOB_OFF;
+                            wd[a] = (int)__builtin_amdgcn_raw_buffer_load_b32(rbits, boff, 0, 0);
+                        }
+                    }
 #pragma unroll
                     for (int a = 0; a < TM; ++a) {
                         const int rbase = col < g.Cout ? ((mrow + a * 32) * (int)epi.ldr + col) * 4 : OOB_OFF;
 #pragma unroll
                         for (int e = 0; e < 16; ++e)
                             rv[a][e] = __uint_as_float(__builtin_amdgcn_raw_buffer_load_b32(rr, rbase + ((e & 3) + 8 * (e >> 2)) * ldrb, 0, 0));
+                    }
+                    if constexpr (MRES) {
+#pragma unroll
+                        for (int a = 0; a < TM; ++a)
+#pragma unroll
+                            for (int e = 0; e < 16; ++e) {
+                                const int w = __builtin_amdgcn_ds_bpermute(((e & 3) + 8 * (e >> 2) + 4 * lh) * 4, wd[a]);
+                                rv[a][e] = __uint_as_float(__float_as_uint(rv[a][e]) & (unsigned)__builtin_amdgcn_sbfe(w, li, 1));
+                            }
                     }
                 }
 #pragma unroll
@@ -1105,17 +1125,17 @@
 #endif
 }
 
-template <int TM, int TN, int WM, int WN, bool PW, int ABL = 0, int NP = 3>
+template <int TM, int TN, int WM, int WN, bool PW, int ABL = 0, int NP = 3, bool MRES = false>
 __global__ __launch_bounds__(64 * WM * WN, (WM * WN) / 4) void k_igemm_ws(
     const float* __restrict__ x, long ldx, const float* __restrict__ x_amax, const unsigned short* __restrict__ ws,
     const unsigned* __restrict__ b_amax, const float* __restrict__ bias,
     float* __restrict__ y, long ldy, ConvGeom g, unsigned xbytes, unsigned wsbytes, unsigned ybytes, unsigned resbytes, int Np,
     float* __restrict__ stats, const float* __restrict__ pivot, long zx, long zws, long zy, BnEpi epi, int mtiles, int ntiles,
     int total_tiles, int tile0) {
-    igemm_ws_body<TM, TN, WM, WN, PW, ABL, NP>(x, ldx, x_amax, ws, b_amax, bias, y, ldy, g, xbytes, wsbytes, ybytes, resbytes, Np, stats,
+    igemm_ws_body<TM, TN, WM, WN, PW, ABL, NP, MRES>(x, ldx, x_amax, ws, b_amax, bias, y, ldy, g, xbytes, wsbytes, ybytes, resbytes, Np, stats,
                                                pivot, zx, zws, zy, epi, mtiles, ntiles, total_tiles, tile0, (int)blockIdx.x, (int)gridDim.x);
 }
-template <bool PW, int NP = 3>
+template <bool PW, int NP = 3, bool MRES = false>
 __global__ __launch_bounds__(512, 2) void k_igemm_ws_mix(
     const float* __restrict__ x, long ldx, const float* __restrict__ x_amax, const unsigned short* __restrict__ ws,
     const unsigned* __restrict__ b_amax, const float* __restrict__ bias,
@@ -1123,10 +1143,10 @@
     float* __restrict__ stats, const float* __restrict__ pivot, long zx, long zws, long zy, BnEpi epi, int mtiles, int ntiles_w,
     int nwide, int wide_tiles, int narrow_tiles) {
     if ((int)blockIdx.x < nwide)
-        igemm_ws_body<2, 2, 2, 4, PW, 0, NP>(x, ldx, x_amax, ws, b_amax, bias, y, ldy, g, xbytes, wsbytes, ybytes, resbytes, Np, stats, pivot,
+        igemm_ws_body<2, 2, 2, 4, PW, 0, NP, MRES>(x, ldx, x_amax, ws, b_amax, bias, y, ldy, g, xbytes, wsbytes, ybytes, resbytes, Np, stats, pivot,
                                              zx, zws, zy, epi, mtiles, ntiles_w, wide_tiles, 0, (int)blockIdx.x, nwide);
     else
-        igemm_ws_body<2, 1, 2, 4, PW, 0, NP>(x, ldx, x_amax, ws, b_amax, bias, y, ldy, g, xbytes, wsbytes, ybytes, resbytes, Np, stats, pivot,
+        igemm_ws_body<2, 1, 2, 4, PW, 0, NP, MRES>(x, ldx, x_amax, ws, b_amax, bias, y, ldy, g, xbytes, wsbytes, ybytes, resbytes, Np, stats, pivot,
                                              zx, zws, zy, epi, mtiles, 2 * ntiles_w, narrow_tiles, 2 * wide_tiles, (int)blockIdx.x - nwide,
                                              (int)gridDim.x - nwide);
 }
@@ -1143,7 +1163,7 @@
     return g_ws_persist;
 }
 U2PL_API int u2pl_igemm_ws_set_persist(int on) { const int old = ws_persist(); g_ws_persist = on != 0; return old; }
-template <int TM, int TN, int WM, int WN, bool PW, int ABL = 0, int NP = 3>
+template <int TM, int TN, int WM, int WN, bool PW, int ABL = 0, int NP = 3, bool MRES = false>
 static int launch_igemm_ws(const float* x, long ldx, const float* x_amax, const void* ws, const float* bias, float* y, long ldy,
                            const ConvGeom& g, hipStream_t stream, float* stats, const float* pivot, int batch, long zx,
                            long zy, const BnEpi* epi, long tile_first = 0, long tile_count = -1) {
@@ -1155,7 +1175,7 @@
     const size_t lds = (size_t)2 * NP * (BM + BN) * WS_ROW_B + (size_t)8 * BN * sizeof(float);
     static bool attr_set = false;
     if (!attr_set) {
-        (void)hipFuncSetAttribute((const void*)k_igemm_ws<TM, TN, WM, WN, PW, ABL, NP>, hipFuncAttributeMaxDynamicSharedMemorySize, (int)lds);
+        (void)hipFuncSetAttribute((const void*)k_igemm_ws<TM, TN, WM, WN, PW, ABL, NP, MRES>, hipFuncAttributeMaxDynamicSharedMemorySize, (int)lds);
         attr_set = true;
     }
     if (NP == 2 && !x_amax) return U2PL_EINVAL;
@@ -1166,6 +1186,8 @@
     if (xb >= (1L << 31) || wsb1 >= (1L << 31) || yb >= (1L << 31)) return U2PL_EINVAL;
     const long resb = ep.res ? ((M - 1) * ep.ldr + g.Cout) * 4 : 0;
     if (resb >= (1L << 31)) return U2PL_EINVAL;
+    if (MRES != (ep.res_bits != nullptr) || (MRES && !ep.res)) return U2PL_EINVAL;
+    if (MRES && ((M - 1) * ep.ldb + g.Cout / 32) * 4 >= (1L << 31)) return U2PL_EINVAL;
     const int mtiles = cdiv(M, BM), ntiles = cdiv(g.Cout, BN);
     const long all_tiles = (long)mtiles * ntiles * batch;
     if (all_tiles >= (1L << 30)) return U2PL_EINVAL;
@@ -1175,14 +1197,14 @@
 #ifdef U2PL_WS_STAMPS
     (void)hipMemcpyToSymbolAsync(HIP_SYMBOL(d_ws_stamps), &g_ws_stamps, sizeof(void*), 0, hipMemcpyHostToDevice, stream);
 #endif
-    U2PL_LAUNCH((k_igemm_ws<TM, TN, WM, WN, PW, ABL, NP>), dim3(grid), dim3(64 * WM * WN), lds, stream, x, ldx, x_amax,
+    U2PL_LAUNCH((k_igemm_ws<TM, TN, WM, WN, PW, ABL, NP, MRES>), dim3(grid), dim3(64 * WM * WN), lds, stream, x, ldx, x_amax,
                 (const unsigned short*)ws, b_amax, bias, y, ldy, g, (unsigned)xb, (unsigned)wsb1, (unsigned)yb, (unsigned)resb, Np, stats, pivot, zx,
                 wsb1 / 2, zy, ep, mtiles, ntiles, (int)total, (int)tile_first);
     U2PL_LAUNCH_CHECK();
     return 0;
 }
 
-template <bool PW, int NP = 3>
+template <bool PW, int NP = 3, bool MRES = false>
 static int launch_igemm_ws_mix(const float* x, long ldx, const float* x_amax, const void* ws, const float* bias, float* y, long ldy,
                                const ConvGeom& g, hipStream_t stream, float* stats, const float* pivot, int batch, long zx,
                                long zy, const BnEpi* epi, long wide_tiles, long narrow_tiles) {
@@ -1192,7 +1214,7 @@
     const size_t lds = (size_t)2 * NP * (128 + 256) * WS_ROW_B + (size_t)8 * 256 * sizeof(float);
     static bool attr_set = false;
     if (!attr_set) {
-        (void)hipFuncSetAttribute((const void*)k_igemm_ws_mix<PW, NP>, hipFuncAttributeMaxDynamicSharedMemorySize, (int)lds);
+        (void)hipFuncSetAttribute((const void*)k_igemm_ws_mix<PW, NP, MRES>, hipFuncAttributeMaxDynamicSharedMemorySize, (int)lds);
         attr_set = true;
     }
     if (NP == 2 && !x_amax) return U2PL_EINVAL;
@@ -1203,9 +1225,11 @@
     if (xb >= (1L << 31) || wsb1 >= (1L << 31) || yb >= (1L << 31)) return U2PL_EINVAL;
     const long resb = ep.res ? ((M - 1) * ep.ldr + g.Cout) * 4 : 0;
     if (resb >= (1L << 31)) return U2PL_EINVAL;
+    if (MRES != (ep.res_bits != nullptr) || (MRES && !ep.res)) return U2PL_EINVAL;
+    if (MRES && ((M - 1) * ep.ldb + g.Cout / 32) * 4 >= (1L << 31)) return U2PL_EINVAL;
     const int mtiles = cdiv(M, 128), ntw = cdiv(g.Cout, 256);
     if ((long)mtiles * 2 * ntw * batch >= (1L << 30)) return U2PL_EINVAL;
-    U2PL_LAUNCH((k_igemm_ws_mix<PW, NP>), dim3((unsigned)(WS_NUM_CUS + narrow_tiles)), dim3(512), lds, stream, x, ldx, x_amax,
+    U2PL_LAUNCH((k_igemm_ws_mix<PW, NP, MRES>), dim3((unsigned)(WS_NUM_CUS + narrow_tiles)), dim3(512), lds, stream, x, ldx, x_amax,
                 (const unsigned short*)ws, b_amax, bias, y, ldy, g, (unsigned)xb, (unsigned)wsb1, (unsigned)yb, (unsigned)resb, Np, stats, pivot, zx,
                 wsb1 / 2, zy, ep, mtiles, ntw, WS_NUM_CUS, (int)wide_tiles, (int)narrow_tiles);
     U2PL_LAUNCH_CHECK();
@@ -1225,14 +1249,19 @@
     if (epi && (stats || batch != 1 || (g.Cout & 3))) return U2PL_EINVAL;
     const bool pw = g.R == 1 && g.S == 1 && g.mul == 1 && g.off_h == 0 && g.off_w == 0 && g.log2div == 0 &&
                     g.Hin == g.Hout && g.Win == g.Wout;
+    const bool mres = epi && epi->res_bits;
+    if (mres && (!pw || !epi->res || (g.Cout & 31))) return U2PL_EINVAL;
     auto go = [&](bool narrow, long first, long count) {
+        if (mres)
+            return narrow ? launch_igemm_ws<2, 1, 2, 4, true, 0, NP, true>(x, ldx, x_amax, ws, bias, y, ldy, g, stream, stats, pivot, batch, zx, zy, epi, first, count)
+                          : launch_igemm_ws<2, 2, 2, 4, true, 0, NP, true>(x, ldx, x_amax, ws, bias, y, ldy, g, stream, stats, pivot, batch, zx, zy, epi, first, count);
         if (!narrow) return pw ? launch_igemm_ws<2, 2, 2, 4, true, 0, NP>(x, ldx, x_amax, ws, bias, y, ldy, g, stream, stats, pivot, batch, zx, zy, epi, first, count)
                                : launch_igemm_ws<2, 2, 2, 4, false, 0, NP>(x, ldx, x_amax, ws, bias, y, ldy, g, stream, stats, pivot, batch, zx, zy, epi, first, count);
         return pw ? launch_igemm_ws<2, 1, 2, 4, true, 0, NP>(x, ldx, x_amax, ws, bias, y, ldy, g, stream, stats, pivot, batch, zx, zy, epi, first, count)
                   : launch_igemm_ws<2, 1, 2, 4, false, 0, NP>(x, ldx, x_amax, ws, bias, y, ldy, g, stream, stats, pivot, batch, zx, zy, epi, first, count);
     };
 #ifdef U2PL_WS_ABLATE
-    if (g_ws_abl && g.Cout > 128 && pw) {
+    if (g_ws_abl && g.Cout > 128 && pw && !mres) {
 #define WS_ABL(A_) case A_: return launch_igemm_ws<2, 2, 2, 4, true, A_, NP>(x, ldx, x_amax, ws, bias, y, ldy, g, stream, stats, pivot, batch, zx, zy, epi)
         switch (g_ws_abl) { WS_ABL(1); WS_ABL(2); WS_ABL(4); WS_ABL(8); WS_ABL(16); WS_ABL(32); WS_ABL(7); WS_ABL(15); WS_ABL(31); WS_ABL(63); default: return U2PL_EINVAL; }
 #undef WS_ABL
@@ -1256,6 +1285,8 @@
     if (two_launch < 0) { const char* e = getenv("U2PL_WS_MIX2"); two_launch = (e && *e) ? (atoi(e) != 0) : 0; }
     const double cm = can_mix ? (double)(full / WS_NUM_CUS) * cw1 + cn1 + (two_launch ? 8.0 : 2.0) * fix : 1e30;
     if (cm < 0.97 * cw && cm < cn) {
+        if (!two_launch && mres)
+            return launch_igemm_ws_mix<true, NP, true>(x, ldx, x_amax, ws, bias, y, ldy, g, stream, stats, pivot, batch, zx, zy, epi, full, 2 * rem);
         if (!two_launch)
             return pw ? launch_igemm_ws_mix<true, NP>(x, ldx, x_amax, ws, bias, y, ldy, g, stream, stats, pivot, batch, zx, zy, epi, full, 2 * rem)
                       : launch_igemm_ws_mix<false, NP>(x, ldx, x_amax, ws, bias, y, ldy, g, stream, stats, pivot, batch, zx, zy, epi, full, 2 * rem);
@@ -1297,6 +1328,16 @@
     const BnEpi epi = {mean, invstd, gamma, beta, res, ldr, relu, nullptr};
     return run_igemm_ws(x, ldx, wsplit, bias, y, ldy, g, stream, nullptr, nullptr, 1, 0, 0, &epi);
 }
+U2PL_API int u2pl_conv2d_fwd_bnact_mres_ws_f32(const float* x, long ldx, const void* wsplit, const float* bias, float* y,
+                                               long ldy, int N, int Hin, int Win, int Cin, int Hout, int Wout, int Cout, int R,
+                                               int S, int stride, int pad, int dil, const float* mean, const float* invstd,
+                                               const float* gamma, const float* beta, const float* res, long ldr,
+                                               const unsigned* res_bits, long ldb, int relu, hipStream_t stream) {
+    if (!mean || !invstd || !gamma || !beta || (Cout & 31) || !res || !res_bits || (ldr & 3) || ldb < Cout / 32) return U2PL_EINVAL;
+    ConvGeom g = {N, Hin, Win, Cin, Hout, Wout, Cout, R, S, stride, -pad, -pad, dil, 0};
+    const BnEpi epi = {mean, invstd, gamma, beta, res, ldr, relu, nullptr, res_bits, ldb};
+    return run_igemm_ws(x, ldx, wsplit, bias, y, ldy, g, stream, nullptr, nullptr, 1, 0, 0, &epi);
+}
 U2PL_API int u2pl_conv2d_dgrad_ws_f32(const float* dy, long lddy, const void* wTsplit, float* dx, long lddx, int N, int Hin,
                                       int Win, int Cin, int Hout, int Wout, int Cout, int R, int S, int stride, int pad,
                                       int dil, hipStream_t stream) {
@@ -1339,6 +1380,17 @@
     const BnEpi epi = {mean, invstd, gamma, beta, res, ldr, relu, (unsigned*)y_amax};
     return run_igemm_ws(x, ldx, wsplit, bias, y, ldy, g, stream, nullptr, nullptr, 1, 0, 0, &epi, x_amax);
 }
+U2PL_API int u2pl_conv2d_fwd_bnact_mres_wsh_f32(const float* x, long ldx, const float* x_amax, const void* wsplit, const float* bias, float* y,
+                                                long ldy, int N, int Hin, int Win, int Cin, int Hout, int Wout, int Cout, int R,
+                                                int S, int stride, int pad, int dil, const float* mean, const float* invstd,
+                                                const float* gamma, const float* beta, const float* res, long ldr,
+                                                const unsigned* res_bits, long ldb, int relu, float* y_amax, hipStream_t stream) {
+    if (!x_amax || !mean || !invstd || !gamma || !beta || (Cout & 31) || !res || !res_bits || (ldr & 3) || ldb < Cout / 32)
+        return U2PL_EINVAL;
+    ConvGeom g = {N, Hin, Win, Cin, Hout, Wout, Cout, R, S, stride, -pad, -pad, dil, 0};
+    const BnEpi epi = {mean, invstd, gamma, beta, res, ldr, relu, (unsigned*)y_amax, res_bits, ldb};
+    return run_igemm_ws(x, ldx, wsplit, bias, y, ldy, g, stream, nullptr, nullptr, 1, 0, 0, &epi, x_amax);
+}
 U2PL_API int u2pl_conv2d_dgrad_wsh_f32(const float* dy, long lddy, const float* dy_amax, const void* wTsplit, float* dx, long lddx, int N,
                                        int Hin, int Win, int Cin, int Hout, int Wout, int Cout, int R, int S, int stride, int pad,
                                        int dil, hipStream_t stream) {
diff --git a/u2pl_amd/graphs.py b/u2pl_amd/graphs.py
--- a/u2pl_amd/graphs.py
+++ b/u2pl_amd/graphs.py
@@ -82,7 +82,8 @@
 
 def _key(xs, modules):
     algo = tuple(sorted(K.CONV_ALGO.items())) + (K.CONV_WS["on"], K.CONV_H["on"], _lib.query("u2pl_conv_get_split"), K.FUSE_EVAL_BN,
-                                                 K._WGRAD["enabled"], K.FUSE_BN_FINISH, K.FUSE_RES_GRAD, K.RELU_MASK_FROM_X)
+                                                 K._WGRAD["enabled"], K.FUSE_BN_FINISH, K.FUSE_RES_GRAD, K.RELU_MASK_FROM_X, K.RELU_MASK_BITS,
+                                                 K.LAZY_DRES)
     bn = tuple(b.training for mod in modules for b in mod.modules() if isinstance(b, K.BatchNorm2d))
     rg = tuple(p.requires_grad for mod in modules for p in mod.parameters())
     return (tuple((tuple(x.shape), x.dtype, x.device.index) for x in xs) + tuple(m.training for m in modules) + algo
diff --git a/u2pl_amd/nn.py b/u2pl_amd/nn.py
--- a/u2pl_amd/nn.py
+++ b/u2pl_amd/nn.py
@@ -192,6 +192,8 @@
         ctx.geom = geom + (ldx,)
         ctx.has_bias = bias is not None
         ctx.wsink, ctx.bsink = wsink, bsink
+        if link is not None:
+            link.lazy = link.lazy is None and LAZY_DRES and Cin % 32 == 0 and _pw_dgrad_fused(ctx.geom, use_bf)
         if pivot is not None:
             if Cin % 32 or pivot is False:
                 return y, None
@@ -251,16 +253,24 @@
     dx = new_act(N, Cin, H, W, dev)
     included = prev is None
     epi = None
+    masked = isinstance(prev, MaskedGrad)
     if prev is not None and Cin % 4 == 0:
         one, zero = _identity_bn(Cin, dev)
-        rr, ldr = as_rows(prev)
+        rr, ldr = (prev.gy, prev.ldg) if masked else as_rows(prev)
         epi = (zero, one, one, zero, rr, ldr, 0)
     mt = wino_tile(Cp, Cin, R, S, stride, pad, dil, H, W) if (Cp == Cout and not ctx.bf) else 0
+    pw = epi is not None and Cp == Cout and _pw_dgrad_fused(ctx.geom, ctx.bf)
+    if masked and (mt or not pw or Cin % 32 or tuple(prev.gy.shape) != (N, Cin, H, W)):
+        raise HipError("a masked residual gradient reached a data gradient that cannot read it (a switch changed between the "
+                       "forward and the backward pass?): set U2PL_NO_LAZY_DRES=1")
     if mt:
         _wino_conv(gy, ldg, weight_k, None, dx, N, H, W, Cin, Cout, dil, mt, True, None, epi)
         included = included or epi is not None
-    elif (epi is not None and R == 1 and S == 1 and stride == 1 and pad == 0 and Cp == Cout and not ctx.bf
-          and _ws_ok(Cin, Cout)):
+    elif pw and masked:
+        _ws_call("u2pl_conv2d_fwd_bnact_mres", gy_in, (gy, ldg), ws_dgrad, weight, None, dx, Cin, N, H, W, Cout, H, W, Cin, 1, 1, 1, 0, 1,
+                 zero, one, one, zero, rr, ldr, prev.bits, prev.ldb, 0, h_tail=(None,))
+        included = True
+    elif pw:
         _ws_call("u2pl_conv2d_fwd_bnact", gy_in, (gy, ldg), ws_dgrad, weight, None, dx, Cin, N, H, W, Cout, H, W, Cin, 1, 1, 1, 0, 1,
                  *epi, h_tail=(None,))
         included = True
@@ -341,6 +351,11 @@
     return db
 
 
+def _pw_dgrad_fused(geom, bf):
+    Cin, Cout, R, S, stride, pad = geom[3], geom[6], geom[7], geom[8], geom[9], geom[10]
+    return R == 1 and S == 1 and stride == 1 and pad == 0 and Cout % 32 == 0 and not bf and _ws_ok(Cin, Cout)
+
+
 _IDENT_BN = {}
 
 
@@ -362,24 +377,54 @@
 FUSE_RES_GRAD = os.environ.get("U2PL_NO_RES_GRAD_FUSION") is None
 
 
+LAZY_DRES = os.environ.get("U2PL_NO_LAZY_DRES") is None
+
+
+class MaskedGrad:
+    __slots__ = ("gy", "ldg", "bits", "ldb")
+
+    def __init__(self, gy, ldg, bits, ldb):
+        self.gy, self.ldg, self.bits, self.ldb = gy, ldg, bits, ldb
+
+
+class ResidualSlot:
+    __slots__ = ("rec",)
+
+    def __init__(self):
+        self.rec = None
+
+
 class GradJoin:
-    __slots__ = ("left", "acc", "armed")
+    __slots__ = ("left", "acc", "armed", "lazy")
 
     def __init__(self, n):
         self.left, self.acc, self.armed = n, None, False
+        self.lazy = None
 
     def _check(self):
         if self.left > 0 and self.acc is not None:
             raise HipError("GradJoin: %d wired consumer(s) never ran their backward -- the gradient of the shared input is "
                            "incomplete (set U2PL_NO_RES_GRAD_FUSION=1 for partial backward passes)" % self.left)
 
-    def settle(self, t, included=False):
+    def _arm(self):
         if not self.armed:
             self.armed = True
             try:
                 torch.autograd.Variable._execution_engine.queue_callback(self._check)
             except RuntimeError:
                 pass
+
+    def park(self, rec):
+        if self.lazy is not True or self.acc is not None or self.left < 2:
+            raise HipError("GradJoin: a masked gradient can only be parked first, for a convolution that reads it")
+        self._arm()
+        self.left -= 1
+        self.acc = rec
+
+    def settle(self, t, included=False):
+        self._arm()
+        if isinstance(self.acc, MaskedGrad) and not included:
+            raise HipError("GradJoin: a masked residual gradient has no in-place add form (set U2PL_NO_LAZY_DRES=1)")
         if self.acc is not None and not included:
             t.add_(self.acc)
         self.left -= 1
@@ -643,7 +688,7 @@
     def forward(ctx, x, gamma, beta, res, drop, mod, relu, gsink, bsink, pre_sums=None, link=None, record=False):
         x, ldx = as_rows(x)
         N, C, H, W = x.shape
-        ctx.link = link if res is not None else None
+        ctx.link = link if (res is not None or isinstance(link, ResidualSlot)) else None
         rr, ldr = (None, 0) if res is None else as_rows(res)
         exchange = mod.training and mod.sync and dist_active()
         count = float(N * H * W)
@@ -676,7 +721,14 @@
         if need_dres and not need_dx:
             raise HipError("BatchNorm backward: a residual gradient without an input gradient has no kernel form")
         C = x.shape[1]
+        link = ctx.link
+        gy_in = gy
         gy, ldg = as_rows(gy)
+        if isinstance(link, ResidualSlot) and not has_res and link.rec is not None:
+            rec, link.rec = link.rec, None
+            if y is not None or rbeta is not None or tuple(rec.gy.shape) != tuple(x.shape) or rec.ldb != C // 32:
+                raise HipError("BatchNorm backward: a masked residual gradient reached a layer that cannot read it")
+            gy, ldg, bits = rec.gy, rec.ldg, rec.bits
         sums = torch.empty(2 * C, dtype=torch.float64, device=gy.device)
         _bn_bwd_sums(gy, ldg, x, ldx, y, mean, invstd, drop, sums, gamma, rbeta, bits)
         maxima = CONV_H["on"]
@@ -689,12 +741,20 @@
             dgamma, dbeta = _param_grads(sums, C, ctx.gsink, ctx.bsink, need_pg)
         if exchange:
             _all_reduce(sums, "syncbn_allreduce", group=ctx.group)
+        lazy = bool(need_dres and need_dx and has_res and ctx.mask_bits and drop is None
+                    and (isinstance(link, ResidualSlot) or (isinstance(link, GradJoin) and link.lazy is True
+                                                            and link.acc is None and link.left > 1)))
         dx = dres = None
         if need_dx:
-            dx, dres = _bn_bwd_apply(gy, ldg, x, ldx, y, mean, invstd, gamma, drop, sums if training else None, count, need_dres,
-                                     pg, rbeta, maxima, bits)
-        if ctx.link is not None and dres is not None:
-            dres = ctx.link.settle(dres)
+            dx, dres = _bn_bwd_apply(gy, ldg, x, ldx, y, mean, invstd, gamma, drop, sums if training else None, count,
+                                     need_dres and not lazy, pg, rbeta, maxima, bits)
+        if lazy and isinstance(link, GradJoin):
+            link.park(MaskedGrad(gy, ldg, bits, C // 32))
+        elif lazy:
+            link.rec = MaskedGrad(gy, ldg, bits, C // 32)
+            dres = gy_in
+        elif isinstance(link, GradJoin) and dres is not None:
+            dres = link.settle(dres)
         return dx, dgamma, dbeta, dres, None, None, None, None, None, None, None, None
 
 
@@ -813,8 +873,9 @@
 
 def conv_bn_res_pair(conv_a, bn_a, xa, conv_b, bn_b, xb, grad_link_b=None):
     if not _packable([bn_a, bn_b]):
-        identity = conv_bn(conv_b, bn_b, xb, grad_link=grad_link_b)
-        return conv_bn(conv_a, bn_a, xa, res=identity, relu=True)
+        slot = ResidualSlot() if (LAZY_DRES and torch.is_grad_enabled()) else None
+        identity = conv_bn(conv_b, bn_b, xb, grad_link=grad_link_b, res_link=slot)
+        return conv_bn(conv_a, bn_a, xa, res=identity, relu=True, res_link=slot)
     ya, sa = _conv_with_stats(conv_a, bn_a, xa)
     yb, sb = _conv_with_stats(conv_b, bn_b, xb, grad_link_b)
     meta = ((bn_a, _grad_sink(bn_a.weight), _grad_sink(bn_a.bias)), (bn_b, _grad_sink(bn_b.weight), _grad_sink(bn_b.bias)))
diff --git a/u2pl_amd/roofline.py b/u2pl_amd/roofline.py
--- a/u2pl_amd/roofline.py
+++ b/u2pl_amd/roofline.py
@@ -14,11 +14,12 @@
     "u2pl_conv2d_fwd_bf16op_f32": 6, "u2pl_conv2d_fwd_bnstats_bf16op_f32": 6, "u2pl_conv2d_dgrad_bf16op_f32": 5,
     "u2pl_conv2d_wgrad_bf16op_f32": 7,
     "u2pl_conv2d_fwd_ws_f32": 6, "u2pl_conv2d_fwd_bnstats_ws_f32": 6, "u2pl_conv2d_fwd_bnact_ws_f32": 6, "u2pl_conv2d_dgrad_ws_f32": 5,
+    "u2pl_conv2d_fwd_bnact_mres_ws_f32": 6,
     "u2pl_conv2d_fwd_wsh_f32": 7, "u2pl_conv2d_fwd_bnstats_wsh_f32": 7, "u2pl_conv2d_fwd_bnact_wsh_f32": 7, "u2pl_conv2d_dgrad_wsh_f32": 6,
-    "u2pl_conv2d_wgrad_h_f32": 9,
+    "u2pl_conv2d_fwd_bnact_mres_wsh_f32": 7, "u2pl_conv2d_wgrad_h_f32": 9,
 }
 H_NAMES = ("u2pl_conv2d_fwd_wsh_f32", "u2pl_conv2d_fwd_bnstats_wsh_f32", "u2pl_conv2d_fwd_bnact_wsh_f32", "u2pl_conv2d_dgrad_wsh_f32",
-           "u2pl_gemm_batched_wsh_f32", "u2pl_conv2d_wgrad_h_f32", "u2pl_wgrad_batched_h_f32")
+           "u2pl_gemm_batched_wsh_f32", "u2pl_conv2d_wgrad_h_f32", "u2pl_wgrad_batched_h_f32", "u2pl_conv2d_fwd_bnact_mres_wsh_f32")
 
 
 def piece_products(name):
@@ -120,7 +121,7 @@
             fl = _conv_flops(name, args)
             d["flops"] += fl
             i = _CONV_GEOM[name]
-            key = (name[12:-4].replace("fwd_bnstats", "fwd").replace("fwd_bnact", "fwd").replace("_bf16op", "@bf16").replace("_wsh", "@wsh").replace("_ws", "@ws"),) + tuple(args[i:i + 9]) + tuple(args[i + 9:i + 12])
+            key = (name[12:-4].replace("fwd_bnstats", "fwd").replace("fwd_bnact_mres", "fwd").replace("fwd_bnact", "fwd").replace("_bf16op", "@bf16").replace("_wsh", "@wsh").replace("_ws", "@ws"),) + tuple(args[i:i + 9]) + tuple(args[i + 9:i + 12])
             sd = shapes.setdefault(key, dict(ms=0.0, calls=0, flops=0.0))
             sd["ms"] += ms
             sd["calls"] += 1
@@ -134,7 +135,8 @@
               "u2pl_gemm_batched_f32", "u2pl_conv2d_fwd_ws_f32", "u2pl_conv2d_fwd_bnstats_ws_f32", "u2pl_conv2d_fwd_bnact_ws_f32",
               "u2pl_conv2d_dgrad_ws_f32", "u2pl_gemm_batched_ws_f32",
               "u2pl_conv2d_fwd_wsh_f32", "u2pl_conv2d_fwd_bnstats_wsh_f32", "u2pl_conv2d_fwd_bnact_wsh_f32",
-              "u2pl_conv2d_dgrad_wsh_f32", "u2pl_gemm_batched_wsh_f32"),
+              "u2pl_conv2d_dgrad_wsh_f32", "u2pl_gemm_batched_wsh_f32",
+              "u2pl_conv2d_fwd_bnact_mres_ws_f32", "u2pl_conv2d_fwd_bnact_mres_wsh_f32"),
     "wgrad": ("u2pl_conv2d_wgrad_f32", "u2pl_wgrad_batched_f32", "u2pl_conv2d_wgrad_h_f32", "u2pl_wgrad_batched_h_f32"),
     "bf16": ("u2pl_conv2d_fwd_bf16op_f32", "u2pl_conv2d_fwd_bnstats_bf16op_f32", "u2pl_conv2d_dgrad_bf16op_f32",
              "u2pl_conv2d_wgrad_bf16op_f32"),
```

After: 37.54. No clear change (-0.8%).
